# ThomasBrouwer/BNMTF

Measured on NVIDIA B200. Metric: BNMF Gibbs+VB sweeps/sec at 65536x32768 K=20, higher is better.
Workload: dtype f64 (statistics: 48-bit fixed point, exact int8 tcgen05 accumulation; solver, moments, draws: IEEE fp64)

## Files before the change

### bnmtf_b200/_lib.py

```python
import ctypes
import os

_HERE = os.path.dirname(os.path.abspath(__file__))
LIB_PATH = os.environ.get("BNMTF_LIB") or os.path.join(_HERE, "libbnmtf_b200.so")

c_i, c_i64, c_u64, c_d, c_p = ctypes.c_int, ctypes.c_int64, ctypes.c_uint64, ctypes.c_double, ctypes.c_void_p

SIGNATURES = {
    "bnmtf_version": [],
    "bnmtf_last_error": [],
    "bnmtf_ld_for": [c_i64],
    "bnmtf_kp_for": [c_i],
    "bnmtf_gram_len": [c_i],
    "bnmtf_pack_dataset_f64": [c_p, c_p, c_i64, c_i64, c_i64, c_p, c_p, c_p],
    "bnmtf_pack_mask_f64": [c_p, c_i64, c_i64, c_i64, c_p, c_p],
    "bnmtf_transpose_dataset_f64": [c_p, c_p, c_i64, c_i64, c_i64, c_p, c_p, c_i64, c_p],
    "bnmtf_pad_factor_f64": [c_p, c_p, c_i64, c_i, c_i64, c_p, c_p, c_p],
    "bnmtf_stats_rx_f64": [c_p, c_p, c_i64, c_i64, c_p, c_i, c_i, c_p, c_p],
    "bnmtf_fixed_point_digits": [],
    "bnmtf_rx_planes_bytes": [c_i64, c_i64],
    "bnmtf_rx_planes_pack_f64": [c_p, c_p, c_i64, c_i64, c_p, c_p, c_p, c_p, c_p],
    "bnmtf_peer_sync_bytes": [],
    "bnmtf_peer_sync_f64": [c_p, c_p, c_i, c_i, c_i, c_p, c_i, c_p],
    "bnmtf_peer_put_f64": [c_p, c_p, c_i64, c_i64, c_i, c_i, c_p],
    "bnmtf_accumulate_f64": [c_p, c_p, c_i64, c_p],
    "bnmtf_sample_mean_f64": [c_p, c_i64, c_i, c_i, c_i, c_p, c_p],
    "bnmtf_range_guard_f64": [c_p, c_i, c_i64, c_p, c_i, c_i, c_i64, c_p, c_p, c_p, c_p],
    "bnmtf_stats_gated_f64": [c_p, c_p, c_p, c_i64, c_i64, c_p, c_p, c_i, c_i, c_i, c_i, c_p, c_p, c_p, c_p],
    "bnmtf_rx_umma_workspace_bytes": [c_i, c_i64],
    "bnmtf_stats_rx_umma_f64": [c_p, c_p, c_p, c_p, c_i64, c_i64, c_i64, c_p, c_i, c_i, c_i, c_p, c_p, c_i64, c_p],
    "bnmtf_stats_gram_f64": [c_p, c_i64, c_i64, c_p, c_p, c_i, c_i, c_i, c_p, c_p, c_p],
    "bnmtf_gram_full_f64": [c_p, c_p, c_i64, c_i, c_i64, c_p, c_p, c_p],
    "bnmtf_small_cluster_size": [c_i64, c_i64, c_i, c_i],
    "bnmtf_small_sweeps_f64": [c_i, c_p, c_p, c_p, c_p, c_i64, c_i64, c_i64, c_i64, c_i, c_p, c_p, c_p, c_p, c_p, c_p, c_p, c_p,
                               c_p, c_p, c_p, c_p, c_p, c_i64, c_d, c_d, c_d, c_d, c_d, c_d, c_u64, c_i, c_p, c_p, c_p, c_p, c_i, c_i, c_p, c_p, c_p],
    "bnmtf_small_tri_cluster_size": [c_i64, c_i64, c_i, c_i, c_i],
    "bnmtf_small_tri_sweeps_f64": [c_i, c_p, c_p, c_p, c_p, c_i64, c_i64, c_i64, c_i64, c_i, c_i, c_p, c_p, c_p, c_p, c_p, c_p, c_i64,
                                   c_d, c_d, c_d, c_d, c_d, c_d, c_u64, c_i, c_p, c_p, c_p, c_p, c_p, c_p, c_p, c_p, c_p],
    "bnmtf_kmeans_distances_f64": [c_p, c_p, c_i64, c_i64, c_p, c_p, c_i, c_p, c_p],
    "bnmtf_stats_gram_fixup_f64": [c_p, c_i64, c_i64, c_i64, c_p, c_p, c_i, c_i, c_p, c_p, c_p],
    "bnmtf_gram_umma_workspace_bytes": [c_i, c_i, c_i64],
    "bnmtf_stats_gram_umma_f64": [c_p, c_i64, c_i64, c_i64, c_p, c_p, c_i, c_i, c_i, c_i, c_i, c_i, c_i, c_p, c_p, c_p,
                                  c_i64, c_p],
    "bnmf_row_solve_f64": [c_i, c_i64, c_i, c_i, c_i, c_i, c_p, c_p, c_p, c_p, c_p, c_p, c_p, c_p, c_p, c_p, c_p,
                           c_i, c_i, c_d, c_u64, c_p, c_u64, c_i64, c_p, c_p, c_p, c_p, c_p, c_i, c_i, c_p, c_p],
    "bnmtf_masked_metrics_f64": [c_p, c_p, c_i64, c_i64, c_p, c_p, c_i, c_i, c_p, c_p, c_p, c_p, c_p],
    "bnmtf_mstat_reduce_f64": [c_p, c_i64, c_p, c_p, c_p],
    "bnmtf_csr_stats_f64": [c_p, c_p, c_p, c_p, c_p, c_p, c_i64, c_i, c_p, c_p, c_i64, c_p, c_p, c_i, c_p, c_p, c_p, c_p, c_p,
                            c_p, c_p],
    "bnmtf_csr_metrics_f64": [c_p, c_p, c_p, c_i64, c_p, c_p, c_i, c_p, c_i, c_p, c_p, c_p],
    "bnmtf_metrics_from_sums_f64": [c_p, c_p, c_d, c_p, c_p, c_p],
    "bnmtf_select_metrics_f64": [c_p, c_p, c_p, c_p],
    "bnmtf_dense_metrics_f64": [c_p, c_p, c_p, c_i64, c_p, c_i, c_p, c_p],
    "bnmtf_vb_factor_terms_f64": [c_p, c_p, c_p, c_p, c_p, c_i64, c_p, c_i, c_p],
    "bnmtf_reduce8_f64": [c_p, c_i, c_p, c_p],
    "bnmtf_reduce1_f64": [c_p, c_i64, c_p, c_p],
    "bnmf_finish_sweep_f64": [c_i, c_d, c_d, c_d, c_d, c_d, c_i64, c_p, c_p, c_p, c_p, c_p, c_p, c_i, c_u64, c_i, c_p, c_p],
    "bnmtf_nmtf_transform_f64": [c_i64, c_i, c_i, c_i, c_i, c_p, c_p, c_p, c_p, c_p, c_p, c_p, c_p, c_p, c_p],
    "bnmtf_nmtf_sq_f64": [c_i64, c_i, c_i, c_i, c_i, c_p, c_p, c_p, c_p, c_p, c_p, c_p, c_i, c_p, c_p],
    "bnmtf_nmtf_sq_scratch_len": [c_i, c_i, c_i],
    "bnmtf_nmtf_sq_parts": [c_i64, c_i, c_i, c_i],
    "bnmtf_coord_solve_f64": [c_i, c_i, c_p, c_p, c_p, c_p, c_p, c_p, c_p, c_p, c_p, c_p, c_i, c_i, c_d, c_u64, c_p, c_u64, c_p],
    "bnmtf_nmtf_extra_f64": [c_i64, c_i, c_i, c_i, c_p, c_p, c_p, c_p, c_p, c_p, c_p, c_p, c_p],
    "bnmtf_nmtf_mstat_f64": [c_i64, c_i, c_i, c_i, c_p, c_p, c_p, c_p, c_p, c_p, c_p],
    "bnmtf_np_build_pred_f64": [c_p, c_p, c_i64, c_i64, c_i64, c_i, c_p, c_p],
    "bnmtf_np_row_update_f64": [c_p, c_p, c_p, c_i64, c_i64, c_i64, c_p, c_p, c_i, c_p],
    "bnmtf_np_s_update_f64": [c_p, c_p, c_p, c_i64, c_i64, c_i64, c_p, c_i, c_i, c_p, c_i, c_i, c_p, c_p, c_i, c_p],
    "bnmtf_np_metrics_f64": [c_p, c_p, c_p, c_i64, c_i64, c_i64, c_p, c_i, c_p, c_p],
    "bnmtf_small_matmul_f64": [c_p, c_p, c_i64, c_i, c_i, c_i, c_p, c_p],
    "bnmtf_tn_moments_f64": [c_p, c_p, c_i64, c_p, c_p, c_p],
    "bnmtf_tn_draw_f64": [c_p, c_p, c_i64, c_u64, c_u64, c_p, c_p],
    "bnmtf_gamma_draw_f64": [c_d, c_d, c_i64, c_u64, c_u64, c_p, c_p],
    "bnmtf_exponential_draw_f64": [c_p, c_i64, c_u64, c_u64, c_p, c_p],
}
_RESTYPES = {"bnmtf_nmtf_sq_scratch_len": c_i64, "bnmtf_last_error": ctypes.c_char_p, "bnmtf_ld_for": c_i64, "bnmtf_gram_len": c_i64,
             "bnmtf_gram_umma_workspace_bytes": c_i64, "bnmtf_rx_planes_bytes": c_i64,
             "bnmtf_rx_umma_workspace_bytes": c_i64, "bnmtf_peer_sync_bytes": c_i64}
_PLAIN = {"bnmtf_nmtf_sq_scratch_len", "bnmtf_nmtf_sq_parts", "bnmtf_small_cluster_size", "bnmtf_small_tri_cluster_size", "bnmtf_fixed_point_digits", "bnmtf_version", "bnmtf_last_error", "bnmtf_ld_for", "bnmtf_kp_for", "bnmtf_gram_len",
          "bnmtf_gram_umma_workspace_bytes", "bnmtf_rx_planes_bytes", "bnmtf_rx_umma_workspace_bytes", "bnmtf_peer_sync_bytes"}

_lib = None

KERNELS_PER_CALL = {"bnmtf_pack_dataset_f64": 1, "bnmtf_pack_mask_f64": 1, "bnmtf_transpose_dataset_f64": 1,
                    "bnmtf_pad_factor_f64": 1, "bnmtf_stats_rx_f64": 1, "bnmtf_stats_rx_umma_f64": 5,
                    "bnmtf_rx_planes_pack_f64": 2, "bnmtf_range_guard_f64": 1, "bnmtf_stats_gated_f64": 2, "bnmtf_stats_gram_f64": 1, "bnmtf_stats_gram_fixup_f64": 1, "bnmtf_kmeans_distances_f64": 1, "bnmtf_small_sweeps_f64": 1, "bnmtf_small_tri_sweeps_f64": 1, "bnmtf_stats_gram_umma_f64": 4, "bnmtf_mstat_reduce_f64": 2,
                    "bnmtf_metrics_from_sums_f64": 1, "bnmtf_select_metrics_f64": 1,
                    "bnmtf_gram_full_f64": 2, "bnmf_row_solve_f64": 1, "bnmtf_masked_metrics_f64": 3, "bnmtf_csr_stats_f64": 2, "bnmtf_csr_metrics_f64": 2,
                    "bnmtf_dense_metrics_f64": 2, "bnmtf_vb_factor_terms_f64": 1, "bnmtf_reduce8_f64": 1,
                    "bnmtf_reduce1_f64": 1, "bnmf_finish_sweep_f64": 1, "bnmtf_tn_moments_f64": 1, "bnmtf_np_build_pred_f64": 1,
                    "bnmtf_np_row_update_f64": 1, "bnmtf_np_s_update_f64": 2, "bnmtf_np_metrics_f64": 2,
                    "bnmtf_small_matmul_f64": 1, "bnmtf_nmtf_transform_f64": 1, "bnmtf_nmtf_sq_f64": 2,
                    "bnmtf_coord_solve_f64": 1, "bnmtf_nmtf_extra_f64": 1, "bnmtf_nmtf_mstat_f64": 1,
                    "bnmtf_tn_draw_f64": 1, "bnmtf_gamma_draw_f64": 1, "bnmtf_exponential_draw_f64": 1}
launch_count = [0]


class BnmtfError(RuntimeError):
    pass


_seed_calls = [0]


def derive_seed():
    import numpy as np
    st = np.random.get_state()
    keys, pos = st[1], int(st[2])
    _seed_calls[0] += 1
    h = (int(keys[pos % 624]) * 2654435761 + int(keys[(pos + 311) % 624]) * 40503 + pos * 97 + _seed_calls[0] * 1000003)
    return int(h % (2 ** 31 - 1))


def load():
    global _lib
    if _lib is not None:
        return _lib
    if not os.path.exists(LIB_PATH):
        raise BnmtfError("libbnmtf_b200.so not built (run `python -m bnmtf_b200.build` or __graft_entry__.build()); "
                         "there is no CPU fallback")
    lib = ctypes.CDLL(LIB_PATH)
    for name, args in SIGNATURES.items():
        fn = getattr(lib, name)
        fn.argtypes = args
        fn.restype = _RESTYPES.get(name, c_i)
    _lib = lib
    return lib


def call(name, *args):
    lib = load()
    rc = getattr(lib, name)(*args)
    if name in _PLAIN:
        return rc
    if rc != 0:
        raise BnmtfError("%s failed (%d): %s" % (name, rc, lib.bnmtf_last_error().decode()))
    launch_count[0] += KERNELS_PER_CALL.get(name, 1)
    return 0
```

### bnmtf_b200/csrc/api.cu

```cuda
#include <cstdarg>
#include <cstdio>
#include "common.cuh"
#include "../../include/bnmtf_b200.h"

namespace bnmtf {

static thread_local char g_err[512] = "";

void set_error(const char* fmt, ...) {
  va_list ap;
  va_start(ap, fmt);
  vsnprintf(g_err, sizeof(g_err), fmt, ap);
  va_end(ap);
}

int check_launch(const char* what) {
  cudaError_t e = cudaGetLastError();
  if (e != cudaSuccess) {
    set_error("%s: %s", what, cudaGetErrorString(e));
    return -1;
  }
  return 0;
}

int launch_stats_rx(const double*, const uint32_t*, int, int, const double*, int, int, double*, const int*, cudaStream_t);
long long rxu_planes_bytes(long long, long long);
long long rxu_workspace_bytes(int, long long);
int launch_rxu_pack(const double*, const uint32_t*, int, int, uint8_t*, double*, int*, int*, cudaStream_t);
long long peer_sync_bytes();
int launch_peer_sync(const unsigned long long*, unsigned long long*, int, int, int, double*, int, cudaStream_t);
int launch_peer_put(const double*, const unsigned long long*, long long, long long, int, int, cudaStream_t);
int launch_accumulate(double*, const double*, long long, cudaStream_t);
int launch_sample_mean(const double*, long long, int, int, int, double*, cudaStream_t);
int launch_range_guard(const double*, int, int, const double*, int, int, int, const void*, int*, unsigned long long*, cudaStream_t);
int launch_stats_rx_umma(const uint8_t*, const double*, const double*, const uint32_t*, int, int, int, const double*, int, int,
                         int, double*, void*, long long, cudaStream_t);
int launch_stats_gram(const uint32_t*, int, int, const double*, const double*, int, int, int, double*, double*, const int*, cudaStream_t);
int launch_gram_full(const double*, const double*, int, int, int, double*, double*, cudaStream_t);
long long umma_workspace_bytes(int, int, long long);
int launch_stats_gram_fixup(const uint32_t*, int, int, int, const double*, const double*, int, int, double*, double*, cudaStream_t);
int launch_stats_gram_umma(const uint32_t*, int, int, int, const double*, const double*, int, int, int, int, int, int, int,
                           double*, double*, void*, long long, cudaStream_t);
int launch_pad_factor(const double*, const double*, int, int, int, double*, double*, cudaStream_t);
int launch_masked_metrics(const double*, const uint32_t*, int, int, const double*, const double*, int, int, const double*, double*, double*, const int*, cudaStream_t);
int launch_mstat_reduce(const double*, int, double*, double*, cudaStream_t);
int launch_csr_stats(const int64_t*, const int32_t*, const double*, const int64_t*, const int32_t*, const int32_t*, long long, int,
                     const int32_t*, const int32_t*, long long, const double*, const double*, int, double*, double*, double*,
                     double*, double*, double*, cudaStream_t);
int launch_csr_metrics(const int64_t*, const int32_t*, const double*, long long, const double*, const double*, int, double*, int,
                       double*, const int*, cudaStream_t);
int launch_metrics_from_sums(const double*, const double*, double, double*, int*, cudaStream_t);
int launch_select_metrics(const int*, const double*, double*, cudaStream_t);
int launch_vb_factor_terms(const double*, const double*, const double*, const double*, const double*, long long, double*, int, cudaStream_t);
int launch_reduce8(const double*, int, double*, cudaStream_t);
int launch_dense_metrics(const double*, const double*, const double*, long long, double*, int, double*, cudaStream_t);
int launch_reduce1(const double*, long long, double*, cudaStream_t);
int launch_tn_moments(const double*, const double*, long long, double*, double*, cudaStream_t);
int launch_tn_draw(const double*, const double*, long long, unsigned long long, unsigned long long, double*, cudaStream_t);
int launch_gamma_draw(double, double, long long, unsigned long long, unsigned long long, double*, cudaStream_t);
int launch_exponential_draw(const double*, long long, unsigned long long, unsigned long long, double*, cudaStream_t);

struct SmallArgs {
  int mode, I, J, K, ldJ, ldI, nrow[2];
  const double* R; const uint32_t* bits; const double* RT; const uint32_t* bitsT;
  double* fac[2]; double* var[2]; double* mu[2]; double* tauf[2]; const double* lam[2];
  double* scalars; double* trace; unsigned long long* iter; int trace_cap;
  double alpha, beta, digamma_alpha_s, lgamma_alpha, lgamma_alpha_s, min_tn;
  unsigned long long seed;
  int sweeps;
  double* all_U; double* all_V;
  double* sum_U; double* sum_V; int burn_in, thinning;
  double* partial;
  unsigned long long* times;
};
struct TriArgs {
  int mode, I, J, K, L, ldJ, ldI, nrow[2];
  const double* R; const uint32_t* bits; const double* RT; const uint32_t* bitsT;
  double* fac[3]; double* var[3]; double* mu[3]; double* tauf[3]; const double* lam[3];
  double* scalars; double* trace; unsigned long long* iter; int trace_cap;
  double alpha, beta, digamma_alpha_s, lgamma_alpha, lgamma_alpha_s, min_tn;
  unsigned long long seed;
  int sweeps;
  const int* orders;
  double* all_F; double* all_S; double* all_G;
  double* partial;
  double* Hpart; double* Hsum;
  unsigned long long* times;
};
int small_tri_cluster_size(int, int, int, int, int);
int launch_small_tri(TriArgs, cudaStream_t);
int small_cluster_size(int, int, int, int);
int launch_small_sweeps(SmallArgs, cudaStream_t);
int launch_kmeans_dist(const double*, const double*, int, int, const double*, const double*, int, double*, cudaStream_t);
int launch_row_solve(const RowSolveArgs&, cudaStream_t);
int launch_np_build_pred(const double*, const double*, int, int, int, int, double*, cudaStream_t);
int launch_np_row_update(const double*, const uint32_t*, double*, int, int, int, double*, const double*, int, cudaStream_t);
int launch_np_s_update(const double*, const uint32_t*, double*, int, int, int, const double*, int, int, const double*, int,
                       int, double*, double*, int, cudaStream_t);
int launch_np_metrics(const double*, const uint32_t*, const double*, int, int, int, double*, int, cudaStream_t);
int launch_small_matmul(const double*, const double*, int, int, int, int, double*, cudaStream_t);
int launch_nmtf_transform(const TransformArgs&, cudaStream_t);
int launch_nmtf_sq(const SqArgs&, int, double*, cudaStream_t);
long long sq_scratch_len(int, int, int);
int sq_parts(long long, int, int, int);
int launch_coord_solve(const CoordArgs&, cudaStream_t);
int launch_nmtf_extra(const ExtraArgs&, cudaStream_t);
int launch_nmtf_mstat(int, int, int, int, const double*, const double*, const double*, const double*, const double*, double*,
                      cudaStream_t);

int launch_finish(const FinishArgs&, cudaStream_t);

__global__ void k_pack_dataset(const double* __restrict__ Rin, const double* __restrict__ Min, long long rows,
                               long long cols, long long ld, double* __restrict__ Rout, uint32_t* __restrict__ bits) {
  const long long wpr = ld >> 5;
  const long long gw = ((long long)blockIdx.x * blockDim.x + threadIdx.x) >> 5;
  const int lane = threadIdx.x & 31;
  if (gw >= rows * wpr) return;
  const long long row = gw / wpr, w = gw - row * wpr;
  const long long j = w * 32 + lane;
  double r = 0.0;
  bool m = false;
  if (j < cols) {
    m = Min[row * cols + j] != 0.0;
    if (Rin) r = Rin[row * cols + j];
  }
  const uint32_t word = __ballot_sync(0xffffffffu, m);
  if (Rout) Rout[row * ld + j] = r;
  if (lane == 0) bits[row * wpr + w] = word;
}

__global__ void __launch_bounds__(1024) k_transpose_dataset(const double* __restrict__ R, const uint32_t* __restrict__ bits,
                                                          long long rows, long long cols, long long ld,
                                                          double* __restrict__ RT, uint32_t* __restrict__ bitsT,
                                                          long long ldT) {
  __shared__ double tile[32][33];
  __shared__ uint32_t words[32];
  const int tx = threadIdx.x, ty = threadIdx.y;
  const long long r0 = (long long)blockIdx.y * 32, c0 = (long long)blockIdx.x * 32;
  const long long wpr = ld >> 5, wprT = ldT >> 5;
  {
    const long long r = r0 + ty, c = c0 + tx;
    tile[ty][tx] = (r < rows && c < ld) ? R[r * ld + c] : 0.0;
    if (tx == 0) words[ty] = (r < rows && c0 < ld) ? bits[r * wpr + (c0 >> 5)] : 0u;
  }
  __syncthreads();
  {
    const long long dr = c0 + ty, dc = r0 + tx;
    if (dr < cols && dc < ldT) RT[dr * ldT + dc] = (dc < rows) ? tile[tx][ty] : 0.0;
    const uint32_t bit = (words[tx] >> ty) & 1u;
    const uint32_t word = __ballot_sync(0xffffffffu, bit != 0u);
    if (tx == 0 && dr < cols && r0 < ldT) bitsT[dr * wprT + (r0 >> 5)] = word;
  }
}

}

using namespace bnmtf;
#define ST(s) reinterpret_cast<cudaStream_t>(s)

extern "C" {

int bnmtf_version(void) { return 100; }
const char* bnmtf_last_error(void) { return g_err; }
int64_t bnmtf_ld_for(int64_t cols) { return round_up64(cols, 64); }
int bnmtf_kp_for(int K) { return 8 * tiles_for(K); }
int64_t bnmtf_gram_len(int K) { const int nt = tiles_for(K); return (int64_t)nt * (nt + 1) / 2 * 64; }

static int check_k(int K) {
  if (K < 1 || K > 63) { set_error("K=%d out of range (1..63)", K); return -2; }
  return 0;
}

int bnmtf_pack_dataset_f64(const double* R_in, const double* M_in, int64_t rows, int64_t cols, int64_t ld,
                           double* R_out, uint32_t* bits_out, void* stream) {
  if (rows <= 0 || cols <= 0 || ld < cols || ld % 64) { set_error("pack_dataset: bad shape"); return -2; }
  const long long warps = rows * (ld / 32);
  const long long blocks = (warps * 32 + 255) / 256;
  k_pack_dataset<<<(unsigned)blocks, 256, 0, ST(stream)>>>(R_in, M_in, rows, cols, ld, R_out, bits_out);
  return check_launch("pack_dataset");
}

int bnmtf_pack_mask_f64(const double* M_in, int64_t rows, int64_t cols, int64_t ld, uint32_t* bits_out, void* stream) {
  return bnmtf_pack_dataset_f64(nullptr, M_in, rows, cols, ld, nullptr, bits_out, stream);
}

int bnmtf_transpose_dataset_f64(const double* R, const uint32_t* bits, int64_t rows, int64_t cols, int64_t ld,
                                double* RT, uint32_t* bitsT, int64_t ldT, void* stream) {
  if (ld % 64 || ldT % 64 || ldT < rows || ld < cols) { set_error("transpose_dataset: bad shape"); return -2; }
  dim3 grid((unsigned)(ld / 32), (unsigned)(ldT / 32));
  k_transpose_dataset<<<grid, dim3(32, 32), 0, ST(stream)>>>(R, bits, rows, cols, ld, RT, bitsT, ldT);
  return check_launch("transpose_dataset");
}

int bnmtf_pad_factor_f64(const double* X, const double* Var, int64_t n, int K, int64_t n_alloc, double* Xp, double* Vp,
                         void* stream) {
  if (check_k(K)) return -2;
  return launch_pad_factor(X, Var, (int)n, K, (int)n_alloc, Xp, Vp, ST(stream));
}

int bnmtf_stats_rx_f64(const double* R, const uint32_t* bits, int64_t rows, int64_t ld, const double* Xp, int K,
                       int nseg, double* RXpart, void* stream) {
  if (check_k(K)) return -2;
  return launch_stats_rx(R, bits, (int)rows, (int)ld, Xp, K, nseg, RXpart, nullptr, ST(stream));
}

int bnmtf_fixed_point_digits(void) { return kDigits; }

int64_t bnmtf_rx_planes_bytes(int64_t rows, int64_t ld) {
  if (rows <= 0 || ld <= 0 || ld % 64) return -1;
  return rxu_planes_bytes(rows, ld);
}

int bnmtf_rx_planes_pack_f64(const double* R, const uint32_t* bits, int64_t rows, int64_t ld, uint8_t* planes,
                             double* rscale, int32_t* rexp_scratch, int32_t* wide_flag, void* stream) {
  return launch_rxu_pack(R, bits, (int)rows, (int)ld, planes, rscale, rexp_scratch, wide_flag, ST(stream));
}

int64_t bnmtf_peer_sync_bytes(void) { return peer_sync_bytes(); }

int bnmtf_peer_sync_f64(const uint64_t* blocks, uint64_t* epoch, int world, int rank, int channel, double* data, int n,
                        void* stream) {
  if (!blocks || !epoch) { set_error("peer_sync: NULL sync block table / epoch array"); return -2; }
  return launch_peer_sync(reinterpret_cast<const unsigned long long*>(blocks), reinterpret_cast<unsigned long long*>(epoch),
                          world, rank, channel, data, n, ST(stream));
}

int bnmtf_peer_put_f64(const double* local, const uint64_t* peers, int64_t offset, int64_t elems, int world, int rank,
                       void* stream) {
  if (!local || !peers || world < 1 || rank < 0 || rank >= world || offset < 0) { set_error("peer_put: bad arguments"); return -2; }
  return launch_peer_put(local, reinterpret_cast<const unsigned long long*>(peers), offset, elems, world, rank, ST(stream));
}

int bnmtf_accumulate_f64(double* dst, const double* src, int64_t n, void* stream) {
  return launch_accumulate(dst, src, n, ST(stream));
}

int bnmtf_sample_mean_f64(const double* samples, int64_t elems, int n_iter, int burn_in, int thinning, double* out,
                          void* stream) {
  return launch_sample_mean(samples, elems, n_iter, burn_in, thinning, out, ST(stream));
}

int bnmtf_range_guard_f64(const double* Gpart, int nseg, int64_t rows, const double* Gfull, int polarity, int K,
                          int64_t cols, const void* gram_workspace, int32_t* flag, uint64_t* trips, void* stream) {
  if (check_k(K)) return -2;
  return launch_range_guard(Gpart, nseg, (int)rows, Gfull, polarity, K, (int)cols, gram_workspace, flag,
                            reinterpret_cast<unsigned long long*>(trips), ST(stream));
}

int bnmtf_stats_gated_f64(const int32_t* run_flag, const double* R, const uint32_t* bits, int64_t rows, int64_t ld,
                          const double* Xp, const double* Vp, int K, int polarity, int nseg_rx, int nseg_gram,
                          double* RXpart, double* Gpart, double* SVpart, void* stream) {
  if (check_k(K)) return -2;
  if (!run_flag) { set_error("stats_gated: run_flag is NULL"); return -2; }
  if ((Vp == nullptr) != (SVpart == nullptr)) { set_error("stats_gated: Vp and SVpart must be given together"); return -2; }
  int rc = 0;
  if (RXpart) rc = launch_stats_rx(R, bits, (int)rows, (int)ld, Xp, K, nseg_rx, RXpart, run_flag, ST(stream));
  if (rc) return rc;
  (void)polarity;
  return launch_stats_gram(bits, (int)rows, (int)ld, Xp, Vp, K, 1, nseg_gram, Gpart, SVpart, run_flag, ST(stream));
}

int64_t bnmtf_rx_umma_workspace_bytes(int K, int64_t ld) {
  if (K < 1 || K > 32 || ld <= 0) return -1;
  return rxu_workspace_bytes(K, ld);
}

int bnmtf_stats_rx_umma_f64(const uint8_t* planes, const double* rscale, const double* R, const uint32_t* bits,
                            int64_t rows, int64_t ld, int64_t cols, const double* Xp, int K, int nseg, int max_ctas,
                            double* RXpart, void* workspace, int64_t workspace_bytes, void* stream) {
  if (check_k(K)) return -2;
  return launch_stats_rx_umma(planes, rscale, R, bits, (int)rows, (int)ld, (int)cols, Xp, K, nseg, max_ctas, RXpart,
                              workspace, workspace_bytes, ST(stream));
}

int bnmtf_stats_gram_f64(const uint32_t* bits, int64_t rows, int64_t ld, const double* Xp, const double* Vp, int K,
                         int polarity, int nseg, double* Gpart, double* SVpart, void* stream) {
  if (check_k(K)) return -2;
  if ((Vp == nullptr) != (SVpart == nullptr)) { set_error("stats_gram: Vp and SVpart must be given together"); return -2; }
  return launch_stats_gram(bits, (int)rows, (int)ld, Xp, Vp, K, polarity, nseg, Gpart, SVpart, nullptr, ST(stream));
}

int bnmtf_small_cluster_size(int64_t I, int64_t J, int K, int vb) {
  if (I > 1000000 || J > 1000000) return 0;
  return small_cluster_size((int)I, (int)J, K, vb);
}

int bnmtf_small_sweeps_f64(int mode, const double* R, const uint32_t* bits, const double* RT, const uint32_t* bitsT, int64_t I,
                           int64_t J, int64_t ldJ, int64_t ldI, int K, double* U, double* varU, double* muU, double* tauU,
                           const double* lambdaU, double* V, double* varV, double* muV, double* tauV, const double* lambdaV,
                           double* scalars, double* trace, uint64_t* iter, int64_t trace_cap, double alpha, double beta,
                           double digamma_alpha_s, double lgamma_alpha, double lgamma_alpha_s, double minimum_TN, uint64_t seed,
                           int sweeps, double* all_U, double* all_V, double* sum_U, double* sum_V, int burn_in, int thinning,
                           double* partial, uint64_t* times, void* stream) {
  if (mode < 0 || mode > 2) { set_error("small_sweeps: bad mode %d", mode); return -2; }
  if (mode == 1 && (!varU || !varV)) { set_error("small_sweeps: VB needs the variance arrays"); return -2; }
  SmallArgs a;
  a.mode = mode; a.I = (int)I; a.J = (int)J; a.K = K; a.ldJ = (int)ldJ; a.ldI = (int)ldI; a.nrow[0] = a.nrow[1] = 0;
  a.R = R; a.bits = bits; a.RT = RT; a.bitsT = bitsT;
  a.fac[0] = U; a.var[0] = varU; a.mu[0] = muU; a.tauf[0] = tauU; a.lam[0] = lambdaU;
  a.fac[1] = V; a.var[1] = varV; a.mu[1] = muV; a.tauf[1] = tauV; a.lam[1] = lambdaV;
  a.scalars = scalars; a.trace = trace; a.iter = reinterpret_cast<unsigned long long*>(iter); a.trace_cap = (int)trace_cap;
  a.alpha = alpha; a.beta = beta; a.digamma_alpha_s = digamma_alpha_s; a.lgamma_alpha = lgamma_alpha;
  a.lgamma_alpha_s = lgamma_alpha_s; a.min_tn = minimum_TN; a.seed = seed; a.sweeps = sweeps;
  a.all_U = all_U; a.all_V = all_V; a.sum_U = sum_U; a.sum_V = sum_V; a.burn_in = burn_in; a.thinning = thinning < 1 ? 1 : thinning;
  a.partial = partial; a.times = reinterpret_cast<unsigned long long*>(times);
  return launch_small_sweeps(a, ST(stream));
}

int bnmtf_small_tri_cluster_size(int64_t I, int64_t J, int K, int L, int vb) {
  if (I > 1000000 || J > 1000000) return 0;
  return small_tri_cluster_size((int)I, (int)J, K, L, vb);
}

int bnmtf_small_tri_sweeps_f64(int mode, const double* R, const uint32_t* bits, const double* RT, const uint32_t* bitsT, int64_t I,
                               int64_t J, int64_t ldJ, int64_t ldI, int K, int L, double* const* F5, double* const* G5,
                               double* const* S5, double* scalars, double* trace, uint64_t* iter, int64_t trace_cap, double alpha,
                               double beta, double digamma_alpha_s, double lgamma_alpha, double lgamma_alpha_s, double minimum_TN,
                               uint64_t seed, int sweeps, const int32_t* orders, double* all_F, double* all_S, double* all_G,
                               double* partial, double* Hpart, double* Hsum, uint64_t* times, void* stream) {
  if (mode < 0 || mode > 2) { set_error("small_tri_sweeps: bad mode %d", mode); return -2; }
  if (!F5 || !G5 || !S5) { set_error("small_tri_sweeps: factor pointer tables missing"); return -2; }
  TriArgs a;
  a.mode = mode; a.I = (int)I; a.J = (int)J; a.K = K; a.L = L; a.ldJ = (int)ldJ; a.ldI = (int)ldI; a.nrow[0] = a.nrow[1] = 0;
  a.R = R; a.bits = bits; a.RT = RT; a.bitsT = bitsT;
  double* const* tabs[3] = {F5, G5, S5};
  for (int f = 0; f < 3; ++f) {
    a.fac[f] = tabs[f][0]; a.var[f] = tabs[f][1]; a.mu[f] = tabs[f][2]; a.tauf[f] = tabs[f][3]; a.lam[f] = tabs[f][4];
    if (!a.fac[f] || !a.mu[f] || !a.tauf[f] || !a.lam[f] || (mode == 1 && !a.var[f])) { set_error("small_tri_sweeps: missing factor array"); return -2; }
  }
  a.scalars = scalars; a.trace = trace; a.iter = reinterpret_cast<unsigned long long*>(iter); a.trace_cap = (int)trace_cap;
  a.alpha = alpha; a.beta = beta; a.digamma_alpha_s = digamma_alpha_s; a.lgamma_alpha = lgamma_alpha;
  a.lgamma_alpha_s = lgamma_alpha_s; a.min_tn = minimum_TN; a.seed = seed; a.sweeps = sweeps; a.orders = orders;
  a.all_F = all_F; a.all_S = all_S; a.all_G = all_G; a.partial = partial; a.Hpart = Hpart; a.Hsum = Hsum;
  a.times = reinterpret_cast<unsigned long long*>(times);
  return launch_small_tri(a, ST(stream));
}

int bnmtf_kmeans_distances_f64(const double* X, const double* M, int64_t n, int64_t d, const double* centroids,
                               const double* mask_centroids, int K, double* dist, void* stream) {
  return launch_kmeans_dist(X, M, (int)n, (int)d, centroids, mask_centroids, K, dist, ST(stream));
}

int bnmtf_stats_gram_fixup_f64(const uint32_t* bits, int64_t rows, int64_t ld, int64_t cols, const double* Xp, const double* Vp,
                               int K, int polarity, double* Gseg, double* SVseg, void* stream) {
  if (check_k(K)) return -2;
  if ((Vp == nullptr) != (SVseg == nullptr)) { set_error("stats_gram_fixup: Vp and SVseg must be given together"); return -2; }
  return launch_stats_gram_fixup(bits, (int)rows, (int)ld, (int)cols, Xp, Vp, K, polarity, Gseg, SVseg, ST(stream));
}

int64_t bnmtf_gram_umma_workspace_bytes(int K, int vb, int64_t ld) {
  if (K < 1 || K > 63 || ld <= 0) return -1;
  return umma_workspace_bytes(K, vb, ld);
}

int bnmtf_stats_gram_umma_f64(const uint32_t* bits, int64_t rows, int64_t ld, int64_t cols, const double* Xp,
                              const double* Vp, int K, int polarity, int nseg, int tile, int pair, int sums,
                              int max_stages, double* Gpart, double* SVpart, void* workspace, int64_t workspace_bytes,
                              void* stream) {
  if (check_k(K)) return -2;
  if ((Vp == nullptr) != (SVpart == nullptr)) { set_error("stats_gram_umma: Vp and SVpart must be given together"); return -2; }
  return launch_stats_gram_umma(bits, (int)rows, (int)ld, (int)cols, Xp, Vp, K, polarity, nseg, tile, pair, sums,
                                max_stages, Gpart, SVpart, workspace, workspace_bytes, ST(stream));
}

int bnmtf_gram_full_f64(const double* Xp, const double* Vp, int64_t n, int K, int64_t dummy_row, double* Gfull,
                        double* scratch, void* stream) {
  if (check_k(K)) return -2;
  return launch_gram_full(Xp, Vp, (int)n, K, (int)dummy_row, Gfull, scratch, ST(stream));
}

int bnmf_row_solve_f64(int mode, int64_t rows, int K, int nseg_rx, int nseg_g, int polarity, const double* RXpart,
                       const double* Gpart, const double* SVpart, const double* Gfull, double* fac, double* var,
                       double* mu, double* tauf, const double* lambda, const double* scalars, const int* order,
                       int n_order, int apply, double min_tn, uint64_t seed, const uint64_t* iter, uint64_t salt,
                       int64_t row_offset, double* sterm, double* extra, double* mstat, const uint64_t* peer_fac,
                       const uint64_t* peer_var, int n_peers, int my_rank, const int32_t* observed_flag, void* stream) {
  if (check_k(K)) return -2;
  if (peer_fac && (n_peers < 2 || my_rank < 0 || my_rank >= n_peers || !apply)) { set_error("row_solve: bad peer arguments"); return -2; }
  if (mode < 0 || mode > 2) { set_error("row_solve: bad mode %d", mode); return -2; }
  if (mode == BNMTF_MODE_VB && (!var || !SVpart)) { set_error("row_solve: VB needs var and SVpart"); return -2; }
  if (!polarity && !Gfull) { set_error("row_solve: polarity 0 needs Gfull"); return -2; }
  RowSolveArgs a;
  a.mode = mode; a.rows = (int)rows; a.K = K; a.nseg_rx = nseg_rx; a.nseg_g = nseg_g; a.polarity = polarity;
  a.n_order = n_order; a.apply = apply; a.RXpart = RXpart; a.Gpart = Gpart; a.SVpart = SVpart; a.Gfull = Gfull;
  a.fac = fac; a.var = var; a.mu = mu; a.tauf = tauf; a.lambda = lambda; a.scalars = scalars; a.order = order;
  a.min_tn = min_tn; a.seed = seed; a.iter = reinterpret_cast<const unsigned long long*>(iter); a.salt = salt;
  a.sterm = sterm; a.extra = extra; a.mstat = mstat; a.row_offset = row_offset;
  a.peer_fac = reinterpret_cast<double* const*>(peer_fac);
  a.peer_var = (mode == BNMTF_MODE_VB) ? reinterpret_cast<double* const*>(peer_var) : nullptr;
  a.n_peers = peer_fac ? n_peers : 0; a.my_rank = my_rank;
  a.observed_flag = observed_flag;
  if (a.peer_fac && mode == BNMTF_MODE_VB && !a.peer_var) { set_error("row_solve: VB peer exchange needs peer_var"); return -2; }
  return launch_row_solve(a, ST(stream));
}

int bnmtf_masked_metrics_f64(const double* R, const uint32_t* bits, int64_t rows, int64_t ld, const double* Ap,
                             const double* Bp, int K, int nseg, const double* statics3, double* partials, double* out8,
                             const int* run_flag, void* stream) {
  if (check_k(K)) return -2;
  return launch_masked_metrics(R, bits, (int)rows, (int)ld, Ap, Bp, K, nseg, statics3, partials, out8, run_flag, ST(stream));
}

int bnmtf_csr_stats_f64(const int64_t* rowptr, const int32_t* colidx, const double* val, const int64_t* item_begin,
                        const int32_t* item_row, const int32_t* item_slot, int64_t n_items, int chunk, const int32_t* heavy_row,
                        const int32_t* heavy_first, int64_t n_heavy, const double* Xp, const double* Vp, int K, double* RXpart,
                        double* Gpart, double* SVpart, double* RXc, double* Gc, double* SVc, void* stream) {
  if (check_k(K)) return -2;
  if (Vp && !SVpart) { set_error("csr_stats: Vp given without SVpart"); return -2; }
  return launch_csr_stats(rowptr, colidx, val, item_begin, item_row, item_slot, n_items, chunk, heavy_row, heavy_first, n_heavy,
                          Xp, Vp, K, RXpart, Gpart, SVpart, RXc, Gc, SVc, ST(stream));
}

int bnmtf_csr_metrics_f64(const int64_t* rowptr, const int32_t* colidx, const double* val, int64_t rows, const double* Ap,
                          const double* Bp, int K, double* partials, int nparts, double* out8, const int* run_flag, void* stream) {
  if (check_k(K)) return -2;
  return launch_csr_metrics(rowptr, colidx, val, rows, Ap, Bp, K, partials, nparts, out8, run_flag, ST(stream));
}

int bnmtf_mstat_reduce_f64(const double* mstat, int64_t rows, double* partial, double* out4, void* stream) {
  if (rows <= 0) { set_error("mstat_reduce: no rows"); return -2; }
  return launch_mstat_reduce(mstat, (int)rows, partial, out4, ST(stream));
}

int bnmtf_metrics_from_sums_f64(const double* sums4, const double* statics3, double guard, double* out8, int* direct_flag,
                                void* stream) {
  return launch_metrics_from_sums(sums4, statics3, guard, out8, direct_flag, ST(stream));
}

int bnmtf_select_metrics_f64(const int* flag, const double* direct8, double* out8, void* stream) {
  return launch_select_metrics(flag, direct8, out8, ST(stream));
}

int bnmtf_vb_factor_terms_f64(const double* ex, const double* var, const double* mu, const double* tauf,
                              const double* lambda, int64_t n, double* partials, int nblocks, void* stream) {
  return launch_vb_factor_terms(ex, var, mu, tauf, lambda, n, partials, nblocks, ST(stream));
}

int bnmtf_dense_metrics_f64(const double* R, const double* P, const double* M, int64_t n, double* partials, int nblocks,
                            double* out8, void* stream) {
  if (nblocks < 1) { set_error("dense_metrics: nblocks < 1"); return -2; }
  return launch_dense_metrics(R, P, M, n, partials, nblocks, out8, ST(stream));
}

int bnmtf_reduce8_f64(const double* partials, int n, double* out8, void* stream) {
  return launch_reduce8(partials, n, out8, ST(stream));
}
int bnmtf_reduce1_f64(const double* x, int64_t n, double* out, void* stream) {
  return launch_reduce1(x, n, out, ST(stream));
}

int bnmf_finish_sweep_f64(int mode, double alpha, double beta, double digamma_alpha_s, double lgamma_alpha,
                          double lgamma_alpha_s, int64_t n_factor_elems, const double* m8, const double* ex1,
                          const double* el8, double* scalars, double* trace, uint64_t* iter, int trace_cap,
                          uint64_t seed, int update_tau, const uint64_t* trace_window, void* stream) {
  FinishArgs a;
  a.mode = mode; a.alpha = alpha; a.beta = beta; a.digamma_alpha_s = digamma_alpha_s; a.lgamma_alpha = lgamma_alpha;
  a.lgamma_alpha_s = lgamma_alpha_s; a.n_factor_elems = (int)n_factor_elems; a.m8 = m8; a.ex1 = ex1; a.el8 = el8;
  a.scalars = scalars; a.trace = trace; a.iter = reinterpret_cast<unsigned long long*>(iter); a.trace_cap = trace_cap;
  a.seed = seed; a.update_tau = update_tau; a.trace_window = reinterpret_cast<const unsigned long long*>(trace_window);
  if (mode == BNMTF_MODE_VB && (!ex1 || !el8)) { set_error("finish_sweep: VB needs ex1 and el8"); return -2; }
  return launch_finish(a, ST(stream));
}

int bnmtf_np_build_pred_f64(const double* A, const double* B, int64_t rows, int64_t cols, int64_t ld, int K, double* P,
                            void* stream) {
  return launch_np_build_pred(A, B, (int)rows, (int)cols, (int)ld, K, P, ST(stream));
}
int bnmtf_np_row_update_f64(const double* R, const uint32_t* bits, double* P, int64_t rows, int64_t cols, int64_t ld,
                            double* A, const double* B, int K, void* stream) {
  return launch_np_row_update(R, bits, P, (int)rows, (int)cols, (int)ld, A, B, K, ST(stream));
}
int bnmtf_np_s_update_f64(const double* R, const uint32_t* bits, double* P, int64_t rows, int64_t cols, int64_t ld,
                          const double* F, int K, int k, const double* G, int L, int l, double* S, double* partials,
                          int nparts, void* stream) {
  if (nparts < 1) { set_error("np_s_update: nparts < 1"); return -2; }
  return launch_np_s_update(R, bits, P, (int)rows, (int)cols, (int)ld, F, K, k, G, L, l, S, partials, nparts, ST(stream));
}
int bnmtf_np_metrics_f64(const double* R, const uint32_t* bits, const double* P, int64_t rows, int64_t cols, int64_t ld,
                         double* partials, int nparts, double* out8, void* stream) {
  int rc = launch_np_metrics(R, bits, P, (int)rows, (int)cols, (int)ld, partials, nparts, ST(stream));
  if (rc) return rc;
  return launch_reduce8(partials, nparts, out8, ST(stream));
}
int bnmtf_small_matmul_f64(const double* A, const double* B, int64_t n, int p, int q, int transB, double* C, void* stream) {
  return launch_small_matmul(A, B, (int)n, p, q, transB, C, ST(stream));
}

int bnmtf_nmtf_transform_f64(int64_t rows, int Ks, int Lo, int polarity, int vb, const double* RXo, const double* Go,
                             const double* SVo, const double* Gfull_o, const double* Smat, const double* varS,
                             double* RXs, double* Gs, double* SVs, void* stream) {
  if (check_k(Ks) || check_k(Lo)) return -2;
  if (vb && (!SVo || !varS || !SVs)) { set_error("nmtf_transform: VB needs SVo, varS, SVs"); return -2; }
  TransformArgs a;
  a.rows = (int)rows; a.Ks = Ks; a.Lo = Lo; a.polarity = polarity; a.vb = vb; a.RXo = RXo; a.Go = Go; a.SVo = SVo;
  a.Gfull_o = Gfull_o; a.Smat = Smat; a.varS = varS; a.RXs = RXs; a.Gs = Gs; a.SVs = SVs;
  return launch_nmtf_transform(a, ST(stream));
}
int bnmtf_nmtf_sq_f64(int64_t rows, int K, int L, int polarity, int vb, const double* RXo, const double* Go,
                      const double* SVo, const double* Gfull_o, const double* F, const double* varF, double* partial,
                      int nparts, double* out, void* stream) {
  if (check_k(K) || check_k(L)) return -2;
  SqArgs a;
  a.rows = (int)rows; a.K = K; a.L = L; a.polarity = polarity; a.vb = vb; a.RXo = RXo; a.Go = Go; a.SVo = SVo;
  a.Gfull_o = Gfull_o; a.F = F; a.varF = varF; a.partial = partial;
  return launch_nmtf_sq(a, nparts, out, ST(stream));
}
int64_t bnmtf_nmtf_sq_scratch_len(int K, int L, int vb) {
  if (check_k(K) || check_k(L)) return -2;
  return (int64_t)sq_scratch_len(K, L, vb);
}
int bnmtf_nmtf_sq_parts(int64_t rows, int K, int L, int vb) {
  if (check_k(K) || check_k(L)) return -2;
  return sq_parts((long long)rows, K, L, vb);
}
int bnmtf_coord_solve_f64(int mode, int D, const double* H, const double* prec, const double* rhs, const double* lambda,
                          double* x, double* var, double* mu, double* tauf, const double* scalars, const int* order,
                          int n_order, int apply, double min_tn, uint64_t seed, const uint64_t* iter, uint64_t salt,
                          void* stream) {
  if (D < 1 || D > 4096) { set_error("coord_solve: D=%d out of range", D); return -2; }
  if (mode == BNMTF_MODE_VB && !var) { set_error("coord_solve: VB needs var"); return -2; }
  CoordArgs a;
  a.mode = mode; a.D = D; a.n_order = n_order; a.apply = apply; a.H = H; a.prec = prec; a.rhs = rhs; a.lambda = lambda;
  a.x = x; a.var = var; a.mu = mu; a.tauf = tauf; a.scalars = scalars; a.order = order; a.min_tn = min_tn; a.seed = seed;
  a.iter = reinterpret_cast<const unsigned long long*>(iter); a.salt = salt;
  return launch_coord_solve(a, ST(stream));
}
int bnmtf_nmtf_extra_f64(int64_t rows, int K, int L, int polarity, const double* Go, const double* SVo,
                         const double* Gfull_o, const double* G, const double* varG, const double* S, const double* varS,
                         double* extra, void* stream) {
  if (check_k(K) || check_k(L)) return -2;
  ExtraArgs a;
  a.rows = (int)rows; a.K = K; a.L = L; a.polarity = polarity; a.Go = Go; a.SVo = SVo; a.Gfull_o = Gfull_o; a.G = G;
  a.varG = varG; a.S = S; a.varS = varS; a.extra = extra;
  return launch_nmtf_extra(a, ST(stream));
}

int bnmtf_nmtf_mstat_f64(int64_t rows, int K, int L, int polarity, const double* RXo, const double* Go,
                         const double* Gfull_o, const double* G, const double* S, double* mstat, void* stream) {
  if (check_k(K) || check_k(L)) return -2;
  return launch_nmtf_mstat((int)rows, K, L, polarity, RXo, Go, Gfull_o, G, S, mstat, ST(stream));
}

int bnmtf_tn_moments_f64(const double* mu, const double* tau, int64_t n, double* ex, double* var, void* stream) {
  return launch_tn_moments(mu, tau, n, ex, var, ST(stream));
}
int bnmtf_tn_draw_f64(const double* mu, const double* tau, int64_t n, uint64_t seed, uint64_t stream_id, double* out,
                      void* stream) {
  return launch_tn_draw(mu, tau, n, seed, stream_id, out, ST(stream));
}
int bnmtf_gamma_draw_f64(double shape, double rate, int64_t n, uint64_t seed, uint64_t stream_id, double* out,
                         void* stream) {
  return launch_gamma_draw(shape, rate, n, seed, stream_id, out, ST(stream));
}
int bnmtf_exponential_draw_f64(const double* lambda, int64_t n, uint64_t seed, uint64_t stream_id, double* out,
                               void* stream) {
  return launch_exponential_draw(lambda, n, seed, stream_id, out, ST(stream));
}

}
```

### bnmtf_b200/csrc/common.cuh

```cuda
#pragma once
#include <cuda_runtime.h>
#include <stdint.h>
#include <math.h>

#ifndef __CUDA_ARCH__
#define BNMTF_HOST 1
#endif

namespace bnmtf {

void set_error(const char* fmt, ...);
int check_launch(const char* what);

#ifndef BNMTF_DIGITS
#define BNMTF_DIGITS 6
#endif
constexpr int kDigits = BNMTF_DIGITS;
static_assert(kDigits == 6 || kDigits == 7, "BNMTF_DIGITS must be 6 or 7");

constexpr int kMaxTiles = 8;
constexpr double kInvSqrt2 = 0.70710678118654752440;
constexpr double kInvSqrt2Pi = 0.39894228040143267794;
constexpr double kSqrt2 = 1.4142135623730951;
constexpr double kSqrt2Pi = 2.5066282746310002;
constexpr double kLog2Pi = 1.8378770664093454836;

__host__ __device__ inline int round_up(int x, int m) { return (x + m - 1) / m * m; }
__host__ __device__ inline int64_t round_up64(int64_t x, int64_t m) { return (x + m - 1) / m * m; }
__host__ __device__ inline int tiles_for(int K) { return (K + 1 + 7) / 8; }
__host__ __device__ inline int tile_pair(int a, int b, int nt) { return a * nt - a * (a - 1) / 2 + (b - a); }


enum Mode { MODE_GIBBS = 0, MODE_VB = 1, MODE_ICM = 2 };

enum Scalar {
  S_TAU = 0,
  S_LOGTAU = 1,
  S_ALPHA_S = 2, S_BETA_S = 3,
  S_SUM_E2 = 4,
  S_ESD = 5,
  S_MSE = 6, S_R2 = 7, S_RP = 8, S_ELBO = 9,
  S_SUM_R = 10, S_SUM_R2 = 11, S_OMEGA = 12,
  S_COUNT = 16
};
constexpr int kGramFullParts = 296;
constexpr int kTraceWidth = 8;

struct RowSolveArgs {
  int mode, rows, K, nseg_rx, nseg_g, polarity, n_order, apply;
  const double* RXpart; const double* Gpart; const double* SVpart; const double* Gfull;
  double* fac; double* var; double* mu; double* tauf; const double* lambda;
  const double* scalars; const int* order; double min_tn;
  unsigned long long seed; const unsigned long long* iter; unsigned long long salt;
  long long row_offset;
  double* sterm;
  double* extra;
  double* mstat;
  double* const* peer_fac; double* const* peer_var; int n_peers, my_rank;
  const int* observed_flag;
};

struct FinishArgs {
  int mode; double alpha, beta, digamma_alpha_s, lgamma_alpha, lgamma_alpha_s; int n_factor_elems;
  const double* m8; const double* ex1; const double* el8;
  double* scalars; double* trace; unsigned long long* iter; int trace_cap;
  unsigned long long seed; int update_tau;
  const unsigned long long* trace_window;
};

struct TransformArgs {
  int rows, Ks, Lo, polarity, vb;
  const double* RXo; const double* Go; const double* SVo; const double* Gfull_o;
  const double* Smat; const double* varS;
  double* RXs; double* Gs; double* SVs;
};

struct SqArgs {
  int rows, K, L, polarity, vb;
  const double* RXo; const double* Go; const double* SVo; const double* Gfull_o;
  const double* F; const double* varF;
  double* partial;
};

struct CoordArgs {
  int mode, D, n_order, apply;
  const double* H; const double* prec; const double* rhs; const double* lambda;
  double* x; double* var; double* mu; double* tauf;
  const double* scalars; const int* order; double min_tn;
  unsigned long long seed; const unsigned long long* iter; unsigned long long salt;
};

struct ExtraArgs {
  int rows, K, L, polarity;
  const double* Go; const double* SVo; const double* Gfull_o;
  const double* G; const double* varG;
  const double* S; const double* varS;
  double* extra;
};

#ifdef __CUDACC__
__device__ __forceinline__ void dmma884(double& c0, double& c1, double a, double b) {
  asm volatile("mma.sync.aligned.m8n8k4.row.col.f64.f64.f64.f64 {%0,%1}, {%2}, {%3}, {%0,%1};\n"
               : "+d"(c0), "+d"(c1) : "d"(a), "d"(b));
}

__device__ __forceinline__ double warp_sum(double v) {
#pragma unroll
  for (int o = 16; o > 0; o >>= 1) v += __shfl_xor_sync(0xffffffffu, v, o);
  return v;
}

struct Philox {
  uint32_t key[2];
  uint32_t ctr[4];
  __device__ Philox(uint64_t seed, uint64_t stream, uint64_t index) {
    key[0] = (uint32_t)seed; key[1] = (uint32_t)(seed >> 32) ^ (uint32_t)(stream >> 32);
    ctr[0] = 0; ctr[1] = (uint32_t)index; ctr[2] = (uint32_t)(index >> 32); ctr[3] = (uint32_t)stream;
  }
  __device__ void next4(uint32_t out[4]) {
    uint32_t c0 = ctr[0], c1 = ctr[1], c2 = ctr[2], c3 = ctr[3], k0 = key[0], k1 = key[1];
#pragma unroll
    for (int r = 0; r < 10; ++r) {
      uint32_t hi0 = __umulhi(0xD2511F53u, c0), lo0 = 0xD2511F53u * c0;
      uint32_t hi1 = __umulhi(0xCD9E8D57u, c2), lo1 = 0xCD9E8D57u * c2;
      c0 = hi1 ^ c1 ^ k0; c1 = lo1; c2 = hi0 ^ c3 ^ k1; c3 = lo0;
      k0 += 0x9E3779B9u; k1 += 0xBB67AE85u;
    }
    out[0] = c0; out[1] = c1; out[2] = c2; out[3] = c3;
    ++ctr[0];
  }
  __device__ void uniform2(double& u0, double& u1) {
    uint32_t r[4]; next4(r);
    uint64_t a = ((uint64_t)r[0] << 21) ^ (uint64_t)(r[1] >> 11);
    uint64_t b = ((uint64_t)r[2] << 21) ^ (uint64_t)(r[3] >> 11);
    u0 = ((double)a + 0.5) * (1.0 / 9007199254740992.0);
    u1 = ((double)b + 0.5) * (1.0 / 9007199254740992.0);
  }
};

__device__ __forceinline__ double clean_nonneg(double v) { return (v >= 0.0 && isfinite(v)) ? v : 0.0; }

__device__ __forceinline__ double erfc_ref(double a) {
  const double t = fabs(a);
  if (t < 1.0) return erfc(a);
  const double y = exp(-__dmul_rn(t, t)) * erfcx(t);
  return a < 0.0 ? 2.0 - y : y;
}

__device__ __forceinline__ void tn_moments(double mu, double tau, double& e, double& v) {
  double sigma = 1.0 / sqrt(tau);
  if (mu < -30.0 * sigma) {
    e = 1.0 / (fabs(mu) * tau);
    v = e * e;
  } else {
    double x = -mu / sigma;
    double lam = (exp(-0.5 * __dmul_rn(x, x)) / kSqrt2Pi) / (0.5 * erfc_ref(x / kSqrt2));
    e = mu + sigma * lam;
    v = sigma * sigma * (1.0 - lam * (lam - x));
  }
  e = clean_nonneg(e);
  v = clean_nonneg(v);
}

__device__ __forceinline__ double tn_draw(double mu, double tau, Philox& rng) {
  if (tau == 0.0) return 0.0;
  double sigma = 1.0 / sqrt(tau);
  double a = -mu / sigma;
  double z;
  if (!(a > 4.0)) {
    double u0, u1; rng.uniform2(u0, u1);
    double tail = 0.5 * erfc(a * kInvSqrt2);
    z = -normcdfinv(u0 * tail);
    z = fmax(z, a);
  } else {
    double lam = 0.5 * (a + sqrt(a * a + 4.0));
    z = a;
    for (int tries = 0; tries < 64; ++tries) {
      double u0, u1; rng.uniform2(u0, u1);
      z = a - log(u0) / lam;
      double d = z - lam;
      if (u1 <= exp(-0.5 * d * d)) break;
    }
  }
  return clean_nonneg(mu + sigma * z);
}
#endif

__host__ __device__ __forceinline__ uint32_t sparse_split(uint32_t v, uint32_t& v0, uint32_t& v1, uint32_t& meta) {
  const uint32_t m = 0x11111111u;
  const uint32_t b0 = v & m, b1 = (v >> 1) & m, b2 = (v >> 2) & m, b3 = (v >> 3) & m;
  const uint32_t c1 = b0 & b1;
  const uint32_t c2 = (b0 ^ b1) & b2;
  const uint32_t i0b0 = b1 & ~b0, i0b1 = b2 & ~(b0 | b1);
  meta = i0b0 | (i0b1 << 1) | ((m & ~c2) << 2) | ((m & ~c1) << 3);
  v0 = b0 | b1 | b2;
  v1 = c1 | c2 | (b3 & ~(c1 | c2));
  return ((c1 & b2) << 2) | ((b3 & (c1 | c2)) << 3);
}


}
```

### bnmtf_b200/csrc/gram_umma.cu

```cuda
#include <cstdlib>
#include "umma.cuh"

namespace bnmtf {

constexpr int UG_SLICES = kDigits;
constexpr int UG_TOP = 8 * UG_SLICES - 1;
constexpr int UG_ROWS = 128;
constexpr int UG_GROUPS = 4;
constexpr int UG_EXP_WARPS = 4 * UG_GROUPS;
constexpr int UG_THREADS = (UG_EXP_WARPS + 3) * 32;
constexpr int UG_MASK_BUFS = 3;

struct UmmaPlan {
  int K, vb, sums, sp;
  int nh_full;
  int ng;
  int nc;
  int nch;
  int cpc;
  int cpc_last;
  int nh_last;
  int gran;
};
constexpr int UG_CHUNK_ROWS = 512;
constexpr int UG_SP_ACC_COLS = 480;

__host__ __device__ inline UmmaPlan make_umma_plan(int K, int vb, int sums, int pair, int sp = 0) {
  UmmaPlan p;
  p.K = K; p.vb = vb; p.sums = sums; p.sp = sp;
  p.ng = K * (K + 1) / 2;
  p.nc = p.ng + (vb ? K : 0) + (sums ? K : 0);
  p.cpc = (sp ? UG_SP_ACC_COLS : 512) / UG_SLICES;
  p.nh_full = ((p.cpc * UG_SLICES + 1) / 2 + 15) / 16 * 16;
  p.nch = (p.nc + p.cpc - 1) / p.cpc;
  p.cpc_last = p.nc - (p.nch - 1) * p.cpc;
  p.gran = (pair && !sp) ? 32 : 16;
  const int nd = p.cpc_last * UG_SLICES;
  p.nh_last = ((nd + 1) / 2 + p.gran - 1) / p.gran * p.gran;
  return p;
}
__host__ __device__ inline int umma_cols_of(const UmmaPlan& p, int ch) { return ch == p.nch - 1 ? p.cpc_last : p.cpc; }
__host__ __device__ inline int umma_nhalf_of(const UmmaPlan& p, int ch) { return ch == p.nch - 1 ? p.nh_last : p.nh_full; }

__host__ __device__ inline void umma_col_pair(int c, const UmmaPlan& pl, int& a, int& b) {
  const int K = pl.K, ng = pl.ng;
  if (c >= ng) {
    a = c - ng; b = -1;
    if (!pl.vb || a >= K) { a -= pl.vb ? K : 0; b = -2; }
    return;
  }
  int aa = 0, rem = c;
  while (rem >= K - aa) { rem -= K - aa; ++aa; }
  a = aa; b = aa + rem;
}

__global__ void __launch_bounds__(256) k_ug_colmax(const double* __restrict__ Xp, const double* __restrict__ Vp, int n,
                                                  int KP, UmmaPlan pl, unsigned long long* __restrict__ colmax) {
  extern __shared__ double xs[];
  constexpr int JT = 64;
  const int K = pl.K;
  unsigned long long m[4] = {0ull, 0ull, 0ull, 0ull};
  for (int j0 = blockIdx.x * JT; j0 < n; j0 += gridDim.x * JT) {
    __syncthreads();
    for (int i = threadIdx.x; i < JT * K; i += blockDim.x) {
      const int jj = i / K, k = i - jj * K;
      const int j = j0 + jj;
      xs[k * (JT + 1) + jj] = (j < n) ? Xp[(size_t)j * KP + k] : 0.0;
      if (pl.vb) xs[(K + k) * (JT + 1) + jj] = (j < n) ? Vp[(size_t)j * KP + k] : 0.0;
    }
    __syncthreads();
    auto tile_max = [&](int c) {
      int a, b;
      umma_col_pair(c, pl, a, b);
      const double* xa = xs + (b == -1 ? (K + a) : a) * (JT + 1);
      const double* xb = b < 0 ? nullptr : xs + b * (JT + 1);
      unsigned long long mm = 0ull;
      for (int jj = 0; jj < JT; ++jj) {
        const double p = xb ? xa[jj] * xb[jj] : xa[jj];
        const unsigned long long u = (unsigned long long)__double_as_longlong(fabs(p));
        mm = u > mm ? u : mm;
      }
      return mm;
    };
#pragma unroll
    for (int q = 0; q < 4; ++q) {
      const int c = threadIdx.x + 256 * q;
      if (c < pl.nc) { const unsigned long long mm = tile_max(c); m[q] = mm > m[q] ? mm : m[q]; }
    }
    for (int c = threadIdx.x + 1024; c < pl.nc; c += 256) atomicMax(colmax + c, tile_max(c));
  }
#pragma unroll
  for (int q = 0; q < 4; ++q) {
    const int c = threadIdx.x + 256 * q;
    if (c < pl.nc && m[q]) atomicMax(colmax + c, m[q]);
  }
}

__global__ void k_ug_scales(const unsigned long long* __restrict__ colmax, int nc, double* __restrict__ cscale,
                            int* __restrict__ cexp) {
  const int c = blockIdx.x * blockDim.x + threadIdx.x;
  if (c >= nc) return;
  const double m = __longlong_as_double((long long)colmax[c]);
  int e = 0;
  double s;
  if (!isfinite(m)) { s = __longlong_as_double(0x7ff8000000000000ll); }
  else {
    if (m > 0.0) { frexp(m, &e); }
    s = scalbn(1.0, e - UG_TOP);
  }
  cscale[c] = s;
  cexp[c] = e;
}

__global__ void __launch_bounds__(128) k_ug_quantize(const double* __restrict__ Xp, const double* __restrict__ Vp, int n,
                                                    int KP, long long ldb, UmmaPlan pl, const int* __restrict__ cexp,
                                                    uint8_t* __restrict__ Bd) {
  extern __shared__ double xs[];
  constexpr int JT = 128, XS = JT + 2;
  const int j0 = blockIdx.x * JT;
  const int K = pl.K;
  int16_t* tab = reinterpret_cast<int16_t*>(xs + (size_t)(pl.vb ? 2 : 1) * K * XS);
  for (int i = threadIdx.x; i < JT * K; i += blockDim.x) {
    const int jj = i / K, k = i - jj * K;
    const int j = j0 + jj;
    xs[k * XS + jj] = (j < n) ? Xp[(size_t)j * KP + k] : 0.0;
    if (pl.vb) xs[(K + k) * XS + jj] = (j < n) ? Vp[(size_t)j * KP + k] : 0.0;
  }
  for (int c = threadIdx.x; c < pl.nc; c += blockDim.x) {
    int a, b;
    umma_col_pair(c, pl, a, b);
    tab[2 * c] = (int16_t)a; tab[2 * c + 1] = (int16_t)b;
  }
  __syncthreads();
  const int jg = (threadIdx.x & 31) * 4, sub = threadIdx.x >> 5;
  const int nvalid = n - (j0 + jg);
  for (int c = sub + 4 * blockIdx.y; c < pl.nc; c += 4 * gridDim.y) {
    const int ch = c / pl.cpc, cl = c - ch * pl.cpc;
    const int a = tab[2 * c], b = tab[2 * c + 1];
    const double* xa = xs + (b == -1 ? (K + a) : a) * XS + jg;
    const double* xb = b < 0 ? nullptr : xs + b * XS + jg;
    const int sh = UG_TOP - cexp[c];
    const bool fast = sh > -1000 && sh < 1000;
    const double pw = fast ? __longlong_as_double((long long)(sh + 1023) << 52) : 0.0;
    uint32_t lo[4], hi[4];
#pragma unroll
    for (int i = 0; i < 4; ++i) {
      const double p = xb ? xa[i] * xb[i] : xa[i];
      long long q = fast ? __double2ll_rn(p * pw) : llrint(scalbn(p, sh));
      q = q > (1ll << UG_TOP) - 1 ? (1ll << UG_TOP) - 1 : (q < -(1ll << UG_TOP) ? -(1ll << UG_TOP) : q);
      const unsigned long long u = i < nvalid ? (unsigned long long)(q + (1ll << UG_TOP)) : 0ull;
      lo[i] = (uint32_t)u; hi[i] = (uint32_t)(u >> 32);
    }
    uint32_t w[8];
    {
      const uint32_t a01 = __byte_perm(lo[0], lo[1], 0x5140), a23 = __byte_perm(lo[2], lo[3], 0x5140);
      const uint32_t c01 = __byte_perm(lo[0], lo[1], 0x7362), c23 = __byte_perm(lo[2], lo[3], 0x7362);
      const uint32_t e01 = __byte_perm(hi[0], hi[1], 0x5140), e23 = __byte_perm(hi[2], hi[3], 0x5140);
      const uint32_t g01 = __byte_perm(hi[0], hi[1], 0x7362), g23 = __byte_perm(hi[2], hi[3], 0x7362);
      w[0] = __byte_perm(a01, a23, 0x5410); w[1] = __byte_perm(a01, a23, 0x7632);
      w[2] = __byte_perm(c01, c23, 0x5410); w[3] = __byte_perm(c01, c23, 0x7632);
      w[4] = __byte_perm(e01, e23, 0x5410); w[5] = __byte_perm(e01, e23, 0x7632);
      w[6] = __byte_perm(g01, g23, 0x5410); w[7] = __byte_perm(g01, g23, 0x7632);
    }
    uint8_t* dst = Bd + ((size_t)ch * UG_CHUNK_ROWS + (size_t)cl * UG_SLICES) * ldb + j0 + jg;
    if (j0 + jg < ldb) {
#pragma unroll
      for (int s = 0; s < UG_SLICES; ++s) *reinterpret_cast<uint32_t*>(dst + (size_t)s * ldb) = w[s];
    }
  }
}

struct UmmaGramArgs {
  const uint32_t* bits; int rows, wpr, cols, polarity;
  int ktiles, tiles_per_seg;
  UmmaPlan pl;
  const double* cscale;
  double* Gout; double* SVout;
  int KP, gl;
  int mask_tma;
  int stages_of[2];
  int dbg;
};

template <int KT, bool PAIR, bool SP, bool MC>
__global__ void __launch_bounds__(UG_THREADS, 1) k_gram_umma(const __grid_constant__ CUtensorMap tmap_full,
                                                            const __grid_constant__ CUtensorMap tmap_last,
                                                            const __grid_constant__ CUtensorMap tmap_bits, UmmaGramArgs a) {
  extern __shared__ uint8_t smem_raw[];
  uint8_t* smem = reinterpret_cast<uint8_t*>((reinterpret_cast<uintptr_t>(smem_raw) + 1023) & ~(uintptr_t)1023);
  const int tid = threadIdx.x, warp = tid >> 5, lane = tid & 31;
  const UmmaPlan& pl = a.pl;
  static_assert(!MC || PAIR, "the multicast form is built on CTA pairs");
  const uint32_t crank = PAIR ? cluster_ctarank() : 0u;
  const uint32_t rank = crank & 1u;
  const uint32_t lead = crank & ~1u;
  const int rb = blockIdx.x, ch = blockIdx.y, seg = blockIdx.z;
  const int n_half = umma_nhalf_of(pl, ch), cpc = umma_cols_of(pl, ch);
  const CUtensorMap& tmap = ch == pl.nch - 1 ? tmap_last : tmap_full;
  constexpr int AKT = SP ? KT / 2 : KT;
  static_assert(!SP || KT == 128, "the sparse form runs 128-column stages");
  const int A_BYTES = UG_ROWS * AKT, B_BYTES = (PAIR ? n_half : 2 * n_half) * KT, STAGE = A_BYTES + B_BYTES;
  const int stages = ch == pl.nch - 1 ? a.stages_of[1] : a.stages_of[0];
  constexpr int MASK_WIN_BYTES = UG_ROWS * 64;
  const uint32_t mask_base = smem_u32(smem) + (uint32_t)stages * STAGE;
  uint64_t* bars = reinterpret_cast<uint64_t*>(smem + (size_t)stages * STAGE + UG_MASK_BUFS * MASK_WIN_BYTES);
  uint32_t* tmem_slot = reinterpret_cast<uint32_t*>(bars + 2 * stages + 1 + 2 * UG_MASK_BUFS);
  int* cnt_smem = reinterpret_cast<int*>(tmem_slot + 2);
  uint16_t* pair_tab = reinterpret_cast<uint16_t*>(cnt_smem + UG_EXP_WARPS * 32);
  const uint32_t smem_base = smem_u32(smem);
  const uint32_t bar_base = smem_u32(bars);
#define FULL_BAR(s) (bar_base + 8u * (uint32_t)(s))
#define EMPTY_BAR(s) (bar_base + 8u * (uint32_t)(stages + (s)))
#define ACCUM_BAR (bar_base + 8u * (uint32_t)(2 * stages))
#define MASK_FULL(b) (bar_base + 8u * (uint32_t)(2 * stages + 1 + (b)))
#define MASK_EMPTY(b) (bar_base + 8u * (uint32_t)(2 * stages + 1 + UG_MASK_BUFS + (b)))

  const int kt_begin = seg * a.tiles_per_seg;
  const int kt_end = min(a.ktiles, kt_begin + a.tiles_per_seg);
  const int ntile = kt_end - kt_begin;

  if (warp == UG_EXP_WARPS && lane == 0) {
    const uint32_t nfull = 4u + (PAIR ? (rank == 0 ? 2u : 0u) : 1u);
    for (int s = 0; s < stages; ++s) { mbar_init(FULL_BAR(s), nfull); mbar_init(EMPTY_BAR(s), MC ? 2 : 1); }
    mbar_init(ACCUM_BAR, 1);
    for (int b = 0; b < UG_MASK_BUFS; ++b) { mbar_init(MASK_FULL(b), 1); mbar_init(MASK_EMPTY(b), 4 * (stages < UG_GROUPS ? stages : UG_GROUPS)); }
    fence_barrier_init();
    asm volatile("prefetch.tensormap [%0];" ::"l"(&tmap) : "memory");
  }
  if (warp == UG_EXP_WARPS + 1) {
    if (PAIR) {
      asm volatile("tcgen05.alloc.cta_group::2.sync.aligned.shared::cta.b32 [%0], 512;" ::"r"(smem_u32(tmem_slot)) : "memory");
      asm volatile("tcgen05.relinquish_alloc_permit.cta_group::2.sync.aligned;" ::: "memory");
    } else {
      asm volatile("tcgen05.alloc.cta_group::1.sync.aligned.shared::cta.b32 [%0], 512;" ::"r"(smem_u32(tmem_slot)) : "memory");
      asm volatile("tcgen05.relinquish_alloc_permit.cta_group::1.sync.aligned;" ::: "memory");
    }
  }
  for (int cl = tid; cl < cpc; cl += UG_THREADS) {
    const int c = ch * pl.cpc + cl;
    int pa = 0xff, pb = 0xfe;
    if (c < pl.nc) { int x, y; umma_col_pair(c, pl, x, y); pa = x; pb = y == -1 ? 0xff : (y == -2 ? 0xfd : y); }
    pair_tab[cl] = (uint16_t)((pa << 8) | pb);
  }
  tc_fence_before();
  if (PAIR) cluster_sync_all(); else __syncthreads();
  tc_fence_after();
  const uint32_t tmem_base = *tmem_slot;

  if (warp < UG_EXP_WARPS) {
    const int r = tid & (UG_ROWS - 1), half = tid >> 7;
    const int row = rb * UG_ROWS + r;
    const bool live = row < a.rows;
    const uint32_t* mrow = a.bits + (size_t)(live ? row : 0) * a.wpr;
    constexpr int WPT = KT / 32;
    constexpr int CPT = KT / 16;
    const int NG = stages < UG_GROUPS ? stages : UG_GROUPS;
    const uint32_t flip = a.polarity ? 0u : 0xffffffffu;
    const uint32_t row_off = (uint32_t)(r >> 3) * (8 * AKT) + (uint32_t)(r & 7) * AKT;
    const uint32_t key = AKT == 128 ? (uint32_t)(r & 7) : (uint32_t)((r >> 1) & 3);
    const uint32_t tlane_e = tmem_base + ((uint32_t)((warp & 3) * 32) << 16) + (uint32_t)UG_SP_ACC_COLS;
    int cnt = 0;
    constexpr int WIN = 16 / WPT;
    const bool mask_tma = a.mask_tma != 0;
    int s = half % stages;
    uint32_t ph = (uint32_t)(half / stages) & 1u;
    const int koff = KT == 64 ? (kt_begin & 1) : 0;
    int c = (half + koff) % WIN, qb = ((half + koff) / WIN) % UG_MASK_BUFS;
    uint32_t qph = (uint32_t)(((half + koff) / WIN) / UG_MASK_BUFS) & 1u;
    const int s_step = NG % stages, ph_step = (NG / stages) & 1;
    for (int it = half < NG ? half : ntile; it < ntile; it += NG) {
      const int wbase = (kt_begin + it) * WPT;
      uint32_t w[WPT];
      int release_win = -1;
      if (mask_tma) {
        mbar_wait(MASK_FULL(qb), qph);
        const uint32_t rowb = mask_base + (uint32_t)qb * MASK_WIN_BYTES + (uint32_t)r * 64u;
        if constexpr (WPT == 4) {
          const uint32_t addr = rowb + ((((uint32_t)c) ^ (uint32_t)((r >> 1) & 3)) << 4);
          asm volatile("ld.shared.v4.b32 {%0, %1, %2, %3}, [%4];" : "=r"(w[0]), "=r"(w[1]), "=r"(w[2]), "=r"(w[3]) : "r"(addr) : "memory");
        } else {
          const uint32_t addr = rowb + ((((uint32_t)(c >> 1)) ^ (uint32_t)((r >> 1) & 3)) << 4) + (uint32_t)(c & 1) * 8u;
          asm volatile("ld.shared.v2.b32 {%0, %1}, [%2];" : "=r"(w[0]), "=r"(w[1]) : "r"(addr) : "memory");
        }
        release_win = (c + NG >= WIN || it + NG >= ntile) ? qb : -1;
      } else {
#pragma unroll
        for (int i = 0; i < WPT; ++i) w[i] = (live && wbase + i < a.wpr) ? mrow[wbase + i] : 0u;
      }
      const bool edge = (wbase + WPT) * 32 > a.cols;
      uint32_t y[CPT][4];
      uint32_t meta[WPT];
#pragma unroll
      for (int i = 0; i < WPT; ++i) {
        uint32_t v = w[i] ^ flip;
        if (edge) {
          const int jb = (wbase + i) * 32;
          if (jb + 32 > a.cols) v = jb >= a.cols ? 0u : (v & ((1u << (a.cols - jb)) - 1u));
        }
        v = live ? v : 0u;
        if constexpr (SP) {
          uint32_t v0, v1;
          const uint32_t ovf = sparse_split(v, v0, v1, meta[i]);
          cnt += __popc(v) - __popc(ovf);
          const uint32_t z = v0 | (v1 << 1);
#pragma unroll
          for (int q = 0; q < 4; ++q) y[i][q] = (((z >> (8 * q)) & 0x33u) * 0x00081081u) & 0x01010101u;
        } else {
          cnt += __popc(v);
#pragma unroll
          for (int q = 0; q < 8; ++q) y[2 * i + (q >> 2)][q & 3] = (((v >> (4 * q)) & 0xfu) * 0x00204081u) & 0x01010101u;
        }
      }
      mbar_wait(EMPTY_BAR(s), ph ^ 1u);
      const uint32_t abase = smem_base + (uint32_t)s * STAGE + row_off;
      if constexpr (SP) {
        static_assert(WPT == 4, "four metadata columns per stage");
        asm volatile("tcgen05.st.sync.aligned.32x32b.x4.b32 [%0], {%1, %2, %3, %4};"
                     ::"r"(tlane_e + 4u * (uint32_t)s), "r"(meta[0]), "r"(meta[1]), "r"(meta[2]), "r"(meta[3]) : "memory");
      }
      if (!((a.dbg & 2) && it >= stages))
#pragma unroll
      for (int cc = 0; cc < (SP ? WPT : CPT); ++cc) {
        const uint32_t addr = abase + ((((uint32_t)cc) ^ key) << 4);
        asm volatile("st.shared.v4.b32 [%0], {%1, %2, %3, %4};" ::"r"(addr), "r"(y[cc][0]), "r"(y[cc][1]), "r"(y[cc][2]), "r"(y[cc][3]) : "memory");
      }
      if constexpr (SP) {
        asm volatile("tcgen05.wait::st.sync.aligned;" ::: "memory");
        tc_fence_before();
      }
      fence_proxy_async();
      __syncwarp();
      if (lane == 0) {
        mbar_arrive(FULL_BAR(s));
        if (release_win >= 0) mbar_arrive(MASK_EMPTY(release_win));
      }
      s += s_step; ph ^= (uint32_t)ph_step;
      if (s >= stages) { s -= stages; ph ^= 1u; }
      c += NG;
      while (c >= WIN) { c -= WIN; if (++qb == UG_MASK_BUFS) { qb = 0; qph ^= 1u; } }
    }
    cnt_smem[tid] = cnt;
    asm volatile("bar.sync 1, %0;" ::"n"(UG_EXP_WARPS * 32) : "memory");
    cnt = 0;
#pragma unroll
    for (int g = 0; g < UG_GROUPS; ++g) cnt += cnt_smem[r + g * UG_ROWS];

    mbar_wait(ACCUM_BAR, 0u);
    tc_fence_after();
    const uint32_t tlane = tmem_base + ((uint32_t)((warp & 3) * 32) << 16);
    double* grow = a.Gout + ((size_t)seg * a.rows + (live ? row : 0)) * a.gl;
    double* srow = a.SVout ? a.SVout + ((size_t)seg * a.rows + (live ? row : 0)) * a.KP : nullptr;
    const int NT = a.KP >> 3;
    constexpr int GRP = 8, GCOLS = GRP * UG_SLICES;
    static_assert(GCOLS % 16 == 0, "group width must be a multiple of the 16-column load");
    for (int g0 = half * GRP; g0 < cpc; g0 += UG_GROUPS * GRP) {
      uint32_t d[GCOLS / 16][16];
#pragma unroll
      for (int q = 0; q < GCOLS / 16; ++q) {
        if (g0 * UG_SLICES + 16 * q + 16 <= 512) tmem_ld16(tlane + (uint32_t)(g0 * UG_SLICES + 16 * q), d[q]);
      }
      tmem_ld_wait();
#pragma unroll
      for (int i = 0; i < GRP; ++i) {
        const int cl = g0 + i;
        if (cl >= cpc || !live) break;
        const uint32_t pr = pair_tab[cl];
        const int pa = pr >> 8, pb = pr & 0xff;
        if (pb == 0xfe) continue;
#define DD(sl) d[(i * UG_SLICES + (sl)) / 16][(i * UG_SLICES + (sl)) % 16]
        const long long lo = (long long)DD(0) + ((long long)DD(1) << 8) + ((long long)DD(2) << 16) + ((long long)DD(3) << 24);
        long long hi = 0;
#pragma unroll
        for (int sl = 4; sl < UG_SLICES; ++sl)
          hi += ((long long)(int)DD(sl) - (sl == UG_SLICES - 1 ? 128ll * cnt : 0ll)) << (8 * (sl - 4));
#undef DD
        const double v = fma((double)hi, 4294967296.0, (double)lo) * a.cscale[ch * pl.cpc + cl];
        if (pb == 0xff) {
          if (srow) srow[pa] = v;
        } else if (pb == 0xfd) {
          const int ta = pa >> 3, tb = pl.K >> 3;
          grow[(ta * NT - ta * (ta - 1) / 2 + (tb - ta)) * 64 + (pa & 7) * 8 + (pl.K & 7)] = v;
        } else {
          const int ta = pa >> 3, tb = pb >> 3;
          const int p = ta * NT - ta * (ta - 1) / 2 + (tb - ta);
          grow[p * 64 + (pa & 7) * 8 + (pb & 7)] = v;
          if (ta == tb) grow[p * 64 + (pb & 7) * 8 + (pa & 7)] = v;
        }
      }
      __syncwarp();
    }
    if (live && ch == 0 && half == 0) {
      const int tk = pl.K >> 3;
      grow[(tk * NT - tk * (tk - 1) / 2) * 64 + (pl.K & 7) * 9] = (double)cnt;
    }
    tc_fence_before();
  } else if (warp == UG_EXP_WARPS) {
    if (lane == 0) {
      int s = -1;
      uint32_t ph = 1u;
      for (int it = 0; it < ntile; ++it) {
        if (++s == stages) s = 0;
        if (s == 0) ph ^= 1u;
        mbar_wait(EMPTY_BAR(s), ph ^ 1u);
        const uint32_t bdst = smem_base + (uint32_t)s * STAGE + A_BYTES;
        const int x = (kt_begin + it) * KT;
        if (PAIR) {
          if ((a.dbg & 1) && it >= stages) { if (rank == 0) mbar_arrive(FULL_BAR(s)); continue; }
          if (rank == 0) mbar_expect_tx(FULL_BAR(s), 2u * (uint32_t)B_BYTES);
          const int hh = n_half >> 1;
          if (MC) {
            const uint32_t which = crank >> 1;
            tma_load_2d_pair_mc(bdst + which * (uint32_t)hh * KT, &tmap, x, ch * UG_CHUNK_ROWS + (int)which * n_half + (int)rank * hh,
                                FULL_BAR(s) & 0xFEFFFFFFu, (uint16_t)((1u << crank) | (1u << (crank ^ 2u))));
            continue;
          }
          const uint32_t lead_full = mapa_u32(FULL_BAR(s), lead);
          tma_load_2d_pair(bdst, &tmap, x, ch * UG_CHUNK_ROWS + (int)rank * hh, lead_full);
          tma_load_2d_pair(bdst + (uint32_t)hh * KT, &tmap, x, ch * UG_CHUNK_ROWS + n_half + (int)rank * hh, lead_full);
          continue;
        }
        if ((a.dbg & 1) && it >= stages) { mbar_arrive(FULL_BAR(s)); continue; }
        mbar_expect_tx(FULL_BAR(s), (uint32_t)B_BYTES);
        tma_load_2d(bdst, &tmap, x, ch * UG_CHUNK_ROWS, FULL_BAR(s));
        tma_load_2d(bdst + (uint32_t)n_half * KT, &tmap, x, ch * UG_CHUNK_ROWS + n_half, FULL_BAR(s));
      }
    }
    __syncwarp();
  } else if (warp == UG_EXP_WARPS + 2) {
    if (lane == 0 && a.mask_tma) {
      constexpr int WIN = 512 / KT;
      const int koff = KT == 64 ? (kt_begin & 1) : 0;
      const int nwin = (ntile + koff + WIN - 1) / WIN;
      for (int q = 0; q < nwin; ++q) {
        const int qb = q % UG_MASK_BUFS;
        if (q >= UG_MASK_BUFS) mbar_wait(MASK_EMPTY(qb), ((uint32_t)(q / UG_MASK_BUFS) & 1u) ^ 1u);
        mbar_expect_tx(MASK_FULL(qb), (uint32_t)MASK_WIN_BYTES);
        tma_load_2d(mask_base + (uint32_t)qb * MASK_WIN_BYTES, &tmap_bits, (kt_begin - koff + q * WIN) * (KT / 32), rb * UG_ROWS, MASK_FULL(qb));
      }
    }
    __syncwarp();
  } else {
    if (PAIR && lane == 0 && rank != 0) {
      int s = -1;
      uint32_t ph = 1u;
      for (int it = 0; it < ntile; ++it) {
        if (++s == stages) s = 0;
        if (s == 0) ph ^= 1u;
        mbar_wait(FULL_BAR(s), ph);
        mbar_arrive_remote(mapa_u32(FULL_BAR(s), lead));
      }
    }
    if (rank == 0) {
      const uint32_t idesc = (SP ? 4u : 0u) | (2u << 4) | ((uint32_t)(n_half >> 3) << 17) |
                             ((uint32_t)((PAIR ? 2 * UG_ROWS : UG_ROWS) >> 4) << 24);
      const uint64_t ad0 = umma_desc<AKT>(smem_base);
      const uint64_t bd00 = umma_desc<KT>(smem_base + A_BYTES);
      const uint64_t bd10 = umma_desc<KT>(smem_base + A_BYTES + (uint32_t)(PAIR ? n_half >> 1 : n_half) * KT);
      const uint64_t dstep = (uint64_t)(STAGE >> 4);
      const uint32_t tm1 = tmem_base + (uint32_t)n_half;
      int s = 0;
      uint32_t ph = 0;
      uint64_t soff = 0;
      mbar_wait(FULL_BAR(0), 0u);
      for (int it = 0; it < ntile; ++it) {
        tc_fence_after();
        const uint64_t ad = ad0 + soff, bd0 = bd00 + soff, bd1 = bd10 + soff;
        int sn = s + 1;
        uint32_t phn = ph;
        if (sn == stages) { sn = 0; phn ^= 1u; }
        if (SP) {
          if (elect_one()) {
            const uint32_t e0 = tmem_base + (uint32_t)UG_SP_ACC_COLS + 4u * (uint32_t)s;
#pragma unroll
            for (int kk = 0; kk < KT / 64; ++kk) {
              const uint32_t acc = (it > 0 || kk > 0) ? 1u : 0u;
              umma_i8_sp<PAIR>(tmem_base, ad + 2 * kk, bd0 + 4 * kk, e0 + 2u * kk, idesc, acc);
              umma_i8_sp<PAIR>(tm1, ad + 2 * kk, bd1 + 4 * kk, e0 + 2u * kk, idesc, acc);
            }
            if (PAIR) umma_commit_pair(EMPTY_BAR(s), MC ? 0xFu : 3u); else umma_commit(EMPTY_BAR(s));
          }
        } else if (elect_one()) {
#pragma unroll
          for (int kk = 0; kk < KT / 32; ++kk) {
            const uint32_t acc = (it > 0 || kk > 0) ? 1u : 0u;
            if (PAIR) {
              umma_i8_pair(tmem_base, ad + 2 * kk, bd0 + 2 * kk, idesc, acc);
              umma_i8_pair(tm1, ad + 2 * kk, bd1 + 2 * kk, idesc, acc);
            } else {
              umma_i8(tmem_base, ad + 2 * kk, bd0 + 2 * kk, idesc, acc);
              umma_i8(tm1, ad + 2 * kk, bd1 + 2 * kk, idesc, acc);
            }
          }
          if (PAIR) umma_commit_pair(EMPTY_BAR(s), MC ? 0xFu : 3u); else umma_commit(EMPTY_BAR(s));
        }
        __syncwarp();
        if (it + 1 < ntile) mbar_wait(FULL_BAR(sn), phn);
        s = sn; ph = phn;
        soff = s == 0 ? 0 : soff + dstep;
      }
      if (elect_one()) { if (PAIR) umma_commit_pair(ACCUM_BAR, 3u << lead); else umma_commit(ACCUM_BAR); }
    }
    __syncwarp();
  }
  if (PAIR) cluster_sync_all(); else __syncthreads();
  if (warp == UG_EXP_WARPS + 1) {
    tc_fence_after();
    if (PAIR) asm volatile("tcgen05.dealloc.cta_group::2.sync.aligned.b32 %0, 512;" ::"r"(tmem_base) : "memory");
    else asm volatile("tcgen05.dealloc.cta_group::1.sync.aligned.b32 %0, 512;" ::"r"(tmem_base) : "memory");
  }
#undef FULL_BAR
#undef EMPTY_BAR
#undef ACCUM_BAR
#undef MASK_FULL
#undef MASK_EMPTY
}

__global__ void __launch_bounds__(256) k_range_guard(const double* __restrict__ Gpart, int nseg, int rows, int gl,
                                                    const double* __restrict__ Gfull, int polarity, int K, int NT, int cols,
                                                    const unsigned long long* __restrict__ colmax, int* __restrict__ flag,
                                                    unsigned long long* __restrict__ trips) {
  const long long gid = (long long)blockIdx.x * blockDim.x + threadIdx.x;
  if (gid >= (long long)rows * K) return;
  const int row = (int)(gid / K), k = (int)(gid - (long long)row * K);
  const int ta = k >> 3, tk = K >> 3;
  const int di = (ta * NT - ta * (ta - 1) / 2) * 64 + (k & 7) * 9;
  const int ci = (tk * NT - tk * (tk - 1) / 2) * 64 + (K & 7) * 9;
  double d = 0.0, cnt = 0.0;
  for (int sgm = 0; sgm < nseg; ++sgm) {
    const double* g = Gpart + ((size_t)sgm * rows + row) * gl;
    d += g[di];
    cnt += g[ci];
  }
  if (!polarity) { d = Gfull[di] - d; cnt = (double)cols - cnt; }
  const double cmax = __longlong_as_double((long long)colmax[k * K - k * (k - 1) / 2]);
  if (cnt > 0.0 && d < 5.9604644775390625e-8 * cnt * cmax) {
    if (atomicOr(flag, 1) == 0 && trips) atomicAdd(trips, 1ull);
  }
}

int launch_range_guard(const double* Gpart, int nseg, int rows, const double* Gfull, int polarity, int K, int cols,
                       const void* workspace, int* flag, unsigned long long* trips, cudaStream_t st) {
  if (rows <= 0 || nseg <= 0) { set_error("range_guard: bad shape"); return -2; }
  const int nt = tiles_for(K);
  cudaMemsetAsync(flag, 0, sizeof(int), st);
  const long long tot = (long long)rows * K;
  k_range_guard<<<(unsigned)((tot + 255) / 256), 256, 0, st>>>(Gpart, nseg, rows, nt * (nt + 1) / 2 * 64, Gfull, polarity, K, nt,
                                                            cols, static_cast<const unsigned long long*>(workspace), flag, trips);
  return check_launch("range_guard");
}

static size_t ws_digits_offset(const UmmaPlan& pl) {
  size_t o = (size_t)pl.nc * 8 * 2 + (size_t)((pl.nc + 1) / 2 * 2) * 4;
  return (o + 1023) / 1024 * 1024;
}

static long long plan_workspace_bytes(const UmmaPlan& pl, long long ld) {
  return (long long)ws_digits_offset(pl) + (long long)pl.nch * UG_CHUNK_ROWS * ld;
}

long long umma_workspace_bytes(int K, int vb, long long ld) {
  long long m = 0;
  for (int sums = 0; sums < 2; ++sums)
    for (int pair = 0; pair < 4; ++pair) {
      const long long b = plan_workspace_bytes(make_umma_plan(K, vb, sums, pair & 1, pair >> 1), ld);
      m = b > m ? b : m;
    }
  return m;
}

int launch_stats_gram_umma(const uint32_t* bits, int rows, int ld, int cols, const double* Xp, const double* Vp, int K,
                           int polarity, int nseg, int kt, int pair, int sums, int max_stages, double* Gout, double* SVout,
                           void* workspace, long long workspace_bytes, cudaStream_t st) {
  if (rows <= 0 || ld <= 0 || ld % 64 || nseg <= 0 || cols <= 0 || cols > ld) { set_error("stats_gram_umma: bad shape"); return -2; }
  if (kt != 64 && kt != 128) { set_error("stats_gram_umma: tile width must be 64 or 128"); return -2; }
  if ((long long)ld * 255 >= 2147483647ll) { set_error("stats_gram_umma: more than 8.4M columns would overflow the int32 accumulators"); return -2; }
  const int vb = Vp != nullptr;
  const int sp = (pair >> 1) & 1;
  const int mc = (pair >> 2) & 1;
  pair &= 1;
  if (mc && !pair) { set_error("stats_gram_umma: the multicast form needs CTA pairs"); return -2; }
  if (sp && kt != 128) { set_error("stats_gram_umma: the sparse form needs tile width 128"); return -2; }
  const UmmaPlan pl = make_umma_plan(K, vb, sums, pair, sp);
  if (workspace_bytes < plan_workspace_bytes(pl, ld)) { set_error("stats_gram_umma: workspace too small"); return -2; }
  EncodeTiledFn encode = get_encode_fn();
  if (!encode) { set_error("stats_gram_umma: cuTensorMapEncodeTiled not available"); return -3; }

  uint8_t* ws = static_cast<uint8_t*>(workspace);
  unsigned long long* colmax = reinterpret_cast<unsigned long long*>(ws);
  double* cscale = reinterpret_cast<double*>(ws + (size_t)pl.nc * 8);
  int* cexp = reinterpret_cast<int*>(ws + (size_t)pl.nc * 16);
  uint8_t* Bd = ws + ws_digits_offset(pl);
  const int KP = 8 * tiles_for(K);
  const int nt = tiles_for(K);

  cudaMemsetAsync(colmax, 0, (size_t)pl.nc * 8, st);
  {
    const size_t sm = (size_t)(vb ? 2 : 1) * K * 65 * sizeof(double);
    int nbm = (cols + 63) / 64;
    if (nbm > 296) nbm = 296;
    k_ug_colmax<<<nbm, 256, sm, st>>>(Xp, Vp, cols, KP, pl, colmax);
    k_ug_scales<<<(pl.nc + 127) / 128, 128, 0, st>>>(colmax, pl.nc, cscale, cexp);
    const size_t sq = (size_t)(vb ? 2 : 1) * K * 130 * sizeof(double) + (size_t)pl.nc * 4;
    if (sq > 48 * 1024) cudaFuncSetAttribute(k_ug_quantize, cudaFuncAttributeMaxDynamicSharedMemorySize, (int)sq);
    k_ug_quantize<<<dim3((ld + 127) / 128, 4), 128, sq, st>>>(Xp, Vp, cols, KP, (long long)ld, pl, cexp, Bd);
  }
  if (check_launch("stats_gram_umma prepass")) return -1;

  CUtensorMap tmaps[2];
  for (int which = 0; which < 2; ++which) {
    const int nh = which ? pl.nh_last : pl.nh_full;
    const cuuint64_t gdim[2] = {(cuuint64_t)ld, (cuuint64_t)pl.nch * UG_CHUNK_ROWS};
    const cuuint64_t gstr[1] = {(cuuint64_t)ld};
    const cuuint32_t box[2] = {(cuuint32_t)kt, (cuuint32_t)(pair ? nh / 2 : nh)};
    const cuuint32_t estr[2] = {1, 1};
    const CUresult r = encode(&tmaps[which], CU_TENSOR_MAP_DATA_TYPE_UINT8, 2, Bd, gdim, gstr, box, estr, CU_TENSOR_MAP_INTERLEAVE_NONE,
                              kt == 128 ? CU_TENSOR_MAP_SWIZZLE_128B : CU_TENSOR_MAP_SWIZZLE_64B,
                              CU_TENSOR_MAP_L2_PROMOTION_L2_256B, CU_TENSOR_MAP_FLOAT_OOB_FILL_NONE);
    if (r != CUDA_SUCCESS) { set_error("stats_gram_umma: cuTensorMapEncodeTiled failed (%d)", (int)r); return -3; }
  }

  UmmaGramArgs a;
  a.bits = bits; a.rows = rows; a.wpr = ld / 32; a.cols = cols; a.polarity = polarity;
  a.ktiles = (ld + kt - 1) / kt;
  a.tiles_per_seg = (a.ktiles + nseg - 1) / nseg;
  const int nseg_eff = (a.ktiles + a.tiles_per_seg - 1) / a.tiles_per_seg;
  if (nseg_eff != nseg) { set_error("stats_gram_umma: nseg=%d leaves empty segments (use <= %d)", nseg, nseg_eff); return -2; }
  a.pl = pl; a.cscale = cscale; a.Gout = Gout; a.SVout = SVout; a.KP = KP; a.gl = nt * (nt + 1) / 2 * 64;
  const int tail = UG_MASK_BUFS * UG_ROWS * 64 + (2 * 16 + 1 + 2 * UG_MASK_BUFS) * 8 + 16 + UG_EXP_WARPS * 32 * 4 + 2 * pl.cpc + 64;
  size_t smem = 0;
  for (int which = 0; which < 2; ++which) {
    const int nh = which ? pl.nh_last : pl.nh_full;
    const int stage_bytes = (sp ? UG_ROWS / 2 : UG_ROWS) * kt + (pair ? nh : 2 * nh) * kt;
    int stages = (227 * 1024 - 1024 - tail) / stage_bytes;
    if (stages > 16) stages = 16;
    if (sp && stages > 8) stages = 8;
    if (max_stages > 0 && stages > max_stages) stages = max_stages;
    if (stages < 2) { set_error("stats_gram_umma: stage does not fit"); return -2; }
    a.stages_of[which] = stages;
    const size_t need = (size_t)stages * stage_bytes + tail + 1024;
    smem = need > smem ? need : smem;
  }
  { const char* e = getenv("BNMTF_UMMA_DBG"); a.dbg = e ? atoi(e) : 0; }
  if (smem < 116 * 1024) smem = 116 * 1024;
  int rbs = (rows + UG_ROWS - 1) / UG_ROWS;
  if (pair) rbs = (rbs + 1) / 2 * 2;
  if (mc) rbs = (rbs + 3) / 4 * 4;
  dim3 grid(rbs, pl.nch, nseg);
  CUtensorMap tmap_bits = tmaps[0];
  a.mask_tma = (ld % 128 == 0 && reinterpret_cast<uintptr_t>(bits) % 16 == 0) ? 1 : 0;
  { const char* e = getenv("BNMTF_GRAM_MASK_TMA"); if (e && atoi(e) == 0) a.mask_tma = 0; }
  if (a.mask_tma) {
    const cuuint64_t gdim[2] = {(cuuint64_t)(ld / 32), (cuuint64_t)rows};
    const cuuint64_t gstr[1] = {(cuuint64_t)(ld / 32) * 4};
    const cuuint32_t box[2] = {16, (cuuint32_t)UG_ROWS};
    const cuuint32_t estr[2] = {1, 1};
    const CUresult r = encode(&tmap_bits, CU_TENSOR_MAP_DATA_TYPE_UINT32, 2, const_cast<uint32_t*>(bits), gdim, gstr, box, estr,
                              CU_TENSOR_MAP_INTERLEAVE_NONE, CU_TENSOR_MAP_SWIZZLE_64B, CU_TENSOR_MAP_L2_PROMOTION_L2_128B,
                              CU_TENSOR_MAP_FLOAT_OOB_FILL_NONE);
    if (r != CUDA_SUCCESS) { set_error("stats_gram_umma: cuTensorMapEncodeTiled (mask) failed (%d)", (int)r); return -3; }
  }
  void (*kern)(const CUtensorMap, const CUtensorMap, const CUtensorMap, UmmaGramArgs) =
      mc ? (sp ? k_gram_umma<128, true, true, true> : (kt == 128 ? k_gram_umma<128, true, false, true> : k_gram_umma<64, true, false, true>))
      : sp ? (pair ? k_gram_umma<128, true, true, false> : k_gram_umma<128, false, true, false>)
         : kt == 128 ? (pair ? k_gram_umma<128, true, false, false> : k_gram_umma<128, false, false, false>)
                     : (pair ? k_gram_umma<64, true, false, false> : k_gram_umma<64, false, false, false>);
  cudaFuncSetAttribute(kern, cudaFuncAttributeMaxDynamicSharedMemorySize, (int)smem);
  cudaLaunchConfig_t cfg = {};
  cfg.gridDim = grid; cfg.blockDim = dim3(UG_THREADS); cfg.dynamicSmemBytes = smem; cfg.stream = st;
  cudaLaunchAttribute attr[1];
  attr[0].id = cudaLaunchAttributeClusterDimension;
  attr[0].val.clusterDim.x = mc ? 4 : (pair ? 2 : 1); attr[0].val.clusterDim.y = 1; attr[0].val.clusterDim.z = 1;
  cfg.attrs = attr; cfg.numAttrs = 1;
  const cudaError_t le = cudaLaunchKernelEx(&cfg, kern, tmaps[0], tmaps[1], tmap_bits, a);
  if (le != cudaSuccess) { set_error("stats_gram_umma: launch failed: %s", cudaGetErrorString(le)); cudaGetLastError(); return -1; }
  return check_launch("stats_gram_umma");
}

}
```

### bnmtf_b200/csrc/stats.cu

```cuda
#include "common.cuh"

namespace bnmtf {

template <int NT>
__global__ void __launch_bounds__(256, 3) k_stats_rx(const double* __restrict__ R, const uint32_t* __restrict__ bits,
                                                 int rows, int ld, const double* __restrict__ Xp, int seg_cols,
                                                 double* __restrict__ out, const int* __restrict__ run_flag) {
  if (run_flag && *run_flag == 0) return;
  constexpr int KP = 8 * NT;
  constexpr int CH = NT <= 4 ? 128 : 64;
  constexpr int XS = KP + 1;
  __shared__ double xs[CH * XS];

  const int warp = threadIdx.x >> 5, lane = threadIdx.x & 31, g = lane >> 2, t = lane & 3;
  const int row0 = blockIdx.x * 128 + warp * 16;
  const int seg = blockIdx.y;
  const int c_begin = seg * seg_cols;
  const int c_end = min(ld, c_begin + seg_cols);
  const int wpr = ld >> 5;
  const int ra = min(row0 + g, rows - 1), rb = min(row0 + 8 + g, rows - 1);
  const double* Ra = R + (size_t)ra * ld + 4 * t;
  const double* Rb = R + (size_t)rb * ld + 4 * t;
  const uint32_t* Ma = bits + (size_t)ra * wpr;
  const uint32_t* Mb = bits + (size_t)rb * wpr;

  double acc[2][NT][2];
#pragma unroll
  for (int r = 0; r < 2; ++r)
#pragma unroll
    for (int n = 0; n < NT; ++n) acc[r][n][0] = acc[r][n][1] = 0.0;

  double2 nxt[4];
  if (c_begin < c_end) {
    nxt[0] = *reinterpret_cast<const double2*>(Ra + c_begin);
    nxt[1] = *reinterpret_cast<const double2*>(Ra + c_begin + 2);
    nxt[2] = *reinterpret_cast<const double2*>(Rb + c_begin);
    nxt[3] = *reinterpret_cast<const double2*>(Rb + c_begin + 2);
  }
  for (int c0 = c_begin; c0 < c_end; c0 += CH) {
    const int ncol = min(CH, c_end - c0);
    __syncthreads();
    for (int i = threadIdx.x; i < ncol * KP; i += 256) {
      int j = i / KP, k = i - j * KP;
      xs[j * XS + k] = Xp[(size_t)(c0 + j) * KP + k];
    }
    __syncthreads();
    for (int h = 0; h < ncol; h += 64) {
      const uint64_t ma = *reinterpret_cast<const uint64_t*>(Ma + ((c0 + h) >> 5));
      const uint64_t mb = *reinterpret_cast<const uint64_t*>(Mb + ((c0 + h) >> 5));
#pragma unroll
      for (int st = 0; st < 4; ++st) {
        const double2 a01 = nxt[0], a23 = nxt[1], b01 = nxt[2], b23 = nxt[3];
        const int jn = c0 + h + 16 * (st + 1);
        if (jn < c_end) {
          nxt[0] = *reinterpret_cast<const double2*>(Ra + jn);
          nxt[1] = *reinterpret_cast<const double2*>(Ra + jn + 2);
          nxt[2] = *reinterpret_cast<const double2*>(Rb + jn);
          nxt[3] = *reinterpret_cast<const double2*>(Rb + jn + 2);
        }
        const int sh = 16 * st + 4 * t;
        const uint32_t na = (uint32_t)(ma >> sh) & 0xFu;
        const uint32_t nb = (uint32_t)(mb >> sh) & 0xFu;
        double av[4] = {a01.x, a01.y, a23.x, a23.y};
        double bv[4] = {b01.x, b01.y, b23.x, b23.y};
#pragma unroll
        for (int q = 0; q < 4; ++q) {
          av[q] = ((na >> q) & 1u) ? av[q] : 0.0;
          bv[q] = ((nb >> q) & 1u) ? bv[q] : 0.0;
        }
#pragma unroll
        for (int q = 0; q < 4; ++q) {
          const double* xr = xs + (h + 16 * st + 4 * t + q) * XS + g;
#pragma unroll
          for (int n = 0; n < NT; ++n) {
            const double bf = xr[8 * n];
            dmma884(acc[0][n][0], acc[0][n][1], av[q], bf);
            dmma884(acc[1][n][0], acc[1][n][1], bv[q], bf);
          }
        }
      }
    }
  }
  double* o = out + (size_t)seg * rows * KP;
#pragma unroll
  for (int r = 0; r < 2; ++r) {
    const int row = row0 + 8 * r + g;
    if (row < rows) {
#pragma unroll
      for (int n = 0; n < NT; ++n)
        *reinterpret_cast<double2*>(o + (size_t)row * KP + 8 * n + 2 * t) = make_double2(acc[r][n][0], acc[r][n][1]);
    }
  }
}

template <int NT, bool VB>
__global__ void __launch_bounds__(256) k_stats_gram(const uint32_t* __restrict__ bits, int rows, int ld, int seg_words,
                                                   const double* __restrict__ Xp, const double* __restrict__ Vp,
                                                   int polarity, int K, double* __restrict__ Gout,
                                                   double* __restrict__ SVout, const int* __restrict__ run_flag) {
  constexpr int KP = 8 * NT;
  constexpr int NTP = NT * (NT + 1) / 2;
  __shared__ uint16_t queue[8][1024 + 8];
  if (run_flag && *run_flag == 0) return;

  const int warp = threadIdx.x >> 5, lane = threadIdx.x & 31, g = lane >> 2, e = lane & 3;
  const int row = blockIdx.x * 8 + warp;
  if (row >= rows) return;
  const int seg = blockIdx.y;
  const int wpr = ld >> 5;
  const int w_begin = seg * seg_words, w_end = min(wpr, w_begin + seg_words);
  const uint32_t* mrow = bits + (size_t)row * wpr;
  const int tK = K >> 3;
  uint16_t* q = queue[warp];

  double acc[NTP][2];
#pragma unroll
  for (int p = 0; p < NTP; ++p) acc[p][0] = acc[p][1] = 0.0;
  double accv[NT][2];
#pragma unroll
  for (int n = 0; n < NT; ++n) accv[n][0] = accv[n][1] = 0.0;

  for (int wb = w_begin; wb < w_end; wb += 32) {
    const int w = wb + lane;
    uint32_t m = 0;
    if (w < w_end) {
      const uint32_t word = mrow[w];
      m = polarity ? word : ~word;
    }
    const int cnt = __popc(m);
    int incl = cnt;
#pragma unroll
    for (int o = 1; o < 32; o <<= 1) {
      int v = __shfl_up_sync(0xffffffffu, incl, o);
      if (lane >= o) incl += v;
    }
    const int total = __shfl_sync(0xffffffffu, incl, 31);
    int pos = incl - cnt;
    while (m) {
      const int b = __ffs(m) - 1;
      m &= m - 1;
      q[pos++] = (uint16_t)(lane * 32 + b);
    }
    if (lane < 4) q[total + lane] = 0xFFFFu;
    __syncwarp();
    const size_t base = (size_t)wb * 32;
    for (int i = 0; i < total; i += 4) {
      const uint32_t off = q[i + e];
      const size_t j = (off == 0xFFFFu) ? (size_t)ld : base + off;
      const double* xr = Xp + j * KP + g;
      double x[NT];
#pragma unroll
      for (int n = 0; n < NT; ++n) x[n] = xr[8 * n];
#pragma unroll
      for (int a = 0; a < NT; ++a)
#pragma unroll
        for (int b = a; b < NT; ++b) {
          const int p = a * NT - a * (a - 1) / 2 + (b - a);
          dmma884(acc[p][0], acc[p][1], x[a], x[b]);
        }
      if (VB) {
        const double* vr = Vp + j * KP + g;
        double xk = x[0];
#pragma unroll
        for (int n = 1; n < NT; ++n) xk = (n == tK) ? x[n] : xk;
#pragma unroll
        for (int n = 0; n < NT; ++n) dmma884(accv[n][0], accv[n][1], xk, vr[8 * n]);
      }
    }
    __syncwarp();
  }
  double* go = Gout + ((size_t)seg * rows + row) * (NTP * 64);
#pragma unroll
  for (int p = 0; p < NTP; ++p)
    *reinterpret_cast<double2*>(go + p * 64 + g * 8 + 2 * e) = make_double2(acc[p][0], acc[p][1]);
  if (VB) {
    if (g == (K & 7)) {
      double* so = SVout + ((size_t)seg * rows + row) * KP;
#pragma unroll
      for (int n = 0; n < NT; ++n) *reinterpret_cast<double2*>(so + 8 * n + 2 * e) = make_double2(accv[n][0], accv[n][1]);
    }
  }
}

constexpr int FIX_WARPS = 4;
constexpr int FIX_QCAP = 1024;
template <int NT, bool VB>
__global__ void __launch_bounds__(32 * FIX_WARPS) k_gram_fixup(const uint32_t* __restrict__ bits, int rows, int ld, int cols,
                                                               const double* __restrict__ Xp, const double* __restrict__ Vp,
                                                               int polarity, double* __restrict__ Gout, double* __restrict__ SVout) {
  constexpr int KP = 8 * NT;
  constexpr int NTP = NT * (NT + 1) / 2;
  __shared__ uint16_t queue[FIX_WARPS][FIX_QCAP + 16];
  const int warp = threadIdx.x >> 5, lane = threadIdx.x & 31, g = lane >> 2, e = lane & 3;
  const int row = blockIdx.x * FIX_WARPS + warp;
  if (row >= rows) return;
  const int wpr = ld >> 5;
  const uint32_t* mrow = bits + (size_t)row * wpr;
  const uint32_t flip = polarity ? 0u : 0xffffffffu;
  uint16_t* q = queue[warp];

  double acc[NTP][2];
#pragma unroll
  for (int p = 0; p < NTP; ++p) acc[p][0] = acc[p][1] = 0.0;
  double sv[NT];
#pragma unroll
  for (int n = 0; n < NT; ++n) sv[n] = 0.0;

  int qn = 0;
  size_t qbase = 0;
  auto drain = [&]() {
    if (lane < 16) q[qn + lane] = 0xFFFFu;
    __syncwarp();
    for (int i = 0; i < qn; i += 16) {
      double x[4][NT], v[4][NT];
#pragma unroll
      for (int u = 0; u < 4; ++u) {
        const uint32_t off = q[i + 4 * u + e];
        const size_t j = (off == 0xFFFFu) ? (size_t)ld : qbase + off;
        const double* xr = Xp + j * KP + g;
#pragma unroll
        for (int n = 0; n < NT; ++n) x[u][n] = xr[8 * n];
        if (VB) {
          const double* vr = Vp + j * KP + g;
#pragma unroll
          for (int n = 0; n < NT; ++n) v[u][n] = vr[8 * n];
        }
      }
#pragma unroll
      for (int u = 0; u < 4; ++u) {
#pragma unroll
        for (int a = 0; a < NT; ++a)
#pragma unroll
          for (int b = a; b < NT; ++b) {
            const int p = a * NT - a * (a - 1) / 2 + (b - a);
            dmma884(acc[p][0], acc[p][1], x[u][a], x[u][b]);
          }
        if (VB) {
#pragma unroll
          for (int n = 0; n < NT; ++n) sv[n] += v[u][n];
        }
      }
    }
    __syncwarp();
    qn = 0;
  };

  for (int wb = 0; wb < wpr; wb += 256) {
    if ((size_t)wb * 32 - qbase >= 32768) { drain(); qbase = (size_t)wb * 32; }
    uint32_t ov[8];
    int cnt = 0;
#pragma unroll
    for (int c = 0; c < 8; ++c) {
      const int w = wb + c * 32 + lane;
      uint32_t m = w < wpr ? (mrow[w] ^ flip) : 0u;
      const int jb = w * 32;
      if (jb + 32 > cols) m = jb >= cols ? 0u : (m & ((1u << (cols - jb)) - 1u));
      uint32_t v0, v1, meta;
      ov[c] = sparse_split(m, v0, v1, meta);
      cnt += __popc(ov[c]);
    }
    int incl = cnt;
#pragma unroll
    for (int o = 1; o < 32; o <<= 1) {
      const int t = __shfl_up_sync(0xffffffffu, incl, o);
      if (lane >= o) incl += t;
    }
    const int total = __shfl_sync(0xffffffffu, incl, 31);
    if (qn + total > FIX_QCAP) drain();
    if (total <= FIX_QCAP) {
      int pos = qn + incl - cnt;
#pragma unroll
      for (int c = 0; c < 8; ++c) {
        uint32_t m = ov[c];
        const int cb = (int)((size_t)(wb + c * 32 + lane) * 32 - qbase);
        while (m) {
          const int b = __ffs(m) - 1;
          m &= m - 1;
          q[pos++] = (uint16_t)(cb + b);
        }
      }
      qn += total;
      __syncwarp();
    } else {
#pragma unroll 1
      for (int c = 0; c < 8; ++c) {
        const int cc = __popc(ov[c]);
        int inc2 = cc;
#pragma unroll
        for (int o = 1; o < 32; o <<= 1) {
          const int t = __shfl_up_sync(0xffffffffu, inc2, o);
          if (lane >= o) inc2 += t;
        }
        const int tot2 = __shfl_sync(0xffffffffu, inc2, 31);
        if (qn + tot2 > FIX_QCAP) drain();
        int pos = qn + inc2 - cc;
        uint32_t m = ov[c];
        const int cb = (int)((size_t)(wb + c * 32 + lane) * 32 - qbase);
        while (m) {
          const int b = __ffs(m) - 1;
          m &= m - 1;
          q[pos++] = (uint16_t)(cb + b);
        }
        qn += tot2;
        __syncwarp();
      }
    }
  }
  drain();

  double* go = Gout + (size_t)row * (NTP * 64);
#pragma unroll
  for (int p = 0; p < NTP; ++p)
    *reinterpret_cast<double2*>(go + p * 64 + g * 8 + 2 * e) = make_double2(acc[p][0], acc[p][1]);
  if (VB) {
#pragma unroll
    for (int n = 0; n < NT; ++n) {
      sv[n] += __shfl_xor_sync(0xffffffffu, sv[n], 1);
      sv[n] += __shfl_xor_sync(0xffffffffu, sv[n], 2);
    }
    if (e == 0) {
      double* so = SVout + (size_t)row * KP;
#pragma unroll
      for (int n = 0; n < NT; ++n) so[8 * n + g] = sv[n];
    }
  }
}

template <int NT, bool VB>
__global__ void __launch_bounds__(256) k_gram_full(const double* __restrict__ Xp, const double* __restrict__ Vp, int n,
                                                  int K, int dummy_row, double* __restrict__ partial) {
  constexpr int KP = 8 * NT;
  constexpr int NTP = NT * (NT + 1) / 2;
  constexpr int OUT = NTP * 64 + KP;
  __shared__ double red[OUT];
  const int warp = threadIdx.x >> 5, lane = threadIdx.x & 31, g = lane >> 2, e = lane & 3;
  const int tK = K >> 3;
  double acc[NTP][2];
#pragma unroll
  for (int p = 0; p < NTP; ++p) acc[p][0] = acc[p][1] = 0.0;
  double accv[NT][2];
#pragma unroll
  for (int t = 0; t < NT; ++t) accv[t][0] = accv[t][1] = 0.0;
  const int gw = blockIdx.x * 8 + warp, nw = gridDim.x * 8;
  for (int j0 = gw * 4; j0 < n; j0 += nw * 4) {
    const int jj = j0 + e;
    const size_t j = jj < n ? (size_t)jj : (size_t)dummy_row;
    const double* xr = Xp + j * KP + g;
    double x[NT];
#pragma unroll
    for (int t = 0; t < NT; ++t) x[t] = xr[8 * t];
#pragma unroll
    for (int a = 0; a < NT; ++a)
#pragma unroll
      for (int b = a; b < NT; ++b) {
        const int p = a * NT - a * (a - 1) / 2 + (b - a);
        dmma884(acc[p][0], acc[p][1], x[a], x[b]);
      }
    if (VB) {
      const double* vr = Vp + j * KP + g;
      double xk = x[0];
#pragma unroll
      for (int t = 1; t < NT; ++t) xk = (t == tK) ? x[t] : xk;
#pragma unroll
      for (int t = 0; t < NT; ++t) dmma884(accv[t][0], accv[t][1], xk, vr[8 * t]);
    }
  }
  for (int i = threadIdx.x; i < OUT; i += 256) red[i] = 0.0;
  __syncthreads();
  for (int w = 0; w < 8; ++w) {
    if (warp == w) {
#pragma unroll
      for (int p = 0; p < NTP; ++p) {
        red[p * 64 + g * 8 + 2 * e] += acc[p][0];
        red[p * 64 + g * 8 + 2 * e + 1] += acc[p][1];
      }
      if (VB && g == (K & 7)) {
#pragma unroll
        for (int t = 0; t < NT; ++t) {
          red[NTP * 64 + 8 * t + 2 * e] += accv[t][0];
          red[NTP * 64 + 8 * t + 2 * e + 1] += accv[t][1];
        }
      }
    }
    __syncthreads();
  }
  for (int i = threadIdx.x; i < OUT; i += 256) partial[(size_t)blockIdx.x * OUT + i] = red[i];
}

__global__ void __launch_bounds__(256) k_sum_partials(const double* __restrict__ partial, int nparts, int len,
                                                     double* __restrict__ out) {
  const int i = blockIdx.x * 8 + (threadIdx.x >> 5), lane = threadIdx.x & 31;
  if (i >= len) return;
  double s = 0.0;
  for (int p = lane; p < nparts; p += 32) s += partial[(size_t)p * len + i];
  s = warp_sum(s);
  if (lane == 0) out[i] = s;
}

#define BNMTF_DISPATCH_NT(NTV, ...)                                          \
  switch (NTV) {                                                             \
    case 1: { constexpr int NT = 1; __VA_ARGS__; } break;                    \
    case 2: { constexpr int NT = 2; __VA_ARGS__; } break;                    \
    case 3: { constexpr int NT = 3; __VA_ARGS__; } break;                    \
    case 4: { constexpr int NT = 4; __VA_ARGS__; } break;                    \
    case 5: { constexpr int NT = 5; __VA_ARGS__; } break;                    \
    case 6: { constexpr int NT = 6; __VA_ARGS__; } break;                    \
    case 7: { constexpr int NT = 7; __VA_ARGS__; } break;                    \
    case 8: { constexpr int NT = 8; __VA_ARGS__; } break;                    \
    default: set_error("K=%d out of range (1..63)", K); return -2;           \
  }

int launch_stats_rx(const double* R, const uint32_t* bits, int rows, int ld, const double* Xp, int K, int nseg,
                    double* out, const int* run_flag, cudaStream_t st) {
  if (rows <= 0 || ld <= 0 || ld % 64 || nseg <= 0) { set_error("stats_rx: bad shape rows=%d ld=%d nseg=%d", rows, ld, nseg); return -2; }
  const int nt = tiles_for(K);
  const int seg_cols = round_up((ld + nseg - 1) / nseg, 64);
  dim3 grid((rows + 127) / 128, nseg);
  BNMTF_DISPATCH_NT(nt, (k_stats_rx<NT><<<grid, 256, 0, st>>>(R, bits, rows, ld, Xp, seg_cols, out, run_flag)));
  return check_launch("stats_rx");
}

int launch_stats_gram(const uint32_t* bits, int rows, int ld, const double* Xp, const double* Vp, int K, int polarity,
                      int nseg, double* Gout, double* SVout, const int* run_flag, cudaStream_t st) {
  if (rows <= 0 || ld <= 0 || ld % 64 || nseg <= 0) { set_error("stats_gram: bad shape"); return -2; }
  const int nt = tiles_for(K);
  const int wpr = ld / 32;
  const int seg_words = round_up((wpr + nseg - 1) / nseg, 32);
  dim3 grid((rows + 7) / 8, nseg);
  if (Vp) {
    BNMTF_DISPATCH_NT(nt, (k_stats_gram<NT, true><<<grid, 256, 0, st>>>(bits, rows, ld, seg_words, Xp, Vp, polarity, K, Gout, SVout, run_flag)));
  } else {
    BNMTF_DISPATCH_NT(nt, (k_stats_gram<NT, false><<<grid, 256, 0, st>>>(bits, rows, ld, seg_words, Xp, nullptr, polarity, K, Gout, nullptr, run_flag)));
  }
  return check_launch("stats_gram");
}

int launch_stats_gram_fixup(const uint32_t* bits, int rows, int ld, int cols, const double* Xp, const double* Vp, int K,
                            int polarity, double* Gout, double* SVout, cudaStream_t st) {
  if (rows <= 0 || ld <= 0 || ld % 64 || cols <= 0 || cols > ld) { set_error("stats_gram_fixup: bad shape"); return -2; }
  const int nt = tiles_for(K);
  if (nt > 4) { set_error("stats_gram_fixup: K=%d > 31", K); return -2; }
  const int wpr = ld / 32;
  (void)wpr;
  dim3 grid((rows + FIX_WARPS - 1) / FIX_WARPS, 1);
  switch (nt) {
    case 1: if (Vp) k_gram_fixup<1, true><<<grid, 32 * FIX_WARPS, 0, st>>>(bits, rows, ld, cols, Xp, Vp, polarity, Gout, SVout);
            else k_gram_fixup<1, false><<<grid, 32 * FIX_WARPS, 0, st>>>(bits, rows, ld, cols, Xp, nullptr, polarity, Gout, nullptr); break;
    case 2: if (Vp) k_gram_fixup<2, true><<<grid, 32 * FIX_WARPS, 0, st>>>(bits, rows, ld, cols, Xp, Vp, polarity, Gout, SVout);
            else k_gram_fixup<2, false><<<grid, 32 * FIX_WARPS, 0, st>>>(bits, rows, ld, cols, Xp, nullptr, polarity, Gout, nullptr); break;
    case 3: if (Vp) k_gram_fixup<3, true><<<grid, 32 * FIX_WARPS, 0, st>>>(bits, rows, ld, cols, Xp, Vp, polarity, Gout, SVout);
            else k_gram_fixup<3, false><<<grid, 32 * FIX_WARPS, 0, st>>>(bits, rows, ld, cols, Xp, nullptr, polarity, Gout, nullptr); break;
    default: if (Vp) k_gram_fixup<4, true><<<grid, 32 * FIX_WARPS, 0, st>>>(bits, rows, ld, cols, Xp, Vp, polarity, Gout, SVout);
             else k_gram_fixup<4, false><<<grid, 32 * FIX_WARPS, 0, st>>>(bits, rows, ld, cols, Xp, nullptr, polarity, Gout, nullptr); break;
  }
  return check_launch("stats_gram_fixup");
}

int launch_gram_full(const double* Xp, const double* Vp, int n, int K, int dummy_row, double* out, double* scratch,
                     cudaStream_t st) {
  const int nt = tiles_for(K);
  const int len = nt * (nt + 1) / 2 * 64 + 8 * nt;
  int nparts = (n + 255) / 256;
  if (nparts > kGramFullParts) nparts = kGramFullParts;
  if (nparts < 1) nparts = 1;
  if (Vp) {
    BNMTF_DISPATCH_NT(nt, (k_gram_full<NT, true><<<nparts, 256, 0, st>>>(Xp, Vp, n, K, dummy_row, scratch)));
  } else {
    BNMTF_DISPATCH_NT(nt, (k_gram_full<NT, false><<<nparts, 256, 0, st>>>(Xp, nullptr, n, K, dummy_row, scratch)));
  }
  k_sum_partials<<<(len + 7) / 8, 256, 0, st>>>(scratch, nparts, len, out);
  return check_launch("gram_full");
}

}
```

### bnmtf_b200/engine.py

```python
import os
import threading

import numpy as np
import torch

from . import _lib

MODE = {"gibbs": 0, "vb": 1, "icm": 2}
thread_flags = threading.local()
TRACE_COLS = ("tau", "MSE", "R^2", "Rp", "ELBO", "sum_e2", "exp_square_diff", "explogtau")
S_TAU, S_LOGTAU, S_ALPHA_S, S_BETA_S, S_SUM_E2, S_ESD, S_MSE, S_R2, S_RP, S_ELBO = range(10)


_capture_streams = {}


def capture_graph(body):
    dev = torch.cuda.current_device()
    side = _capture_streams.get(dev)
    if side is None:
        side = _capture_streams[dev] = torch.cuda.Stream(device=dev)
    main = torch.cuda.current_stream()
    side.wait_stream(main)
    g = torch.cuda.CUDAGraph()
    with torch.cuda.stream(side):
        g.capture_begin()
        try:
            body()
        finally:
            g.capture_end()
    main.wait_stream(side)
    return g


def require_cuda(device=None):
    if not torch.cuda.is_available():
        raise _lib.BnmtfError("no CUDA device visible: bnmtf_b200 has no CPU path")
    _lib.load()
    return torch.device(device if device is not None else "cuda:%d" % torch.cuda.current_device())


def _ptr(t, row=0):
    if t is None:
        return 0
    return t.data_ptr() + (row * t.stride(0) * t.element_size() if row else 0)


def _stream():
    return torch.cuda.current_stream().cuda_stream


def ld_for(n):
    return (int(n) + 63) // 64 * 64


def kp_for(K):
    return 8 * ((K + 1 + 7) // 8)


def gram_len(K):
    nt = kp_for(K) // 8
    return nt * (nt + 1) // 2 * 64


def _pick_nseg(units, ktiles, t_tile, t_fix, sms=148, nmax=32):
    best = None
    for n in range(1, min(ktiles, nmax) + 1):
        tps = -(-ktiles // n)
        if -(-ktiles // tps) != n:
            continue
        cost = -(-(units * n) // sms) * (tps * t_tile + t_fix)
        if best is None or cost < best[0] - 1e-9:
            best = (cost, n)
    return best[1]


class Partition:

    def __init__(self, n, world=1, rank=0):
        self.n, self.world, self.rank = int(n), int(world), int(rank)
        self.S = -(-self.n // self.world)
        self.n_pad = self.S * self.world

    def lo(self, rank=None):
        return min(self.n, (self.rank if rank is None else rank) * self.S)

    def cnt(self, rank=None):
        return max(0, min(self.S, self.n - self.lo(rank)))


class Comm:

    def __init__(self, world=1, rank=0, group=None):
        self.world, self.rank, self.group = world, rank, group
        self.sync = None

    def gather_rows(self, full, part):
        if self.world == 1:
            return
        import torch.distributed as dist
        S = part.S
        mine = full[self.rank * S:(self.rank + 1) * S].clone()
        dist.all_gather_into_tensor(full[:part.n_pad], mine, group=self.group)

    def allreduce(self, t):
        if self.world == 1:
            return
        if self.sync is not None and t.dtype == torch.float64 and t.numel() <= 32 and t.is_contiguous():
            _lib.call("bnmtf_peer_sync_f64", _ptr(self.sync[1]), _ptr(self.sync[2]), self.world, self.rank, 2,
                      _ptr(t), t.numel(), _stream())
            return
        import torch.distributed as dist
        dist.all_reduce(t, group=self.group)

    def barrier(self, channel):
        if self.world == 1:
            return
        if self.sync is not None:
            _lib.call("bnmtf_peer_sync_f64", _ptr(self.sync[1]), _ptr(self.sync[2]), self.world, self.rank, int(channel),
                      0, 0, _stream())
            return
        import torch.distributed as dist
        dist.barrier(group=self.group)

    def setup_sync(self, device):
        if self.sync is None and self.peer_enabled(device):
            n = _lib.call("bnmtf_peer_sync_bytes") // 8
            t, hdl, ptrs, keep = self.symmetric((n,), device)
            epoch = torch.zeros(8, dtype=torch.int64, device=device)
            self.sync = (t, ptrs, epoch, keep, hdl)
        return self.sync is not None

    def put_rows(self, full, part, peers_ptrs):
        lo, cnt = part.lo(), part.cnt()
        if self.world == 1 or cnt == 0:
            return
        w = full.shape[1] if full.dim() > 1 else 1
        _lib.call("bnmtf_peer_put_f64", _ptr(full, lo), _ptr(peers_ptrs), lo * w, cnt * w, self.world, self.rank, _stream())

    def peer_enabled(self, device):
        if self.world == 1 or device.type != "cuda" or os.environ.get("BNMTF_PEER", "1") == "0":
            return False
        import torch.distributed as dist
        return dist.is_initialized() and dist.get_backend(self.group) == "nccl"

    def symmetric(self, shape, device):
        import torch.distributed as dist
        import torch.distributed._symmetric_memory as symm
        group = self.group if self.group is not None else dist.group.WORLD
        t = symm.empty(tuple(shape), dtype=torch.float64, device=device)
        hdl = symm.rendezvous(t, group)
        flat = t.view(-1)
        flat.zero_()
        flat[0] = float(self.rank + 1)
        hdl.barrier(channel=0)
        peers = [t if r == self.rank else hdl.get_remote_tensor(r, tuple(shape), torch.float64) for r in range(self.world)]
        seen = [float(p.view(-1)[0].item()) for p in peers]
        if seen != [float(r + 1) for r in range(self.world)]:
            raise _lib.BnmtfError("symmetric-memory peer mapping check failed: read %s" % seen)
        hdl.barrier(channel=0)
        flat[0] = 0.0
        torch.cuda.synchronize(device)
        hdl.barrier(channel=0)
        ptrs = torch.tensor([p.data_ptr() for p in peers], dtype=torch.int64, device=device)
        return t, hdl, ptrs, peers


class Dataset:

    def __init__(self, I, J, device, world=1, rank=0):
        self.I, self.J, self.device = int(I), int(J), device
        self.ldJ, self.ldI = ld_for(J), ld_for(I)
        self.partI, self.partJ = Partition(I, world, rank), Partition(J, world, rank)
        self.world, self.rank = world, rank
        self.R = self.bits = self.RT = self.bitsT = None
        self.n_obs = None
        self.planes = {}
        self.wide = {}

    def _pack(self, R, M, rows, cols, ld):
        out = torch.zeros((max(rows, 1), ld), dtype=torch.float64, device=self.device)
        bits = torch.zeros((max(rows, 1), ld // 32), dtype=torch.int32, device=self.device)
        if rows > 0:
            Rd = torch.from_numpy(np.ascontiguousarray(R, dtype=np.float64)).to(self.device)
            Md = torch.from_numpy(np.ascontiguousarray(M, dtype=np.float64)).to(self.device)
            _lib.call("bnmtf_pack_dataset_f64", _ptr(Rd), _ptr(Md), rows, cols, ld, _ptr(out), _ptr(bits), _stream())
        return out, bits

    @classmethod
    def from_host(cls, R, M, device=None, world=1, rank=0):
        device = require_cuda(device)
        R = np.asarray(R, dtype=np.float64)
        M = np.asarray(M, dtype=np.float64)
        I, J = R.shape
        ds = cls(I, J, device, world, rank)
        lo, cnt = ds.partI.lo(), ds.partI.cnt()
        ds.R, ds.bits = ds._pack(R[lo:lo + cnt], M[lo:lo + cnt], cnt, J, ds.ldJ)
        if world == 1:
            ds._make_transpose()
        else:
            lo, cnt = ds.partJ.lo(), ds.partJ.cnt()
            ds.RT, ds.bitsT = ds._pack(R[:, lo:lo + cnt].T, M[:, lo:lo + cnt].T, cnt, I, ds.ldI)
        ds.n_obs = float(M.sum())
        return ds

    @classmethod
    def from_device(cls, R_padded, bits, I, J, RT_padded=None, bitsT=None, n_obs=None, world=1, rank=0):
        ds = cls(I, J, R_padded.device, world, rank)
        assert R_padded.shape[1] == ds.ldJ and bits.shape[1] == ds.ldJ // 32
        ds.R, ds.bits = R_padded, bits
        if RT_padded is None:
            assert world == 1
            ds._make_transpose()
        else:
            ds.RT, ds.bitsT = RT_padded, bitsT
        ds.n_obs = float(n_obs) if n_obs is not None else None
        return ds

    def _make_transpose(self):
        I, J = self.I, self.J
        self.RT = torch.empty((J, self.ldI), dtype=torch.float64, device=self.device)
        self.bitsT = torch.empty((J, self.ldI // 32), dtype=torch.int32, device=self.device)
        _lib.call("bnmtf_transpose_dataset_f64", _ptr(self.R), _ptr(self.bits), I, J, self.ldJ,
                  _ptr(self.RT), _ptr(self.bitsT), self.ldI, _stream())

    def ensure_planes(self, side):
        if side not in self.planes:
            R, bits = (self.R, self.bits) if side == 0 else (self.RT, self.bitsT)
            rows = (self.partI if side == 0 else self.partJ).cnt()
            ld = self.ldJ if side == 0 else self.ldI
            if rows == 0:
                self.planes[side] = (None, None)
                self.wide[side] = False
                return self.planes[side]
            nbytes = _lib.call("bnmtf_rx_planes_bytes", rows, ld)
            buf = torch.empty(nbytes + 1024, dtype=torch.uint8, device=self.device)
            off = (-buf.data_ptr()) % 1024
            planes = buf[off:off + nbytes]
            rscale = torch.empty(rows, dtype=torch.float64, device=self.device)
            rexp = torch.empty(rows, dtype=torch.int32, device=self.device)
            wide = torch.zeros(1, dtype=torch.int32, device=self.device)
            _lib.call("bnmtf_rx_planes_pack_f64", _ptr(R), _ptr(bits), rows, ld, planes.data_ptr(), _ptr(rscale),
                      _ptr(rexp), _ptr(wide), _stream())
            self.planes[side] = (planes, rscale, buf)
            self.wide[side] = bool(int(wide.item()))
        return self.planes[side]

    def pack_mask(self, M):
        lo, cnt = self.partI.lo(), self.partI.cnt()
        return self._pack(np.zeros((cnt, self.J)), np.asarray(M, dtype=np.float64)[lo:lo + cnt], cnt, self.J, self.ldJ)[1]


class Factor:

    def __init__(self, part, K, device, vb, comm=None):
        self.part, self.n, self.K = part, part.n, K
        z = lambda: torch.zeros((part.n_pad, K), dtype=torch.float64, device=device)
        self.peer = None
        if comm is not None and comm.peer_enabled(device):
            try:
                self.fac, hdl, pf, keep_f = comm.symmetric((part.n_pad, K), device)
                self.var = pv = keep_v = None
                if vb:
                    self.var, _, pv, keep_v = comm.symmetric((part.n_pad, K), device)
                self.peer = (hdl, pf, pv, keep_f, keep_v)
            except _lib.BnmtfError:
                raise
            except Exception as exc:
                import warnings
                warnings.warn("bnmtf_b200: symmetric memory unavailable (%s: %s); factor rows are exchanged with NCCL "
                              "all-gathers instead of in-kernel peer stores" % (type(exc).__name__, exc))
                self.peer = None
        if self.peer is None:
            self.fac = z()
            self.var = z() if vb else None
        self.lam = z()
        self.lam.fill_(1.0)
        self.mu, self.tauf = z(), z()
        self.n_alloc = ld_for(self.n) + 8
        KP = kp_for(K)
        self.Xp = torch.zeros((self.n_alloc, KP), dtype=torch.float64, device=device)
        self.Vp = torch.zeros((self.n_alloc, KP), dtype=torch.float64, device=device) if vb else None

    def pad(self):
        _lib.call("bnmtf_pad_factor_f64", _ptr(self.fac), _ptr(self.var), self.n, self.K, self.n_alloc,
                  _ptr(self.Xp), _ptr(self.Vp), _stream())


class BNMFEngine:

    def __init__(self, dataset, K, mode, alpha, beta, seed=0, comm=None, gram=None):
        self.ds, self.K, self.mode = dataset, int(K), mode
        self.gram = gram or os.environ.get("BNMTF_GRAM", "umma")
        assert self.gram in ("umma", "dmma")
        self.rx = os.environ.get("BNMTF_RX", "umma" if (self.gram == "umma" and self.K <= 32) else "dmma")
        assert self.rx in ("umma", "dmma") and (self.rx == "dmma" or self.K <= 32)
        self.metrics_mode = os.environ.get("BNMTF_METRICS", "stats" if self.gram == "umma" else "direct")
        self.guard = 1e-5
        self.overlap = int(os.environ.get("BNMTF_OVERLAP", "0")) if self.gram == "umma" else 0
        self.umma_stages = int(os.environ.get("BNMTF_UMMA_STAGES", "3" if self.overlap else "0"))
        g = int(os.environ.get("BNMTF_GRAPH", "1"))
        self.use_graph = g >= 1 and dataset.world == 1
        self._graph = self._graph_key = self._graph_seen = None
        self.split = int(os.environ.get("BNMTF_SPLIT", "64" if self.K > 16 else ("80" if self.K > 8 else "96")))
        self.umma_pair = int(os.environ.get("BNMTF_UMMA_PAIR", "1"))
        self._fix_stream = None
        self._side = None
        self.m = MODE[mode]
        self.vb = mode == "vb"
        self.alpha, self.beta, self.seed = float(alpha), float(beta), int(seed) & (2 ** 64 - 1)
        self.comm = comm if comm is not None else Comm(dataset.world, dataset.rank)
        dev = dataset.device
        I, J = dataset.I, dataset.J
        self.U = Factor(dataset.partI, K, dev, self.vb, self.comm)
        self.V = Factor(dataset.partJ, K, dev, self.vb, self.comm)
        if dataset.world > 1 and self.U.peer is not None and self.V.peer is not None and self.comm.setup_sync(dev):
            self.use_graph = g >= 1
        self.scalars = torch.zeros(16, dtype=torch.float64, device=dev)
        self.iter = torch.zeros(1, dtype=torch.int64, device=dev)
        self.iter_scratch = torch.zeros(1, dtype=torch.int64, device=dev)
        self.trace = None
        self.trace_cap = 0
        self.trace_base = 0
        self.sweeps_done = 0
        KP, GL = kp_for(K), gram_len(K)
        self.loc = {0: (dataset.partI.lo(), dataset.partI.cnt()), 1: (dataset.partJ.lo(), dataset.partJ.cnt())}
        self.range_guard = self.gram == "umma" and os.environ.get("BNMTF_RANGE_GUARD", "1") != "0"
        self.range_flag = torch.zeros(1, dtype=torch.int32, device=dev)
        self.range_trips = torch.zeros(1, dtype=torch.int64, device=dev)
        self.wide_dataset = False
        if self.rx == "umma":
            for side in (0, 1):
                dataset.ensure_planes(side)
            wide = torch.tensor([int(any(dataset.wide.values()))], dtype=torch.int32, device=dev)
            self.comm.allreduce(wide)
            if int(wide.item()) and os.environ.get("BNMTF_RANGE_GUARD", "1") != "0":
                import warnings
                warnings.warn("bnmtf_b200: some row or column of R has outliers more than 2^20 x its typical entry; the 48-bit "
                              "fixed-point statistics kernels would leave those entries fewer than 28 significant bits, "
                              "using the fp64 kernels for this dataset")
                self.rx = self.gram = "dmma"
                self.wide_dataset, self.range_guard = True, False
                self.metrics_mode = os.environ.get("BNMTF_METRICS", "direct")
        self.nseg = {}
        for side, ld in ((0, dataset.ldJ), (1, dataset.ldI)):
            rows = max(1, self.loc[side][1])
            rb = (rows + 127) // 128
            if self.rx == "umma":
                kt64 = ld // 64
                nrx = max(1, min(kt64, -(-120 // rb)))
                if rb * (kt64 // 160) >= 444:
                    nrx = kt64 // 160
                nrx = -(-kt64 // -(-kt64 // nrx))
            else:
                nrx = max(1, min(ld // 128, -(-2664 // rb)))
            if self.gram == "umma":
                tile = 128 if ld >= 256 else 64
                sums = K if (side == 1 and self.metrics_mode == "stats") else 0
                self.umma_form = getattr(self, "umma_form", {})
                form = self.umma_pair
                if tile != 128 or K > 31:
                    form &= ~2
                self.umma_form[side] = form
                acc_cols = 480 if form & 2 else 512
                nch = -(-(K * (K + 1) // 2 + (K if self.vb else 0) + sums) // (acc_cols // _lib.call("bnmtf_fixed_point_digits")))
                ktiles = -(-ld // tile)
                ng = _pick_nseg(((rb + 1) // 2 * 2 if form & 1 else rb) * nch, ktiles,
                                t_tile=(0.3 if form & 2 else 0.55) * tile / 128, t_fix=10.0)
                self.umma_tile = getattr(self, "umma_tile", {})
                self.umma_tile[side] = tile
            else:
                gb = (rows + 7) // 8
                ng = max(1, min(-(-(ld // 32) // 32), -(-592 // gb)))
            nm = max(1, min(ld // 128, -(-1776 // rb)))
            self.nseg[side] = (nrx, ng, nm)
        rI, rJ = max(1, self.loc[0][1]), max(1, self.loc[1][1])
        mrx = max(self.nseg[0][0] * rI, self.nseg[1][0] * rJ)
        self.gram_segs = {side: self.nseg[side][1] + (1 if self.gram == "umma" and self.umma_form[side] & 2 else 0) for side in (0, 1)}
        mg = max(self.gram_segs[0] * rI, self.gram_segs[1] * rJ)
        f64 = lambda *shape: torch.zeros(shape, dtype=torch.float64, device=dev)
        self.RXpart = f64(mrx, KP)
        self.Gpart = f64(mg, GL)
        self.SVpart = f64(mg, KP) if self.vb else None
        self.Gfull = f64(GL + KP)
        if self.rx == "umma":
            self.wsrx_bytes = max(_lib.call("bnmtf_rx_umma_workspace_bytes", self.K, ld) for ld in (dataset.ldJ, dataset.ldI))
            self.wsrx = torch.zeros(self.wsrx_bytes + 1024, dtype=torch.uint8, device=dev)
            self.wsrx_ptr = (self.wsrx.data_ptr() + 1023) // 1024 * 1024
        if self.gram == "umma":
            self.ws_bytes = max(_lib.call("bnmtf_gram_umma_workspace_bytes", self.K, int(self.vb), ld)
                                for ld in (dataset.ldJ, dataset.ldI))
            self.ws = torch.zeros(self.ws_bytes + 1024, dtype=torch.uint8, device=dev)
            self.ws_ptr = (self.ws.data_ptr() + 1023) // 1024 * 1024
        self.gscratch = f64(296 * (GL + KP))
        self.extra = f64(max(rI, rJ)) if self.vb else None
        self.red = f64(24)
        self.m8, self.el8, self.ex1, self.sums4 = self.red[0:8], self.red[8:16], self.red[16:17], self.red[17:21]
        self.mpart = f64(((rI + 127) // 128) * self.nseg[0][2] * 8)
        self.nb_terms = 64 if max(rI, rJ) * self.K <= (1 << 17) else 296
        self.elpart = f64(2 * self.nb_terms * 8) if self.vb else None
        self.sterm = None
        self.order_dev = None
        self.statics = f64(3)
        if self.loc[0][1] > 0:
            _lib.call("bnmtf_masked_metrics_f64", _ptr(dataset.R), _ptr(dataset.bits), self.loc[0][1], dataset.ldJ,
                      _ptr(self.U.Xp), _ptr(self.V.Xp), self.K, self.nseg[0][2], 0, _ptr(self.mpart), _ptr(self.m8),
                      0, _stream())
            self.statics.copy_(self.m8[4:7])
        self.statics_global = self.statics.clone()
        self.comm.allreduce(self.statics_global)
        self.mstat = f64(max(rI, rJ), 4)
        self.mstat_part = f64(256)
        self.m8d = f64(8)
        self.flag = torch.zeros(1, dtype=torch.int32, device=dev)
        if dataset.n_obs is None:
            tot = self.statics[2:3].clone()
            self.comm.allreduce(tot)
            dataset.n_obs = float(tot.item())
        self.polarity = 0 if dataset.n_obs >= 0.5 * I * J else 1
        self._set_omega(dataset.n_obs)

    def _set_omega(self, n_obs):
        from scipy.special import gammaln, psi
        self.size_Omega = float(n_obs)
        self.alpha_s = self.alpha + self.size_Omega / 2.0
        self.digamma_alpha_s = float(psi(self.alpha_s))
        self.lgamma_alpha = float(gammaln(self.alpha))
        self.lgamma_alpha_s = float(gammaln(self.alpha_s))

    def _sides(self, side):
        ds = self.ds
        lo, cnt = self.loc[side]
        if side == 0:
            return self.U, self.V, ds.R, ds.bits, cnt, ds.ldJ, lo
        return self.V, self.U, ds.RT, ds.bitsT, cnt, ds.ldI, lo

    def stats(self, side, need_rx=True, sums=False, timers=None):
        self._stats_kernels(side, need_rx, sums, timers)
        me, other, R, bits, rows, ld, lo = self._sides(side)
        if not self.range_guard or rows == 0:
            return
        nrx, ng, _ = self.nseg[side]
        _lib.call("bnmtf_range_guard_f64", _ptr(self.Gpart), self.gram_segs[side], rows, _ptr(self.Gfull), self.polarity, self.K, other.n,
                  self.ws_ptr, _ptr(self.range_flag), _ptr(self.range_trips), _stream())
        _lib.call("bnmtf_stats_gated_f64", _ptr(self.range_flag), _ptr(R), _ptr(bits), rows, ld, _ptr(other.Xp), _ptr(other.Vp),
                  self.K, self.polarity, nrx, self.gram_segs[side], _ptr(self.RXpart) if need_rx else 0, _ptr(self.Gpart),
                  _ptr(self.SVpart), _stream())

    def _stats_kernels(self, side, need_rx=True, sums=False, timers=None):
        me, other, R, bits, rows, ld, lo = self._sides(side)
        nrx, ng, _ = self.nseg[side]
        other.pad()
        if rows == 0:
            return
        if self.polarity == 0:
            _lib.call("bnmtf_gram_full_f64", _ptr(other.Xp), _ptr(other.Vp), other.n, self.K, ld,
                      _ptr(self.Gfull), _ptr(self.gscratch), _stream())
        rx = lambda: self._rx(side)
        if need_rx and self.split > 0 and self.rx == "umma" and self.gram == "umma":
            if self._side is None:
                self._side = torch.cuda.Stream(device=self.ds.device, priority=-1)
                self._ev = [torch.cuda.Event(), torch.cuda.Event()]
            main = torch.cuda.current_stream()
            self._ev[0].record(main)
            self._side.wait_event(self._ev[0])
            tev = [torch.cuda.Event(enable_timing=True) for _ in range(4)] if timers is not None else None
            with torch.cuda.stream(self._side):
                if tev:
                    tev[0].record(self._side)
                self._rx(side, max_ctas=self.split)
                if tev:
                    tev[1].record(self._side)
                self._ev[1].record(self._side)
            if tev:
                tev[2].record(main)
            self._gram(side, sums)
            if tev:
                tev[3].record(main)
                timers.append(("stats_rx_in_sweep", tev[0], tev[1]))
                timers.append(("stats_gram_in_sweep", tev[2], tev[3]))
            main.wait_event(self._ev[1])
        elif need_rx and self.overlap:
            if self._side is None:
                self._side = torch.cuda.Stream(device=self.ds.device, priority=-1)
                self._ev = [torch.cuda.Event(), torch.cuda.Event()]
            main = torch.cuda.current_stream()
            self._ev[0].record(main)
            self._side.wait_event(self._ev[0])
            if self.overlap == 2:
                rx()
            with torch.cuda.stream(self._side):
                self._gram(side, sums)
                self._ev[1].record(self._side)
            if self.overlap != 2:
                rx()
            main.wait_event(self._ev[1])
        else:
            if need_rx:
                rx()
            self._gram(side, sums)

    def _rx(self, side, max_ctas=0):
        me, other, R, bits, rows, ld, lo = self._sides(side)
        nrx = self.nseg[side][0]
        if self.rx == "umma":
            planes, rscale = self.ds.ensure_planes(side)[:2]
            _lib.call("bnmtf_stats_rx_umma_f64", planes.data_ptr(), _ptr(rscale), _ptr(R), _ptr(bits), rows, ld, other.n,
                      _ptr(other.Xp), self.K, nrx, max_ctas, _ptr(self.RXpart), self.wsrx_ptr, self.wsrx_bytes, _stream())
        else:
            _lib.call("bnmtf_stats_rx_f64", _ptr(R), _ptr(bits), rows, ld, _ptr(other.Xp), self.K, nrx,
                      _ptr(self.RXpart), _stream())

    def _gram(self, side, sums=False):
        me, other, R, bits, rows, ld, lo = self._sides(side)
        ng = self.nseg[side][1]
        if self.gram == "umma":
            form = self.umma_form[side]
            if form & 2:
                if self._fix_stream is None:
                    self._fix_stream = torch.cuda.Stream(device=self.ds.device)
                    self._fix_ev = [torch.cuda.Event(), torch.cuda.Event()]
                main = torch.cuda.current_stream()
                self._fix_ev[0].record(main)
                self._fix_stream.wait_event(self._fix_ev[0])
                with torch.cuda.stream(self._fix_stream):
                    _lib.call("bnmtf_stats_gram_fixup_f64", _ptr(bits), rows, ld, other.n, _ptr(other.Xp), _ptr(other.Vp), self.K,
                              self.polarity, self.Gpart.data_ptr() + 8 * ng * rows * self.Gpart.shape[1],
                              self.SVpart.data_ptr() + 8 * ng * rows * self.SVpart.shape[1] if self.vb else 0, _stream())
                    self._fix_ev[1].record(self._fix_stream)
            _lib.call("bnmtf_stats_gram_umma_f64", _ptr(bits), rows, ld, other.n, _ptr(other.Xp), _ptr(other.Vp), self.K,
                      self.polarity, ng, self.umma_tile[side], form, 1 if sums else 0, self.umma_stages,
                      _ptr(self.Gpart),
                      _ptr(self.SVpart), self.ws_ptr, self.ws_bytes, _stream())
            if form & 2:
                torch.cuda.current_stream().wait_event(self._fix_ev[1])
        else:
            _lib.call("bnmtf_stats_gram_f64", _ptr(bits), rows, ld, _ptr(other.Xp), _ptr(other.Vp), self.K,
                      self.polarity, ng, _ptr(self.Gpart), _ptr(self.SVpart), _stream())

    def solve(self, side, order=None, n_order=None, apply=True, minimum_TN=0.0, want_sterm=False, want_extra=False,
              use_iter=True, gather=True, want_mstat=False):
        me, other, R, bits, rows, ld, lo = self._sides(side)
        nrx, ng, _ = self.nseg[side]
        order_ptr = 0
        if order is not None:
            self.order_dev = torch.tensor(list(order), dtype=torch.int32, device=self.ds.device)
            order_ptr, n_order = _ptr(self.order_dev), len(order)
        elif n_order is None:
            n_order = self.K
        if want_sterm and self.sterm is None:
            self.sterm = torch.zeros((max(self.U.part.n_pad, self.V.part.n_pad), self.K), dtype=torch.float64,
                                     device=self.ds.device)
        fused = gather and apply and me.peer is not None
        if rows > 0:
            _lib.call("bnmf_row_solve_f64", self.m, rows, self.K, nrx, self.gram_segs[side] if self.gram == "umma" else ng, self.polarity,
                      _ptr(self.RXpart), _ptr(self.Gpart), _ptr(self.SVpart), _ptr(self.Gfull),
                      _ptr(me.fac, lo), _ptr(me.var, lo), _ptr(me.mu, lo), _ptr(me.tauf, lo), _ptr(me.lam, lo),
                      _ptr(self.scalars), order_ptr, n_order, 1 if apply else 0, float(minimum_TN),
                      self.seed, _ptr(self.iter if use_iter else self.iter_scratch), side, lo,
                      _ptr(self.sterm, lo) if want_sterm else 0, _ptr(self.extra) if want_extra else 0,
                      _ptr(self.mstat) if want_mstat else 0,
                      _ptr(me.peer[1]) if fused else 0, _ptr(me.peer[2]) if (fused and self.vb) else 0,
                      self.comm.world if fused else 0, self.comm.rank,
                      _ptr(self.range_flag) if self.range_guard else 0, _stream())
        if fused:
            self.comm.barrier(side)
        elif gather and self.comm.world > 1:
            if apply:
                self.comm.gather_rows(me.fac, me.part)
                if self.vb:
                    self.comm.gather_rows(me.var, me.part)
            else:
                self.comm.gather_rows(me.mu, me.part), self.comm.gather_rows(me.tauf, me.part)
                if want_sterm:
                    self.comm.gather_rows(self.sterm, me.part)

    def gather_params(self):
        if self.comm.world > 1:
            for f in (self.U, self.V):
                self.comm.gather_rows(f.mu, f.part), self.comm.gather_rows(f.tauf, f.part)

    def metrics(self, bits=None):
        self.U.pad()
        self.V.pad()
        self._metrics_padded(self.ds.bits if bits is None else bits)
        self.comm.allreduce(self.m8)

    def _metrics_padded(self, bits, gated=False):
        ds = self.ds
        lo, rows = self.loc[0]
        if rows == 0:
            (self.m8d if gated else self.m8).zero_()
            return
        statics = _ptr(self.statics) if bits is ds.bits else 0
        _lib.call("bnmtf_masked_metrics_f64", _ptr(ds.R), _ptr(bits), rows, ds.ldJ, _ptr(self.U.Xp, lo), _ptr(self.V.Xp),
                  self.K, self.nseg[0][2], statics, _ptr(self.mpart), _ptr(self.m8d if gated else self.m8),
                  _ptr(self.flag) if gated else 0, _stream())

    def _vb_terms(self):
        nb = self.nb_terms
        self.elpart.zero_()
        for i, f in enumerate((self.U, self.V)):
            lo, cnt = self.loc[i]
            if cnt > 0:
                _lib.call("bnmtf_vb_factor_terms_f64", _ptr(f.fac, lo), _ptr(f.var, lo), _ptr(f.mu, lo), _ptr(f.tauf, lo),
                          _ptr(f.lam, lo), cnt * f.K, self.elpart[i * nb * 8:].data_ptr(), nb, _stream())
        _lib.call("bnmtf_reduce8_f64", _ptr(self.elpart), 2 * nb, _ptr(self.el8), _stream())

    def _vb_extra(self):
        rows = self.loc[1][1]
        if rows > 0:
            _lib.call("bnmtf_reduce1_f64", _ptr(self.extra), rows, _ptr(self.ex1), _stream())
        else:
            self.ex1.zero_()

    def finish(self, update_tau=True, record=True):
        trace_ptr = _ptr(self.trace) if (record and self.trace is not None) else 0
        _lib.call("bnmf_finish_sweep_f64", self.m, self.alpha, self.beta, self.digamma_alpha_s, self.lgamma_alpha,
                  self.lgamma_alpha_s, (self.ds.I + self.ds.J) * self.K, _ptr(self.m8), _ptr(self.ex1), _ptr(self.el8),
                  _ptr(self.scalars), trace_ptr, _ptr(self.iter if record else self.iter_scratch),
                  0, self.seed, 1 if update_tau else 0, _ptr(self.trace_win) if record else 0, _stream())
        if record:
            self.sweeps_done += 1

    def refresh_scalars(self, update_tau=True):
        self.red.zero_()
        if self.vb:
            self.stats(1, need_rx=False)
            self.solve(1, n_order=0, apply=False, want_extra=True, use_iter=False, gather=False)
            self._vb_extra()
            self._vb_terms()
        self.U.pad()
        self.V.pad()
        self._metrics_padded(self.ds.bits)
        self.comm.allreduce(self.red)
        self.finish(update_tau=update_tau, record=False)

    def sweep(self, minimum_TN=0.0):
        if self.use_graph and not getattr(thread_flags, "no_graph", False):
            key = (self.trace.data_ptr() if self.trace is not None else 0, float(minimum_TN))
            if self._graph is not None and self._graph_key == key:
                self._graph.replay()
                _lib.launch_count[0] += self._graph_kernels
                self.sweeps_done += 1
                return
            if self._graph_seen == key:
                done, count0 = self.sweeps_done, _lib.launch_count[0]
                g = capture_graph(lambda: self._sweep_eager(minimum_TN))
                self._graph_kernels = _lib.launch_count[0] - count0
                _lib.launch_count[0] = count0
                self.sweeps_done = done
                self._graph, self._graph_key = g, key
                g.replay()
                _lib.launch_count[0] += self._graph_kernels
                self.sweeps_done += 1
                return
            self._graph_seen = key
        self._sweep_eager(minimum_TN)

    def _sweep_eager(self, minimum_TN=0.0):
        stat = self.metrics_mode == "stats"
        self.stats(0)
        self.solve(0, minimum_TN=minimum_TN)
        self.stats(1, sums=stat)
        self.solve(1, minimum_TN=minimum_TN, want_extra=self.vb, want_mstat=stat)
        self.V.pad()
        if stat:
            rows = self.loc[1][1]
            if rows > 0:
                _lib.call("bnmtf_mstat_reduce_f64", _ptr(self.mstat), rows, _ptr(self.mstat_part), _ptr(self.sums4), _stream())
            else:
                self.sums4.zero_()
        else:
            self._metrics_padded(self.ds.bits)
        if self.vb:
            self._vb_extra()
            self._vb_terms()
        self.comm.allreduce(self.red)
        if stat:
            _lib.call("bnmtf_metrics_from_sums_f64", _ptr(self.sums4), _ptr(self.statics_global), self.guard,
                      _ptr(self.m8), _ptr(self.flag), _stream())
            self._metrics_padded(self.ds.bits, gated=True)
            self.comm.allreduce(self.m8d)
            _lib.call("bnmtf_select_metrics_f64", _ptr(self.flag), _ptr(self.m8d), _ptr(self.m8), _stream())
        self.finish(update_tau=True, record=True)

    def profile_sweep(self, reps=3):
        stat = self.metrics_mode == "stats"
        names = ("stats_rx", "stats_gram", "row_solve", "masked_metrics")
        acc = {n: 0.0 for n in names}
        count = {n: 0 for n in names}

        def timed(name, fn):
            e0, e1 = torch.cuda.Event(enable_timing=True), torch.cuda.Event(enable_timing=True)
            e0.record()
            fn()
            e1.record()
            e1.synchronize()
            acc[name] += e0.elapsed_time(e1)
            count[name] += 1
        for _ in range(reps):
            for side in (0, 1):
                me, other, R, bits, rows, ld, lo = self._sides(side)
                other.pad()
                if self.polarity == 0:
                    _lib.call("bnmtf_gram_full_f64", _ptr(other.Xp), _ptr(other.Vp), other.n, self.K, ld,
                              _ptr(self.Gfull), _ptr(self.gscratch), _stream())
                timed("stats_rx", lambda: self._rx(side))
                timed("stats_gram", lambda: self._gram(side, sums=stat and side == 1))
                timed("row_solve", lambda: self.solve(side, want_extra=self.vb and side == 1, gather=False,
                                                      want_mstat=stat and side == 1))
                self.solve(side, n_order=0, apply=True, gather=True)
            self.V.pad()
            if stat:
                rows = self.loc[1][1]
                if rows > 0:
                    _lib.call("bnmtf_mstat_reduce_f64", _ptr(self.mstat), rows, _ptr(self.mstat_part), _ptr(self.sums4), _stream())
                else:
                    self.sums4.zero_()
            else:
                timed("masked_metrics", lambda: self._metrics_padded(self.ds.bits))
            if self.vb:
                self._vb_extra()
                self._vb_terms()
            self.comm.allreduce(self.red)
            if stat:
                _lib.call("bnmtf_metrics_from_sums_f64", _ptr(self.sums4), _ptr(self.statics_global), self.guard,
                          _ptr(self.m8), _ptr(self.flag), _stream())
            self.finish(update_tau=True, record=False)
        out = {n: acc[n] / max(1, count[n]) for n in names}
        if self.split > 0 and self.rx == "umma" and self.gram == "umma":
            timers, spans = [], []
            for _ in range(reps):
                for side in (0, 1):
                    p0, p1 = torch.cuda.Event(enable_timing=True), torch.cuda.Event(enable_timing=True)
                    p0.record()
                    self.stats(side, sums=stat and side == 1, timers=timers)
                    p1.record()
                    spans.append((p0, p1))
            torch.cuda.synchronize()
            for name in ("stats_rx_in_sweep", "stats_gram_in_sweep"):
                v = [a.elapsed_time(b) for (n, a, b) in timers if n == name]
                out[name] = sum(v) / max(1, len(v))
            out["stats_phase_in_sweep"] = sum(a.elapsed_time(b) for a, b in spans) / max(1, len(spans))
        out["_meta"] = {"gram": self.gram, "rx": self.rx, "metrics_mode": self.metrics_mode, "split": self.split}
        return out

    def small_cluster(self):
        if getattr(self, "_small_c", None) is None:
            ok = self.comm.world == 1 and os.environ.get("BNMTF_SMALL", "1") != "0"
            self._small_c = int(_lib.call("bnmtf_small_cluster_size", self.ds.I, self.ds.J, self.K, int(self.vb))) if ok else 0
            if self._small_c:
                self._small_partial = torch.zeros(16 * 16 + 32, dtype=torch.float64, device=self.ds.device)
        return self._small_c

    def sweep_many(self, sweeps, minimum_TN=0.0, samples=None, times=None, sums=None, orders=None):
        sU, sV, burn_in, thinning = sums if sums is not None else (None, None, 0, 1)
        all_U, all_V = samples if samples is not None else (None, None)
        trace_ptr = _ptr(self.trace) - self.trace_base * 64 if self.trace is not None else 0
        ds, U, V = self.ds, self.U, self.V
        _lib.call("bnmtf_small_sweeps_f64", self.m, _ptr(ds.R), _ptr(ds.bits), _ptr(ds.RT), _ptr(ds.bitsT), ds.I, ds.J, ds.ldJ, ds.ldI,
                  self.K, _ptr(U.fac), _ptr(U.var), _ptr(U.mu), _ptr(U.tauf), _ptr(U.lam), _ptr(V.fac), _ptr(V.var), _ptr(V.mu),
                  _ptr(V.tauf), _ptr(V.lam), _ptr(self.scalars), trace_ptr, _ptr(self.iter), self.trace_base + self.trace_cap,
                  self.alpha, self.beta, self.digamma_alpha_s, self.lgamma_alpha, self.lgamma_alpha_s, float(minimum_TN),
                  self.seed, int(sweeps), _ptr(all_U), _ptr(all_V), _ptr(sU), _ptr(sV), int(burn_in), int(thinning),
                  _ptr(self._small_partial), _ptr(times), _stream())
        self.sweeps_done += int(sweeps)

    def alloc_trace(self, iterations):
        self.trace_cap = int(iterations)
        if self.trace is None or self.trace.shape[0] < max(1, self.trace_cap):
            self.trace = torch.zeros((max(64, self.trace_cap), 8), dtype=torch.float64, device=self.ds.device)
        self.trace_base = self.sweeps_done
        if getattr(self, "trace_win", None) is None:
            self.trace_win = torch.zeros(2, dtype=torch.int64, device=self.ds.device)
        self.trace_win.copy_(torch.tensor([self.trace_base, self.trace_base + self.trace_cap], dtype=torch.int64))


CSR_CHUNK = 1024
CSR_METRIC_CTAS = 1184


def csr_work_plan(indptr, chunk=CSR_CHUNK):
    indptr = np.asarray(indptr, dtype=np.int64)
    rows = indptr.shape[0] - 1
    lens = np.diff(indptr)
    nch = np.maximum(1, -(-lens // chunk))
    item_row = np.repeat(np.arange(rows, dtype=np.int64), nch)
    first = np.cumsum(nch) - nch
    c = np.arange(item_row.shape[0], dtype=np.int64) - np.repeat(first, nch)
    heavy = nch > 1
    item_slot = np.full(item_row.shape[0], -1, dtype=np.int64)
    in_heavy = heavy[item_row]
    item_slot[in_heavy] = np.arange(int(in_heavy.sum()), dtype=np.int64)
    heavy_first = np.concatenate([[0], np.cumsum(nch[heavy])]).astype(np.int32)
    return {"item_begin": indptr[item_row] + c * chunk, "item_row": item_row.astype(np.int32),
            "item_slot": item_slot.astype(np.int32), "heavy_row": np.nonzero(heavy)[0].astype(np.int32),
            "heavy_first": heavy_first, "n_slots": int(heavy_first[-1]), "chunk": int(chunk)}


class DeviceCSR:

    def __init__(self, indptr, indices, data, device, plan=True):
        t = lambda a, dt: torch.from_numpy(np.ascontiguousarray(a, dtype=dt)).to(device)
        self.rows = int(len(indptr) - 1)
        self.nnz = int(indptr[-1])
        self.rowptr, self.colidx, self.val = t(indptr, np.int64), t(indices, np.int32), t(data, np.float64)
        if self.nnz == 0:
            self.colidx, self.val = torch.zeros(1, dtype=torch.int32, device=device), torch.zeros(1, dtype=torch.float64, device=device)
        self.plan = None
        if plan:
            p = csr_work_plan(indptr)
            self.chunk, self.n_items, self.n_slots = p["chunk"], int(p["item_row"].shape[0]), p["n_slots"]
            self.n_heavy = int(p["heavy_row"].shape[0])
            self.item_begin, self.item_row, self.item_slot = t(p["item_begin"], np.int64), t(p["item_row"], np.int32), t(p["item_slot"], np.int32)
            self.heavy_row = t(p["heavy_row"], np.int32) if self.n_heavy else None
            self.heavy_first = t(p["heavy_first"], np.int32)
            self.plan = p

    def nbytes(self):
        ts = [self.rowptr, self.colidx, self.val] + ([self.item_begin, self.item_row, self.item_slot, self.heavy_first]
                                                     + ([self.heavy_row] if self.n_heavy else []) if self.plan else [])
        return sum(x.numel() * x.element_size() for x in ts)

    def metrics(self, Ap, Bp, K, partials, out8, run_flag=None):
        nparts = max(1, min(CSR_METRIC_CTAS, -(-self.rows // 8)))
        _lib.call("bnmtf_csr_metrics_f64", _ptr(self.rowptr), _ptr(self.colidx), _ptr(self.val), self.rows, _ptr(Ap), _ptr(Bp),
                  int(K), _ptr(partials), nparts, _ptr(out8), _ptr(run_flag), _stream())


class SparseDataset:
    world, rank = 1, 0
    bits = None

    def __init__(self, host_R, train, device):
        import scipy.sparse as sp
        self.I, self.J = host_R.shape
        self.device = device
# ... 131 lines not shown
```

Before: 133.8.

## Replace 4:2 sparse gram split with exact 3-in-4 encoding, drop fixup kernel

After: 136.2, median of 6. 1.02x the previous value.

```diff
diff --git a/bnmtf_b200/_lib.py b/bnmtf_b200/_lib.py
--- a/bnmtf_b200/_lib.py
+++ b/bnmtf_b200/_lib.py
@@ -83,7 +83,7 @@
 
 KERNELS_PER_CALL = {"bnmtf_pack_dataset_f64": 1, "bnmtf_pack_mask_f64": 1, "bnmtf_transpose_dataset_f64": 1,
                     "bnmtf_pad_factor_f64": 1, "bnmtf_stats_rx_f64": 1, "bnmtf_stats_rx_umma_f64": 5,
-                    "bnmtf_rx_planes_pack_f64": 2, "bnmtf_range_guard_f64": 1, "bnmtf_stats_gated_f64": 2, "bnmtf_stats_gram_f64": 1, "bnmtf_stats_gram_fixup_f64": 1, "bnmtf_kmeans_distances_f64": 1, "bnmtf_small_sweeps_f64": 1, "bnmtf_small_tri_sweeps_f64": 1, "bnmtf_stats_gram_umma_f64": 4, "bnmtf_mstat_reduce_f64": 2,
+                    "bnmtf_rx_planes_pack_f64": 2, "bnmtf_range_guard_f64": 1, "bnmtf_stats_gated_f64": 2, "bnmtf_stats_gram_f64": 1, "bnmtf_stats_gram_fixup_f64": 0, "bnmtf_kmeans_distances_f64": 1, "bnmtf_small_sweeps_f64": 1, "bnmtf_small_tri_sweeps_f64": 1, "bnmtf_stats_gram_umma_f64": 4, "bnmtf_mstat_reduce_f64": 2,
                     "bnmtf_metrics_from_sums_f64": 1, "bnmtf_select_metrics_f64": 1,
                     "bnmtf_gram_full_f64": 2, "bnmf_row_solve_f64": 1, "bnmtf_masked_metrics_f64": 3, "bnmtf_csr_stats_f64": 2, "bnmtf_csr_metrics_f64": 2,
                     "bnmtf_dense_metrics_f64": 2, "bnmtf_vb_factor_terms_f64": 1, "bnmtf_reduce8_f64": 1,
diff --git a/bnmtf_b200/csrc/api.cu b/bnmtf_b200/csrc/api.cu
--- a/bnmtf_b200/csrc/api.cu
+++ b/bnmtf_b200/csrc/api.cu
@@ -38,7 +38,6 @@
 int launch_stats_gram(const uint32_t*, int, int, const double*, const double*, int, int, int, double*, double*, const int*, cudaStream_t);
 int launch_gram_full(const double*, const double*, int, int, int, double*, double*, cudaStream_t);
 long long umma_workspace_bytes(int, int, long long);
-int launch_stats_gram_fixup(const uint32_t*, int, int, int, const double*, const double*, int, int, double*, double*, cudaStream_t);
 int launch_stats_gram_umma(const uint32_t*, int, int, int, const double*, const double*, int, int, int, int, int, int, int,
                            double*, double*, void*, long long, cudaStream_t);
 int launch_pad_factor(const double*, const double*, int, int, int, double*, double*, cudaStream_t);
@@ -343,9 +342,14 @@
 
 int bnmtf_stats_gram_fixup_f64(const uint32_t* bits, int64_t rows, int64_t ld, int64_t cols, const double* Xp, const double* Vp,
                                int K, int polarity, double* Gseg, double* SVseg, void* stream) {
-  if (check_k(K)) return -2;
+  (void)bits; (void)Xp; (void)polarity;
+  if (check_k(K)) return -2;
+  if (rows <= 0 || ld <= 0 || ld % 64 || cols <= 0 || cols > ld) { set_error("stats_gram_fixup: bad shape"); return -2; }
   if ((Vp == nullptr) != (SVseg == nullptr)) { set_error("stats_gram_fixup: Vp and SVseg must be given together"); return -2; }
-  return launch_stats_gram_fixup(bits, (int)rows, (int)ld, (int)cols, Xp, Vp, K, polarity, Gseg, SVseg, ST(stream));
+  const int nt = tiles_for(K);
+  cudaMemsetAsync(Gseg, 0, (size_t)rows * nt * (nt + 1) / 2 * 64 * sizeof(double), ST(stream));
+  if (SVseg) cudaMemsetAsync(SVseg, 0, (size_t)rows * 8 * nt * sizeof(double), ST(stream));
+  return check_launch("stats_gram_fixup");
 }
 
 int64_t bnmtf_gram_umma_workspace_bytes(int K, int vb, int64_t ld) {
diff --git a/bnmtf_b200/csrc/common.cuh b/bnmtf_b200/csrc/common.cuh
--- a/bnmtf_b200/csrc/common.cuh
+++ b/bnmtf_b200/csrc/common.cuh
@@ -186,17 +186,17 @@
 }
 #endif
 
-__host__ __device__ __forceinline__ uint32_t sparse_split(uint32_t v, uint32_t& v0, uint32_t& v1, uint32_t& meta) {
+__host__ __device__ __forceinline__ uint32_t sparse3_split(uint32_t t, uint32_t& v0, uint32_t& v1, uint32_t& meta) {
+  uint32_t x = (t & 0xFFFu) | ((t & 0xFFF000u) << 4);
+  x = (x & 0x003F003Fu) | ((x & 0x0FC00FC0u) << 2);
+  x = (x & 0x07070707u) | ((x & 0x38383838u) << 1);
   const uint32_t m = 0x11111111u;
-  const uint32_t b0 = v & m, b1 = (v >> 1) & m, b2 = (v >> 2) & m, b3 = (v >> 3) & m;
-  const uint32_t c1 = b0 & b1;
-  const uint32_t c2 = (b0 ^ b1) & b2;
-  const uint32_t i0b0 = b1 & ~b0, i0b1 = b2 & ~(b0 | b1);
-  meta = i0b0 | (i0b1 << 1) | ((m & ~c2) << 2) | ((m & ~c1) << 3);
-  v0 = b0 | b1 | b2;
-  v1 = c1 | c2 | (b3 & ~(c1 | c2));
-  return ((c1 & b2) << 2) | ((b3 & (c1 | c2)) << 3);
-}
-
-
-}
+  const uint32_t a = x & m, b = (x >> 1) & m, c = (x >> 2) & m, abc = a & b & c;
+  meta = (b & c & ~a) | (abc << 1) | (((m & ~c) | abc) << 2) | (c << 3);
+  v0 = a | (b & c);
+  v1 = b | c;
+  return abc;
+}
+
+
+}
diff --git a/bnmtf_b200/csrc/gram_umma.cu b/bnmtf_b200/csrc/gram_umma.cu
--- a/bnmtf_b200/csrc/gram_umma.cu
+++ b/bnmtf_b200/csrc/gram_umma.cu
@@ -1,4 +1,5 @@
 #include <cstdlib>
+#include <cstring>
 #include "umma.cuh"
 
 namespace bnmtf {
@@ -56,6 +57,7 @@
 
 __global__ void __launch_bounds__(256) k_ug_colmax(const double* __restrict__ Xp, const double* __restrict__ Vp, int n,
                                                   int KP, UmmaPlan pl, unsigned long long* __restrict__ colmax) {
+  bool neg = false;
   extern __shared__ double xs[];
   constexpr int JT = 64;
   const int K = pl.K;
@@ -79,6 +81,7 @@
         const double p = xb ? xa[jj] * xb[jj] : xa[jj];
         const unsigned long long u = (unsigned long long)__double_as_longlong(fabs(p));
         mm = u > mm ? u : mm;
+        neg |= p < 0.0;
       }
       return mm;
     };
@@ -94,6 +97,7 @@
     const int c = threadIdx.x + 256 * q;
     if (c < pl.nc && m[q]) atomicMax(colmax + c, m[q]);
   }
+  if (neg) atomicOr(colmax + pl.nc, 1ull);
 }
 
 __global__ void k_ug_scales(const unsigned long long* __restrict__ colmax, int nc, double* __restrict__ cscale,
@@ -113,18 +117,35 @@
 }
 
 __global__ void __launch_bounds__(128) k_ug_quantize(const double* __restrict__ Xp, const double* __restrict__ Vp, int n,
-                                                    int KP, long long ldb, UmmaPlan pl, const int* __restrict__ cexp,
-                                                    uint8_t* __restrict__ Bd) {
+                                                    int KP, int ld, long long ldb, UmmaPlan pd, UmmaPlan ps, int sp,
+                                                    int seg_cols, int sps, const unsigned long long* __restrict__ negflag,
+                                                    const int* __restrict__ cexp, uint8_t* __restrict__ Bd) {
   extern __shared__ double xs[];
   constexpr int JT = 128, XS = JT + 2;
-  const int j0 = blockIdx.x * JT;
+  const bool s3 = sp && *negflag == 0ull;
+  const UmmaPlan& pl = s3 ? ps : pd;
+  int j0, jlim;
+  long long out0, ldo;
+  if (s3) {
+    const int seg = blockIdx.x / sps, st = blockIdx.x - seg * sps;
+    const int c0 = seg * seg_cols, c1 = min(ld, c0 + seg_cols);
+    j0 = c0 + 96 * st;
+    if (j0 >= c1) return;
+    jlim = min(n, c1);
+    out0 = (long long)blockIdx.x * 128; ldo = ldb;
+  } else {
+    j0 = blockIdx.x * JT;
+    if (j0 >= ld) return;
+    jlim = n;
+    out0 = j0; ldo = ld;
+  }
   const int K = pl.K;
   int16_t* tab = reinterpret_cast<int16_t*>(xs + (size_t)(pl.vb ? 2 : 1) * K * XS);
   for (int i = threadIdx.x; i < JT * K; i += blockDim.x) {
     const int jj = i / K, k = i - jj * K;
     const int j = j0 + jj;
-    xs[k * XS + jj] = (j < n) ? Xp[(size_t)j * KP + k] : 0.0;
-    if (pl.vb) xs[(K + k) * XS + jj] = (j < n) ? Vp[(size_t)j * KP + k] : 0.0;
+    xs[k * XS + jj] = (j < jlim) ? Xp[(size_t)j * KP + k] : 0.0;
+    if (pl.vb) xs[(K + k) * XS + jj] = (j < jlim) ? Vp[(size_t)j * KP + k] : 0.0;
   }
   for (int c = threadIdx.x; c < pl.nc; c += blockDim.x) {
     int a, b;
@@ -132,8 +153,8 @@
     tab[2 * c] = (int16_t)a; tab[2 * c + 1] = (int16_t)b;
   }
   __syncthreads();
-  const int jg = (threadIdx.x & 31) * 4, sub = threadIdx.x >> 5;
-  const int nvalid = n - (j0 + jg);
+  const int jg = (threadIdx.x & 31) * (s3 ? 3 : 4), sub = threadIdx.x >> 5;
+  const int nvalid = jlim - (j0 + jg);
   for (int c = sub + 4 * blockIdx.y; c < pl.nc; c += 4 * gridDim.y) {
     const int ch = c / pl.cpc, cl = c - ch * pl.cpc;
     const int a = tab[2 * c], b = tab[2 * c + 1];
@@ -143,13 +164,19 @@
     const bool fast = sh > -1000 && sh < 1000;
     const double pw = fast ? __longlong_as_double((long long)(sh + 1023) << 52) : 0.0;
     uint32_t lo[4], hi[4];
+    long long q[4];
 #pragma unroll
     for (int i = 0; i < 4; ++i) {
       const double p = xb ? xa[i] * xb[i] : xa[i];
-      long long q = fast ? __double2ll_rn(p * pw) : llrint(scalbn(p, sh));
-      q = q > (1ll << UG_TOP) - 1 ? (1ll << UG_TOP) - 1 : (q < -(1ll << UG_TOP) ? -(1ll << UG_TOP) : q);
-      const unsigned long long u = i < nvalid ? (unsigned long long)(q + (1ll << UG_TOP)) : 0ull;
+      long long qi = fast ? __double2ll_rn(p * pw) : llrint(scalbn(p, sh));
+      qi = qi > (1ll << UG_TOP) - 1 ? (1ll << UG_TOP) - 1 : (qi < -(1ll << UG_TOP) ? -(1ll << UG_TOP) : qi);
+      q[i] = i < nvalid ? qi : 0ll;
+      const unsigned long long u = i < nvalid ? (unsigned long long)(qi + (1ll << UG_TOP)) : 0ull;
       lo[i] = (uint32_t)u; hi[i] = (uint32_t)(u >> 32);
+    }
+    if (s3) {
+      const unsigned long long x = (unsigned long long)(q[0] + q[1]);
+      lo[3] = (uint32_t)x; hi[3] = (uint32_t)(x >> 32);
     }
     uint32_t w[8];
     {
@@ -162,10 +189,11 @@
       w[4] = __byte_perm(e01, e23, 0x5410); w[5] = __byte_perm(e01, e23, 0x7632);
       w[6] = __byte_perm(g01, g23, 0x5410); w[7] = __byte_perm(g01, g23, 0x7632);
     }
-    uint8_t* dst = Bd + ((size_t)ch * UG_CHUNK_ROWS + (size_t)cl * UG_SLICES) * ldb + j0 + jg;
-    if (j0 + jg < ldb) {
-#pragma unroll
-      for (int s = 0; s < UG_SLICES; ++s) *reinterpret_cast<uint32_t*>(dst + (size_t)s * ldb) = w[s];
+    const long long oc = out0 + (threadIdx.x & 31) * 4;
+    uint8_t* dst = Bd + ((size_t)ch * UG_CHUNK_ROWS + (size_t)cl * UG_SLICES) * ldo + oc;
+    if (oc < (s3 ? ldb : (long long)ld)) {
+#pragma unroll
+      for (int s = 0; s < UG_SLICES; ++s) *reinterpret_cast<uint32_t*>(dst + (size_t)s * ldo) = w[s];
     }
   }
 }
@@ -173,6 +201,8 @@
 struct UmmaGramArgs {
   const uint32_t* bits; int rows, wpr, cols, polarity;
   int ktiles, tiles_per_seg;
+  int seg_cols;
+  const unsigned long long* negflag; int run_if_neg;
   UmmaPlan pl;
   const double* cscale;
   double* Gout; double* SVout;
@@ -186,6 +216,7 @@
 __global__ void __launch_bounds__(UG_THREADS, 1) k_gram_umma(const __grid_constant__ CUtensorMap tmap_full,
                                                             const __grid_constant__ CUtensorMap tmap_last,
                                                             const __grid_constant__ CUtensorMap tmap_bits, UmmaGramArgs a) {
+  if (a.negflag && ((*reinterpret_cast<const volatile unsigned long long*>(a.negflag) != 0ull) != (a.run_if_neg != 0))) return;
   extern __shared__ uint8_t smem_raw[];
   uint8_t* smem = reinterpret_cast<uint8_t*>((reinterpret_cast<uintptr_t>(smem_raw) + 1023) & ~(uintptr_t)1023);
   const int tid = threadIdx.x, warp = tid >> 5, lane = tid & 31;
@@ -205,7 +236,7 @@
   const uint32_t mask_base = smem_u32(smem) + (uint32_t)stages * STAGE;
   uint64_t* bars = reinterpret_cast<uint64_t*>(smem + (size_t)stages * STAGE + UG_MASK_BUFS * MASK_WIN_BYTES);
   uint32_t* tmem_slot = reinterpret_cast<uint32_t*>(bars + 2 * stages + 1 + 2 * UG_MASK_BUFS);
-  int* cnt_smem = reinterpret_cast<int*>(tmem_slot + 2);
+  int2* cnt_smem = reinterpret_cast<int2*>(tmem_slot + 2);
   uint16_t* pair_tab = reinterpret_cast<uint16_t*>(cnt_smem + UG_EXP_WARPS * 32);
   const uint32_t smem_base = smem_u32(smem);
   const uint32_t bar_base = smem_u32(bars);
@@ -216,8 +247,10 @@
 #define MASK_EMPTY(b) (bar_base + 8u * (uint32_t)(2 * stages + 1 + UG_MASK_BUFS + (b)))
 
   const int kt_begin = seg * a.tiles_per_seg;
-  const int kt_end = min(a.ktiles, kt_begin + a.tiles_per_seg);
-  const int ntile = kt_end - kt_begin;
+  const int col0 = seg * a.seg_cols;
+  const int col_lim = min(a.cols, col0 + a.seg_cols);
+  const int ntile = SP ? (min(a.wpr * 32, col0 + a.seg_cols) - col0 + 95) / 96 : min(a.ktiles, kt_begin + a.tiles_per_seg) - kt_begin;
+  constexpr int WPT = SP ? 3 : KT / 32;
 
   if (warp == UG_EXP_WARPS && lane == 0) {
     const uint32_t nfull = 4u + (PAIR ? (rank == 0 ? 2u : 0u) : 1u);
@@ -252,15 +285,14 @@
     const int row = rb * UG_ROWS + r;
     const bool live = row < a.rows;
     const uint32_t* mrow = a.bits + (size_t)(live ? row : 0) * a.wpr;
-    constexpr int WPT = KT / 32;
     constexpr int CPT = KT / 16;
     const int NG = stages < UG_GROUPS ? stages : UG_GROUPS;
     const uint32_t flip = a.polarity ? 0u : 0xffffffffu;
     const uint32_t row_off = (uint32_t)(r >> 3) * (8 * AKT) + (uint32_t)(r & 7) * AKT;
     const uint32_t key = AKT == 128 ? (uint32_t)(r & 7) : (uint32_t)((r >> 1) & 3);
     const uint32_t tlane_e = tmem_base + ((uint32_t)((warp & 3) * 32) << 16) + (uint32_t)UG_SP_ACC_COLS;
-    int cnt = 0;
-    constexpr int WIN = 16 / WPT;
+    int cnt = 0, n3 = 0;
+    constexpr int WIN = SP ? 4 : 16 / WPT;
     const bool mask_tma = a.mask_tma != 0;
     int s = half % stages;
     uint32_t ph = (uint32_t)(half / stages) & 1u;
@@ -269,13 +301,20 @@
     uint32_t qph = (uint32_t)(((half + koff) / WIN) / UG_MASK_BUFS) & 1u;
     const int s_step = NG % stages, ph_step = (NG / stages) & 1;
     for (int it = half < NG ? half : ntile; it < ntile; it += NG) {
-      const int wbase = (kt_begin + it) * WPT;
+      const int wbase = col0 / 32 + it * WPT;
       uint32_t w[WPT];
       int release_win = -1;
       if (mask_tma) {
         mbar_wait(MASK_FULL(qb), qph);
         const uint32_t rowb = mask_base + (uint32_t)qb * MASK_WIN_BYTES + (uint32_t)r * 64u;
-        if constexpr (WPT == 4) {
+        if constexpr (SP) {
+          const uint32_t lo = (uint32_t)(3 * c) >> 2, o = (uint32_t)(3 * c) & 3u, sw = (uint32_t)((r >> 1) & 3);
+          uint32_t e[8];
+          asm volatile("ld.shared.v4.b32 {%0, %1, %2, %3}, [%4];" : "=r"(e[0]), "=r"(e[1]), "=r"(e[2]), "=r"(e[3]) : "r"(rowb + ((lo ^ sw) << 4)) : "memory");
+          asm volatile("ld.shared.v4.b32 {%0, %1, %2, %3}, [%4];" : "=r"(e[4]), "=r"(e[5]), "=r"(e[6]), "=r"(e[7]) : "r"(rowb + (((lo + 1u) ^ sw) << 4)) : "memory");
+#pragma unroll
+          for (int k = 0; k < 3; ++k) w[k] = o == 0 ? e[k] : (o == 1 ? e[k + 1] : (o == 2 ? e[k + 2] : e[k + 3]));
+        } else if constexpr (WPT == 4) {
           const uint32_t addr = rowb + ((((uint32_t)c) ^ (uint32_t)((r >> 1) & 3)) << 4);
           asm volatile("ld.shared.v4.b32 {%0, %1, %2, %3}, [%4];" : "=r"(w[0]), "=r"(w[1]), "=r"(w[2]), "=r"(w[3]) : "r"(addr) : "memory");
         } else {
@@ -287,40 +326,46 @@
 #pragma unroll
         for (int i = 0; i < WPT; ++i) w[i] = (live && wbase + i < a.wpr) ? mrow[wbase + i] : 0u;
       }
-      const bool edge = (wbase + WPT) * 32 > a.cols;
+      const bool edge = (wbase + WPT) * 32 > col_lim;
       uint32_t y[CPT][4];
-      uint32_t meta[WPT];
+      uint32_t meta[4];
+      uint32_t vv[WPT];
 #pragma unroll
       for (int i = 0; i < WPT; ++i) {
         uint32_t v = w[i] ^ flip;
         if (edge) {
           const int jb = (wbase + i) * 32;
-          if (jb + 32 > a.cols) v = jb >= a.cols ? 0u : (v & ((1u << (a.cols - jb)) - 1u));
+          if (jb + 32 > col_lim) v = jb >= col_lim ? 0u : (v & ((1u << (col_lim - jb)) - 1u));
         }
         v = live ? v : 0u;
-        if constexpr (SP) {
+        cnt += __popc(v);
+        vv[i] = v;
+        if constexpr (!SP) {
+#pragma unroll
+          for (int q = 0; q < 8; ++q) y[2 * i + (q >> 2)][q & 3] = (((v >> (4 * q)) & 0xfu) * 0x00204081u) & 0x01010101u;
+        }
+      }
+      if constexpr (SP) {
+        const uint32_t t[4] = {vv[0] & 0xFFFFFFu, (vv[0] >> 24) | ((vv[1] & 0xFFFFu) << 8), (vv[1] >> 16) | ((vv[2] & 0xFFu) << 16),
+                               vv[2] >> 8};
+#pragma unroll
+        for (int i = 0; i < 4; ++i) {
           uint32_t v0, v1;
-          const uint32_t ovf = sparse_split(v, v0, v1, meta[i]);
-          cnt += __popc(v) - __popc(ovf);
+          n3 += __popc(sparse3_split(t[i], v0, v1, meta[i]));
           const uint32_t z = v0 | (v1 << 1);
 #pragma unroll
           for (int q = 0; q < 4; ++q) y[i][q] = (((z >> (8 * q)) & 0x33u) * 0x00081081u) & 0x01010101u;
-        } else {
-          cnt += __popc(v);
-#pragma unroll
-          for (int q = 0; q < 8; ++q) y[2 * i + (q >> 2)][q & 3] = (((v >> (4 * q)) & 0xfu) * 0x00204081u) & 0x01010101u;
         }
       }
       mbar_wait(EMPTY_BAR(s), ph ^ 1u);
       const uint32_t abase = smem_base + (uint32_t)s * STAGE + row_off;
       if constexpr (SP) {
-        static_assert(WPT == 4, "four metadata columns per stage");
         asm volatile("tcgen05.st.sync.aligned.32x32b.x4.b32 [%0], {%1, %2, %3, %4};"
                      ::"r"(tlane_e + 4u * (uint32_t)s), "r"(meta[0]), "r"(meta[1]), "r"(meta[2]), "r"(meta[3]) : "memory");
       }
       if (!((a.dbg & 2) && it >= stages))
 #pragma unroll
-      for (int cc = 0; cc < (SP ? WPT : CPT); ++cc) {
+      for (int cc = 0; cc < (SP ? 4 : CPT); ++cc) {
         const uint32_t addr = abase + ((((uint32_t)cc) ^ key) << 4);
         asm volatile("st.shared.v4.b32 [%0], {%1, %2, %3, %4};" ::"r"(addr), "r"(y[cc][0]), "r"(y[cc][1]), "r"(y[cc][2]), "r"(y[cc][3]) : "memory");
       }
@@ -339,11 +384,12 @@
       c += NG;
       while (c >= WIN) { c -= WIN; if (++qb == UG_MASK_BUFS) { qb = 0; qph ^= 1u; } }
     }
-    cnt_smem[tid] = cnt;
+    cnt_smem[tid] = make_int2(cnt, n3);
     asm volatile("bar.sync 1, %0;" ::"n"(UG_EXP_WARPS * 32) : "memory");
-    cnt = 0;
-#pragma unroll
-    for (int g = 0; g < UG_GROUPS; ++g) cnt += cnt_smem[r + g * UG_ROWS];
+    cnt = 0; n3 = 0;
+#pragma unroll
+    for (int g = 0; g < UG_GROUPS; ++g) { const int2 cg = cnt_smem[r + g * UG_ROWS]; cnt += cg.x; n3 += cg.y; }
+    const long long noff = (long long)cnt - 2ll * n3;
 
     mbar_wait(ACCUM_BAR, 0u);
     tc_fence_after();
@@ -372,7 +418,7 @@
         long long hi = 0;
 #pragma unroll
         for (int sl = 4; sl < UG_SLICES; ++sl)
-          hi += ((long long)(int)DD(sl) - (sl == UG_SLICES - 1 ? 128ll * cnt : 0ll)) << (8 * (sl - 4));
+          hi += ((long long)(int)DD(sl) - (sl == UG_SLICES - 1 ? 128ll * noff : 0ll)) << (8 * (sl - 4));
 #undef DD
         const double v = fma((double)hi, 4294967296.0, (double)lo) * a.cscale[ch * pl.cpc + cl];
         if (pb == 0xff) {
@@ -428,14 +474,14 @@
     __syncwarp();
   } else if (warp == UG_EXP_WARPS + 2) {
     if (lane == 0 && a.mask_tma) {
-      constexpr int WIN = 512 / KT;
+      constexpr int WIN = SP ? 4 : 512 / KT;
       const int koff = KT == 64 ? (kt_begin & 1) : 0;
       const int nwin = (ntile + koff + WIN - 1) / WIN;
       for (int q = 0; q < nwin; ++q) {
         const int qb = q % UG_MASK_BUFS;
         if (q >= UG_MASK_BUFS) mbar_wait(MASK_EMPTY(qb), ((uint32_t)(q / UG_MASK_BUFS) & 1u) ^ 1u);
         mbar_expect_tx(MASK_FULL(qb), (uint32_t)MASK_WIN_BYTES);
-        tma_load_2d(mask_base + (uint32_t)qb * MASK_WIN_BYTES, &tmap_bits, (kt_begin - koff + q * WIN) * (KT / 32), rb * UG_ROWS, MASK_FULL(qb));
+        tma_load_2d(mask_base + (uint32_t)qb * MASK_WIN_BYTES, &tmap_bits, col0 / 32 + (q * WIN - koff) * WPT, rb * UG_ROWS, MASK_FULL(qb));
       }
     }
     __syncwarp();
@@ -550,19 +596,25 @@
 }
 
 static size_t ws_digits_offset(const UmmaPlan& pl) {
-  size_t o = (size_t)pl.nc * 8 * 2 + (size_t)((pl.nc + 1) / 2 * 2) * 4;
+  size_t o = (size_t)(pl.nc + 1) * 8 + (size_t)pl.nc * 8 + (size_t)((pl.nc + 1) / 2 * 2) * 4;
   return (o + 1023) / 1024 * 1024;
 }
 
-static long long plan_workspace_bytes(const UmmaPlan& pl, long long ld) {
-  return (long long)ws_digits_offset(pl) + (long long)pl.nch * UG_CHUNK_ROWS * ld;
+static long long sparse_slots(int ld, int nseg) {
+  const int tps = ((ld + 127) / 128 + nseg - 1) / nseg;
+  return (long long)nseg * ((tps * 128 + 95) / 96) * 128;
+}
+
+static long long plan_workspace_bytes(const UmmaPlan& pl, long long width) {
+  return (long long)ws_digits_offset(pl) + (long long)pl.nch * UG_CHUNK_ROWS * width;
 }
 
 long long umma_workspace_bytes(int K, int vb, long long ld) {
-  long long m = 0;
+  long long m = 0, w3 = 0;
+  for (int n = 1; n <= 32; ++n) { const long long w = sparse_slots((int)ld, n); w3 = w > w3 ? w : w3; }
   for (int sums = 0; sums < 2; ++sums)
     for (int pair = 0; pair < 4; ++pair) {
-      const long long b = plan_workspace_bytes(make_umma_plan(K, vb, sums, pair & 1, pair >> 1), ld);
+      const long long b = plan_workspace_bytes(make_umma_plan(K, vb, sums, pair & 1, pair >> 1), pair >> 1 ? w3 : ld);
       m = b > m ? b : m;
     }
   return m;
@@ -580,76 +632,48 @@
   pair &= 1;
   if (mc && !pair) { set_error("stats_gram_umma: the multicast form needs CTA pairs"); return -2; }
   if (sp && kt != 128) { set_error("stats_gram_umma: the sparse form needs tile width 128"); return -2; }
-  const UmmaPlan pl = make_umma_plan(K, vb, sums, pair, sp);
-  if (workspace_bytes < plan_workspace_bytes(pl, ld)) { set_error("stats_gram_umma: workspace too small"); return -2; }
+  const UmmaPlan pd = make_umma_plan(K, vb, sums, pair, 0);
+  const UmmaPlan ps = make_umma_plan(K, vb, sums, pair, 1);
+  const int ktiles = (ld + kt - 1) / kt;
+  const int tps = (ktiles + nseg - 1) / nseg;
+  const int nseg_eff = (ktiles + tps - 1) / tps;
+  if (nseg_eff != nseg) { set_error("stats_gram_umma: nseg=%d leaves empty segments (use <= %d)", nseg, nseg_eff); return -2; }
+  const int sps = (tps * kt + 95) / 96;
+  const long long ldb = (long long)nseg * sps * 128;
+  long long need = plan_workspace_bytes(pd, ld);
+  if (sp) need = plan_workspace_bytes(ps, ldb) > need ? plan_workspace_bytes(ps, ldb) : need;
+  if (workspace_bytes < need) { set_error("stats_gram_umma: workspace too small"); return -2; }
   EncodeTiledFn encode = get_encode_fn();
   if (!encode) { set_error("stats_gram_umma: cuTensorMapEncodeTiled not available"); return -3; }
 
+  const int nc = pd.nc;
   uint8_t* ws = static_cast<uint8_t*>(workspace);
   unsigned long long* colmax = reinterpret_cast<unsigned long long*>(ws);
-  double* cscale = reinterpret_cast<double*>(ws + (size_t)pl.nc * 8);
-  int* cexp = reinterpret_cast<int*>(ws + (size_t)pl.nc * 16);
-  uint8_t* Bd = ws + ws_digits_offset(pl);
+  double* cscale = reinterpret_cast<double*>(ws + (size_t)(nc + 1) * 8);
+  int* cexp = reinterpret_cast<int*>(ws + (size_t)(2 * nc + 1) * 8);
+  uint8_t* Bd = ws + ws_digits_offset(pd);
   const int KP = 8 * tiles_for(K);
   const int nt = tiles_for(K);
 
-  cudaMemsetAsync(colmax, 0, (size_t)pl.nc * 8, st);
+  cudaMemsetAsync(colmax, 0, (size_t)(nc + 1) * 8, st);
   {
     const size_t sm = (size_t)(vb ? 2 : 1) * K * 65 * sizeof(double);
     int nbm = (cols + 63) / 64;
     if (nbm > 296) nbm = 296;
-    k_ug_colmax<<<nbm, 256, sm, st>>>(Xp, Vp, cols, KP, pl, colmax);
-    k_ug_scales<<<(pl.nc + 127) / 128, 128, 0, st>>>(colmax, pl.nc, cscale, cexp);
-    const size_t sq = (size_t)(vb ? 2 : 1) * K * 130 * sizeof(double) + (size_t)pl.nc * 4;
+    k_ug_colmax<<<nbm, 256, sm, st>>>(Xp, Vp, cols, KP, pd, colmax);
+    k_ug_scales<<<(nc + 127) / 128, 128, 0, st>>>(colmax, nc, cscale, cexp);
+    const size_t sq = (size_t)(vb ? 2 : 1) * K * 130 * sizeof(double) + (size_t)nc * 4;
     if (sq > 48 * 1024) cudaFuncSetAttribute(k_ug_quantize, cudaFuncAttributeMaxDynamicSharedMemorySize, (int)sq);
-    k_ug_quantize<<<dim3((ld + 127) / 128, 4), 128, sq, st>>>(Xp, Vp, cols, KP, (long long)ld, pl, cexp, Bd);
+    const int gx = sp && nseg * sps > (ld + 127) / 128 ? nseg * sps : (ld + 127) / 128;
+    k_ug_quantize<<<dim3(gx, 4), 128, sq, st>>>(Xp, Vp, cols, KP, ld, ldb, pd, ps, sp, tps * kt, sps, colmax + nc, cexp, Bd);
   }
   if (check_launch("stats_gram_umma prepass")) return -1;
 
-  CUtensorMap tmaps[2];
-  for (int which = 0; which < 2; ++which) {
-    const int nh = which ? pl.nh_last : pl.nh_full;
-    const cuuint64_t gdim[2] = {(cuuint64_t)ld, (cuuint64_t)pl.nch * UG_CHUNK_ROWS};
-    const cuuint64_t gstr[1] = {(cuuint64_t)ld};
-    const cuuint32_t box[2] = {(cuuint32_t)kt, (cuuint32_t)(pair ? nh / 2 : nh)};
-    const cuuint32_t estr[2] = {1, 1};
-    const CUresult r = encode(&tmaps[which], CU_TENSOR_MAP_DATA_TYPE_UINT8, 2, Bd, gdim, gstr, box, estr, CU_TENSOR_MAP_INTERLEAVE_NONE,
-                              kt == 128 ? CU_TENSOR_MAP_SWIZZLE_128B : CU_TENSOR_MAP_SWIZZLE_64B,
-                              CU_TENSOR_MAP_L2_PROMOTION_L2_256B, CU_TENSOR_MAP_FLOAT_OOB_FILL_NONE);
-    if (r != CUDA_SUCCESS) { set_error("stats_gram_umma: cuTensorMapEncodeTiled failed (%d)", (int)r); return -3; }
-  }
-
-  UmmaGramArgs a;
-  a.bits = bits; a.rows = rows; a.wpr = ld / 32; a.cols = cols; a.polarity = polarity;
-  a.ktiles = (ld + kt - 1) / kt;
-  a.tiles_per_seg = (a.ktiles + nseg - 1) / nseg;
-  const int nseg_eff = (a.ktiles + a.tiles_per_seg - 1) / a.tiles_per_seg;
-  if (nseg_eff != nseg) { set_error("stats_gram_umma: nseg=%d leaves empty segments (use <= %d)", nseg, nseg_eff); return -2; }
-  a.pl = pl; a.cscale = cscale; a.Gout = Gout; a.SVout = SVout; a.KP = KP; a.gl = nt * (nt + 1) / 2 * 64;
-  const int tail = UG_MASK_BUFS * UG_ROWS * 64 + (2 * 16 + 1 + 2 * UG_MASK_BUFS) * 8 + 16 + UG_EXP_WARPS * 32 * 4 + 2 * pl.cpc + 64;
-  size_t smem = 0;
-  for (int which = 0; which < 2; ++which) {
-    const int nh = which ? pl.nh_last : pl.nh_full;
-    const int stage_bytes = (sp ? UG_ROWS / 2 : UG_ROWS) * kt + (pair ? nh : 2 * nh) * kt;
-    int stages = (227 * 1024 - 1024 - tail) / stage_bytes;
-    if (stages > 16) stages = 16;
-    if (sp && stages > 8) stages = 8;
-    if (max_stages > 0 && stages > max_stages) stages = max_stages;
-    if (stages < 2) { set_error("stats_gram_umma: stage does not fit"); return -2; }
-    a.stages_of[which] = stages;
-    const size_t need = (size_t)stages * stage_bytes + tail + 1024;
-    smem = need > smem ? need : smem;
-  }
-  { const char* e = getenv("BNMTF_UMMA_DBG"); a.dbg = e ? atoi(e) : 0; }
-  if (smem < 116 * 1024) smem = 116 * 1024;
-  int rbs = (rows + UG_ROWS - 1) / UG_ROWS;
-  if (pair) rbs = (rbs + 1) / 2 * 2;
-  if (mc) rbs = (rbs + 3) / 4 * 4;
-  dim3 grid(rbs, pl.nch, nseg);
-  CUtensorMap tmap_bits = tmaps[0];
-  a.mask_tma = (ld % 128 == 0 && reinterpret_cast<uintptr_t>(bits) % 16 == 0) ? 1 : 0;
-  { const char* e = getenv("BNMTF_GRAM_MASK_TMA"); if (e && atoi(e) == 0) a.mask_tma = 0; }
-  if (a.mask_tma) {
+  CUtensorMap tmap_bits;
+  memset(&tmap_bits, 0, sizeof(tmap_bits));
+  const int mask_tma = (ld % 128 == 0 && reinterpret_cast<uintptr_t>(bits) % 16 == 0 && !(getenv("BNMTF_GRAM_MASK_TMA") &&
+                        atoi(getenv("BNMTF_GRAM_MASK_TMA")) == 0)) ? 1 : 0;
+  if (mask_tma) {
     const cuuint64_t gdim[2] = {(cuuint64_t)(ld / 32), (cuuint64_t)rows};
     const cuuint64_t gstr[1] = {(cuuint64_t)(ld / 32) * 4};
     const cuuint32_t box[2] = {16, (cuuint32_t)UG_ROWS};
@@ -659,21 +683,67 @@
                               CU_TENSOR_MAP_FLOAT_OOB_FILL_NONE);
     if (r != CUDA_SUCCESS) { set_error("stats_gram_umma: cuTensorMapEncodeTiled (mask) failed (%d)", (int)r); return -3; }
   }
-  void (*kern)(const CUtensorMap, const CUtensorMap, const CUtensorMap, UmmaGramArgs) =
-      mc ? (sp ? k_gram_umma<128, true, true, true> : (kt == 128 ? k_gram_umma<128, true, false, true> : k_gram_umma<64, true, false, true>))
-      : sp ? (pair ? k_gram_umma<128, true, true, false> : k_gram_umma<128, false, true, false>)
-         : kt == 128 ? (pair ? k_gram_umma<128, true, false, false> : k_gram_umma<128, false, false, false>)
-                     : (pair ? k_gram_umma<64, true, false, false> : k_gram_umma<64, false, false, false>);
-  cudaFuncSetAttribute(kern, cudaFuncAttributeMaxDynamicSharedMemorySize, (int)smem);
-  cudaLaunchConfig_t cfg = {};
-  cfg.gridDim = grid; cfg.blockDim = dim3(UG_THREADS); cfg.dynamicSmemBytes = smem; cfg.stream = st;
-  cudaLaunchAttribute attr[1];
-  attr[0].id = cudaLaunchAttributeClusterDimension;
-  attr[0].val.clusterDim.x = mc ? 4 : (pair ? 2 : 1); attr[0].val.clusterDim.y = 1; attr[0].val.clusterDim.z = 1;
-  cfg.attrs = attr; cfg.numAttrs = 1;
-  const cudaError_t le = cudaLaunchKernelEx(&cfg, kern, tmaps[0], tmaps[1], tmap_bits, a);
-  if (le != cudaSuccess) { set_error("stats_gram_umma: launch failed: %s", cudaGetErrorString(le)); cudaGetLastError(); return -1; }
-  return check_launch("stats_gram_umma");
-}
-
-}
+  const int dbg = getenv("BNMTF_UMMA_DBG") ? atoi(getenv("BNMTF_UMMA_DBG")) : 0;
+
+  auto launch = [&](const UmmaPlan& pl, int spx, long long width, const unsigned long long* negflag, int run_if_neg) -> int {
+    CUtensorMap tmaps[2];
+    for (int which = 0; which < 2; ++which) {
+      const int nh = which ? pl.nh_last : pl.nh_full;
+      const cuuint64_t gdim[2] = {(cuuint64_t)width, (cuuint64_t)pl.nch * UG_CHUNK_ROWS};
+      const cuuint64_t gstr[1] = {(cuuint64_t)width};
+      const cuuint32_t box[2] = {(cuuint32_t)kt, (cuuint32_t)(pair ? nh / 2 : nh)};
+      const cuuint32_t estr[2] = {1, 1};
+      const CUresult r = encode(&tmaps[which], CU_TENSOR_MAP_DATA_TYPE_UINT8, 2, Bd, gdim, gstr, box, estr, CU_TENSOR_MAP_INTERLEAVE_NONE,
+                                kt == 128 ? CU_TENSOR_MAP_SWIZZLE_128B : CU_TENSOR_MAP_SWIZZLE_64B,
+                                CU_TENSOR_MAP_L2_PROMOTION_L2_256B, CU_TENSOR_MAP_FLOAT_OOB_FILL_NONE);
+      if (r != CUDA_SUCCESS) { set_error("stats_gram_umma: cuTensorMapEncodeTiled failed (%d)", (int)r); return -3; }
+    }
+    UmmaGramArgs a;
+    a.bits = bits; a.rows = rows; a.wpr = ld / 32; a.cols = cols; a.polarity = polarity;
+    a.ktiles = spx ? nseg * sps : ktiles;
+    a.tiles_per_seg = spx ? sps : tps;
+    a.seg_cols = tps * kt;
+    a.negflag = negflag; a.run_if_neg = run_if_neg;
+    a.pl = pl; a.cscale = cscale; a.Gout = Gout; a.SVout = SVout; a.KP = KP; a.gl = nt * (nt + 1) / 2 * 64;
+    a.mask_tma = mask_tma; a.dbg = dbg;
+    const int tail = UG_MASK_BUFS * UG_ROWS * 64 + (2 * 16 + 1 + 2 * UG_MASK_BUFS) * 8 + 16 + UG_EXP_WARPS * 32 * 8 + 2 * pl.cpc + 64;
+    size_t smem = 0;
+    for (int which = 0; which < 2; ++which) {
+      const int nh = which ? pl.nh_last : pl.nh_full;
+      const int stage_bytes = (spx ? UG_ROWS / 2 : UG_ROWS) * kt + (pair ? nh : 2 * nh) * kt;
+      int stages = (227 * 1024 - 1024 - tail) / stage_bytes;
+      if (stages > 16) stages = 16;
+      if (spx && stages > 8) stages = 8;
+      if (max_stages > 0 && stages > max_stages) stages = max_stages;
+      if (stages < 2) { set_error("stats_gram_umma: stage does not fit"); return -2; }
+      a.stages_of[which] = stages;
+      const size_t need = (size_t)stages * stage_bytes + tail + 1024;
+      smem = need > smem ? need : smem;
+    }
+    if (smem < 116 * 1024) smem = 116 * 1024;
+    int rbs = (rows + UG_ROWS - 1) / UG_ROWS;
+    if (pair) rbs = (rbs + 1) / 2 * 2;
+    if (mc) rbs = (rbs + 3) / 4 * 4;
+    const dim3 grid(rbs, pl.nch, nseg);
+    void (*kern)(const CUtensorMap, const CUtensorMap, const CUtensorMap, UmmaGramArgs) =
+        mc ? (spx ? k_gram_umma<128, true, true, true> : (kt == 128 ? k_gram_umma<128, true, false, true> : k_gram_umma<64, true, false, true>))
+        : spx ? (pair ? k_gram_umma<128, true, true, false> : k_gram_umma<128, false, true, false>)
+           : kt == 128 ? (pair ? k_gram_umma<128, true, false, false> : k_gram_umma<128, false, false, false>)
+                       : (pair ? k_gram_umma<64, true, false, false> : k_gram_umma<64, false, false, false>);
+    cudaFuncSetAttribute(kern, cudaFuncAttributeMaxDynamicSharedMemorySize, (int)smem);
+    cudaLaunchConfig_t cfg = {};
+    cfg.gridDim = grid; cfg.blockDim = dim3(UG_THREADS); cfg.dynamicSmemBytes = smem; cfg.stream = st;
+    cudaLaunchAttribute attr[1];
+    attr[0].id = cudaLaunchAttributeClusterDimension;
+    attr[0].val.clusterDim.x = mc ? 4 : (pair ? 2 : 1); attr[0].val.clusterDim.y = 1; attr[0].val.clusterDim.z = 1;
+    cfg.attrs = attr; cfg.numAttrs = 1;
+    const cudaError_t le = cudaLaunchKernelEx(&cfg, kern, tmaps[0], tmaps[1], mask_tma ? tmap_bits : tmaps[0], a);
+    if (le != cudaSuccess) { set_error("stats_gram_umma: launch failed: %s", cudaGetErrorString(le)); cudaGetLastError(); return -1; }
+    return check_launch("stats_gram_umma");
+  };
+  if (!sp) return launch(pd, 0, ld, nullptr, 0);
+  const int r = launch(ps, 1, ldb, colmax + nc, 0);
+  return r ? r : launch(pd, 0, ld, colmax + nc, 1);
+}
+
+}
diff --git a/bnmtf_b200/csrc/stats.cu b/bnmtf_b200/csrc/stats.cu
--- a/bnmtf_b200/csrc/stats.cu
+++ b/bnmtf_b200/csrc/stats.cu
@@ -182,150 +182,6 @@
   }
 }
 
-constexpr int FIX_WARPS = 4;
-constexpr int FIX_QCAP = 1024;
-template <int NT, bool VB>
-__global__ void __launch_bounds__(32 * FIX_WARPS) k_gram_fixup(const uint32_t* __restrict__ bits, int rows, int ld, int cols,
-                                                               const double* __restrict__ Xp, const double* __restrict__ Vp,
-                                                               int polarity, double* __restrict__ Gout, double* __restrict__ SVout) {
-  constexpr int KP = 8 * NT;
-  constexpr int NTP = NT * (NT + 1) / 2;
-  __shared__ uint16_t queue[FIX_WARPS][FIX_QCAP + 16];
-  const int warp = threadIdx.x >> 5, lane = threadIdx.x & 31, g = lane >> 2, e = lane & 3;
-  const int row = blockIdx.x * FIX_WARPS + warp;
-  if (row >= rows) return;
-  const int wpr = ld >> 5;
-  const uint32_t* mrow = bits + (size_t)row * wpr;
-  const uint32_t flip = polarity ? 0u : 0xffffffffu;
-  uint16_t* q = queue[warp];
-
-  double acc[NTP][2];
-#pragma unroll
-  for (int p = 0; p < NTP; ++p) acc[p][0] = acc[p][1] = 0.0;
-  double sv[NT];
-#pragma unroll
-  for (int n = 0; n < NT; ++n) sv[n] = 0.0;
-
-  int qn = 0;
-  size_t qbase = 0;
-  auto drain = [&]() {
-    if (lane < 16) q[qn + lane] = 0xFFFFu;
-    __syncwarp();
-    for (int i = 0; i < qn; i += 16) {
-      double x[4][NT], v[4][NT];
-#pragma unroll
-      for (int u = 0; u < 4; ++u) {
-        const uint32_t off = q[i + 4 * u + e];
-        const size_t j = (off == 0xFFFFu) ? (size_t)ld : qbase + off;
-        const double* xr = Xp + j * KP + g;
-#pragma unroll
-        for (int n = 0; n < NT; ++n) x[u][n] = xr[8 * n];
-        if (VB) {
-          const double* vr = Vp + j * KP + g;
-#pragma unroll
-          for (int n = 0; n < NT; ++n) v[u][n] = vr[8 * n];
-        }
-      }
-#pragma unroll
-      for (int u = 0; u < 4; ++u) {
-#pragma unroll
-        for (int a = 0; a < NT; ++a)
-#pragma unroll
-          for (int b = a; b < NT; ++b) {
-            const int p = a * NT - a * (a - 1) / 2 + (b - a);
-            dmma884(acc[p][0], acc[p][1], x[u][a], x[u][b]);
-          }
-        if (VB) {
-#pragma unroll
-          for (int n = 0; n < NT; ++n) sv[n] += v[u][n];
-        }
-      }
-    }
-    __syncwarp();
-    qn = 0;
-  };
-
-  for (int wb = 0; wb < wpr; wb += 256) {
-    if ((size_t)wb * 32 - qbase >= 32768) { drain(); qbase = (size_t)wb * 32; }
-    uint32_t ov[8];
-    int cnt = 0;
-#pragma unroll
-    for (int c = 0; c < 8; ++c) {
-      const int w = wb + c * 32 + lane;
-      uint32_t m = w < wpr ? (mrow[w] ^ flip) : 0u;
-      const int jb = w * 32;
-      if (jb + 32 > cols) m = jb >= cols ? 0u : (m & ((1u << (cols - jb)) - 1u));
-      uint32_t v0, v1, meta;
-      ov[c] = sparse_split(m, v0, v1, meta);
-      cnt += __popc(ov[c]);
-    }
-    int incl = cnt;
-#pragma unroll
-    for (int o = 1; o < 32; o <<= 1) {
-      const int t = __shfl_up_sync(0xffffffffu, incl, o);
-      if (lane >= o) incl += t;
-    }
-    const int total = __shfl_sync(0xffffffffu, incl, 31);
-    if (qn + total > FIX_QCAP) drain();
-    if (total <= FIX_QCAP) {
-      int pos = qn + incl - cnt;
-#pragma unroll
-      for (int c = 0; c < 8; ++c) {
-        uint32_t m = ov[c];
-        const int cb = (int)((size_t)(wb + c * 32 + lane) * 32 - qbase);
-        while (m) {
-          const int b = __ffs(m) - 1;
-          m &= m - 1;
-          q[pos++] = (uint16_t)(cb + b);
-        }
-      }
-      qn += total;
-      __syncwarp();
-    } else {
-#pragma unroll 1
-      for (int c = 0; c < 8; ++c) {
-        const int cc = __popc(ov[c]);
-        int inc2 = cc;
-#pragma unroll
-        for (int o = 1; o < 32; o <<= 1) {
-          const int t = __shfl_up_sync(0xffffffffu, inc2, o);
-          if (lane >= o) inc2 += t;
-        }
-        const int tot2 = __shfl_sync(0xffffffffu, inc2, 31);
-        if (qn + tot2 > FIX_QCAP) drain();
-        int pos = qn + inc2 - cc;
-        uint32_t m = ov[c];
-        const int cb = (int)((size_t)(wb + c * 32 + lane) * 32 - qbase);
-        while (m) {
-          const int b = __ffs(m) - 1;
-          m &= m - 1;
-          q[pos++] = (uint16_t)(cb + b);
-        }
-        qn += tot2;
-        __syncwarp();
-      }
-    }
-  }
-  drain();
-
-  double* go = Gout + (size_t)row * (NTP * 64);
-#pragma unroll
-  for (int p = 0; p < NTP; ++p)
-    *reinterpret_cast<double2*>(go + p * 64 + g * 8 + 2 * e) = make_double2(acc[p][0], acc[p][1]);
-  if (VB) {
-#pragma unroll
-    for (int n = 0; n < NT; ++n) {
-      sv[n] += __shfl_xor_sync(0xffffffffu, sv[n], 1);
-      sv[n] += __shfl_xor_sync(0xffffffffu, sv[n], 2);
-    }
-    if (e == 0) {
-      double* so = SVout + (size_t)row * KP;
-#pragma unroll
-      for (int n = 0; n < NT; ++n) so[8 * n + g] = sv[n];
-    }
-  }
-}
-
 template <int NT, bool VB>
 __global__ void __launch_bounds__(256) k_gram_full(const double* __restrict__ Xp, const double* __restrict__ Vp, int n,
                                                   int K, int dummy_row, double* __restrict__ partial) {
@@ -435,27 +291,6 @@
   return check_launch("stats_gram");
 }
 
-int launch_stats_gram_fixup(const uint32_t* bits, int rows, int ld, int cols, const double* Xp, const double* Vp, int K,
-                            int polarity, double* Gout, double* SVout, cudaStream_t st) {
-  if (rows <= 0 || ld <= 0 || ld % 64 || cols <= 0 || cols > ld) { set_error("stats_gram_fixup: bad shape"); return -2; }
-  const int nt = tiles_for(K);
-  if (nt > 4) { set_error("stats_gram_fixup: K=%d > 31", K); return -2; }
-  const int wpr = ld / 32;
-  (void)wpr;
-  dim3 grid((rows + FIX_WARPS - 1) / FIX_WARPS, 1);
-  switch (nt) {
-    case 1: if (Vp) k_gram_fixup<1, true><<<grid, 32 * FIX_WARPS, 0, st>>>(bits, rows, ld, cols, Xp, Vp, polarity, Gout, SVout);
-            else k_gram_fixup<1, false><<<grid, 32 * FIX_WARPS, 0, st>>>(bits, rows, ld, cols, Xp, nullptr, polarity, Gout, nullptr); break;
-    case 2: if (Vp) k_gram_fixup<2, true><<<grid, 32 * FIX_WARPS, 0, st>>>(bits, rows, ld, cols, Xp, Vp, polarity, Gout, SVout);
-            else k_gram_fixup<2, false><<<grid, 32 * FIX_WARPS, 0, st>>>(bits, rows, ld, cols, Xp, nullptr, polarity, Gout, nullptr); break;
-    case 3: if (Vp) k_gram_fixup<3, true><<<grid, 32 * FIX_WARPS, 0, st>>>(bits, rows, ld, cols, Xp, Vp, polarity, Gout, SVout);
-            else k_gram_fixup<3, false><<<grid, 32 * FIX_WARPS, 0, st>>>(bits, rows, ld, cols, Xp, nullptr, polarity, Gout, nullptr); break;
-    default: if (Vp) k_gram_fixup<4, true><<<grid, 32 * FIX_WARPS, 0, st>>>(bits, rows, ld, cols, Xp, Vp, polarity, Gout, SVout);
-             else k_gram_fixup<4, false><<<grid, 32 * FIX_WARPS, 0, st>>>(bits, rows, ld, cols, Xp, nullptr, polarity, Gout, nullptr); break;
-  }
-  return check_launch("stats_gram_fixup");
-}
-
 int launch_gram_full(const double* Xp, const double* Vp, int n, int K, int dummy_row, double* out, double* scratch,
                      cudaStream_t st) {
   const int nt = tiles_for(K);
diff --git a/bnmtf_b200/engine.py b/bnmtf_b200/engine.py
--- a/bnmtf_b200/engine.py
+++ b/bnmtf_b200/engine.py
@@ -304,7 +304,7 @@
         self._graph = self._graph_key = self._graph_seen = None
         self.split = int(os.environ.get("BNMTF_SPLIT", "64" if self.K > 16 else ("80" if self.K > 8 else "96")))
         self.umma_pair = int(os.environ.get("BNMTF_UMMA_PAIR", "1"))
-        self._fix_stream = None
+        self.umma_sparse = "BNMTF_UMMA_PAIR" not in os.environ
         self._side = None
         self.m = MODE[mode]
         self.vb = mode == "vb"
@@ -358,15 +358,15 @@
                 tile = 128 if ld >= 256 else 64
                 sums = K if (side == 1 and self.metrics_mode == "stats") else 0
                 self.umma_form = getattr(self, "umma_form", {})
-                form = self.umma_pair
-                if tile != 128 or K > 31:
+                form = self.umma_pair | (2 if self.umma_sparse else 0)
+                digits = _lib.call("bnmtf_fixed_point_digits")
+                nc = K * (K + 1) // 2 + (K if self.vb else 0) + sums
+                nch = -(-nc // (512 // digits))
+                if tile != 128 or -(-nc // (480 // digits)) > nch:
                     form &= ~2
                 self.umma_form[side] = form
-                acc_cols = 480 if form & 2 else 512
-                nch = -(-(K * (K + 1) // 2 + (K if self.vb else 0) + sums) // (acc_cols // _lib.call("bnmtf_fixed_point_digits")))
                 ktiles = -(-ld // tile)
-                ng = _pick_nseg(((rb + 1) // 2 * 2 if form & 1 else rb) * nch, ktiles,
-                                t_tile=(0.3 if form & 2 else 0.55) * tile / 128, t_fix=10.0)
+                ng = _pick_nseg(((rb + 1) // 2 * 2 if form & 1 else rb) * nch, ktiles, t_tile=0.55 * tile / 128, t_fix=10.0)
                 self.umma_tile = getattr(self, "umma_tile", {})
                 self.umma_tile[side] = tile
             else:
@@ -376,7 +376,7 @@
             self.nseg[side] = (nrx, ng, nm)
         rI, rJ = max(1, self.loc[0][1]), max(1, self.loc[1][1])
         mrx = max(self.nseg[0][0] * rI, self.nseg[1][0] * rJ)
-        self.gram_segs = {side: self.nseg[side][1] + (1 if self.gram == "umma" and self.umma_form[side] & 2 else 0) for side in (0, 1)}
+        self.gram_segs = {side: self.nseg[side][1] for side in (0, 1)}
         mg = max(self.gram_segs[0] * rI, self.gram_segs[1] * rJ)
         f64 = lambda *shape: torch.zeros(shape, dtype=torch.float64, device=dev)
         self.RXpart = f64(mrx, KP)
@@ -515,25 +515,10 @@
         me, other, R, bits, rows, ld, lo = self._sides(side)
         ng = self.nseg[side][1]
         if self.gram == "umma":
-            form = self.umma_form[side]
-            if form & 2:
-                if self._fix_stream is None:
-                    self._fix_stream = torch.cuda.Stream(device=self.ds.device)
-                    self._fix_ev = [torch.cuda.Event(), torch.cuda.Event()]
-                main = torch.cuda.current_stream()
-                self._fix_ev[0].record(main)
-                self._fix_stream.wait_event(self._fix_ev[0])
-                with torch.cuda.stream(self._fix_stream):
-                    _lib.call("bnmtf_stats_gram_fixup_f64", _ptr(bits), rows, ld, other.n, _ptr(other.Xp), _ptr(other.Vp), self.K,
-                              self.polarity, self.Gpart.data_ptr() + 8 * ng * rows * self.Gpart.shape[1],
-                              self.SVpart.data_ptr() + 8 * ng * rows * self.SVpart.shape[1] if self.vb else 0, _stream())
-                    self._fix_ev[1].record(self._fix_stream)
             _lib.call("bnmtf_stats_gram_umma_f64", _ptr(bits), rows, ld, other.n, _ptr(other.Xp), _ptr(other.Vp), self.K,
-                      self.polarity, ng, self.umma_tile[side], form, 1 if sums else 0, self.umma_stages,
+                      self.polarity, ng, self.umma_tile[side], self.umma_form[side], 1 if sums else 0, self.umma_stages,
                       _ptr(self.Gpart),
                       _ptr(self.SVpart), self.ws_ptr, self.ws_bytes, _stream())
-            if form & 2:
-                torch.cuda.current_stream().wait_event(self._fix_ev[1])
         else:
             _lib.call("bnmtf_stats_gram_f64", _ptr(bits), rows, ld, _ptr(other.Xp), _ptr(other.Vp), self.K,
                       self.polarity, ng, _ptr(self.Gpart), _ptr(self.SVpart), _stream())
```
